# jinlinyi/PerspectiveFields

Hardware: NVIDIA H100
Metric: images/sec at 640x480 (Paramnet-360Cities-edina), H100 vs ref CPU (higher is better)
Workload: dtype f32 via 3x bf16 split MMA, fp32 accumulate

## Files before the change

include/pf_b200.h:

```cpp
#ifndef PF_B200_H_
#define PF_B200_H_

#include <stddef.h>
#include <stdint.h>

#ifdef __cplusplus
extern "C" {
#endif

#define PF_ABI_VERSION 2

typedef struct pf_engine* pf_handle;

enum pf_status { PF_OK = 0, PF_ERR_ARG = -1, PF_ERR_CUDA = -2, PF_ERR_WEIGHT = -3, PF_ERR_WORKSPACE = -4 };

enum pf_dtype { PF_F32 = 0, PF_BF16 = 1 };

enum pf_param_net { PF_PARAM_NONE = 0, PF_PARAM_CENTERED = 1 , PF_PARAM_UNCENTERED = 2  };

typedef struct pf_model_desc {
  int gravity_classes;
  int latitude_classes;
  int param_net;
  int param_input_size;
  float pixel_mean[3];
  float pixel_std[3];
} pf_model_desc;

typedef struct pf_batch {
  int n;
  const uint8_t* images_u8;
  const int64_t* image_offset;
  const float* images_chw;
  const int32_t* height;
  const int32_t* width;
  float* pred_gravity;
  float* pred_latitude;
  float* gravity_original;
  const int64_t* gravity_original_offset;
  float* latitude_original;
  const int64_t* latitude_original_offset;
  float* params;
} pf_batch;

int pf_abi_version(void);
const char* pf_last_error(void);

int64_t pf_kernel_launch_count(void);

int pf_create(int device, const pf_model_desc* desc, pf_handle* out);
int pf_create_sized(int device, const pf_model_desc* desc, int net_h, int net_w, pf_handle* out);
int pf_destroy(pf_handle h);

int pf_set_weight(pf_handle h, const char* name, const void* dev_ptr, int64_t numel, int dtype);
int pf_finalize(pf_handle h);

int64_t pf_workspace_bytes(pf_handle h, int n, int max_h);

int pf_forward(pf_handle h, const pf_batch* batch, void* workspace, int64_t workspace_bytes, void* stream);

int pf_profile_enable(pf_handle h, int on );
int pf_profile_read(pf_handle h, double* out21);
int pf_profile_kernels_enable(pf_handle h, int max_launches);
int pf_profile_kernels_read(pf_handle h, char* buf, int cap);

int pf_set_option(pf_handle h, const char* name, int value);

int pf_debug_enable(pf_handle h, int on);
int pf_debug_count(pf_handle h);
const char* pf_debug_name(pf_handle h, int i);
int64_t pf_debug_numel(pf_handle h, const char* name);
int pf_debug_copy(pf_handle h, const char* name, float* dst_dev, int64_t numel, void* stream);

typedef struct pf_camera {
  int32_t height, width;
  double focal_rel;
  double elevation, roll;
  double cx_rel, cy_rel;
  int64_t up_offset;
  int64_t lat_offset;
} pf_camera;
int pf_camera_fields(int device, const pf_camera* cams, int n, float* up, float* lat, void* stream);
int pf_camera_fields_vp(int device, const pf_camera* cams, const double* vp, int n, float* up, float* lat, void* stream);

typedef struct pf_pano_view {
  int32_t height, width;
  double f, xi;
  double az, el, roll;
  int64_t im_offset;
  int64_t field_offset;
} pf_pano_view;
int pf_pano_views(int device, const uint8_t* pano, int pano_h, int pano_w, const pf_pano_view* views, int n, uint8_t* im, float* ntheta,
                  float* nphi, float* up, float* lat, float* xy, double* offset, int32_t* status, void* stream);

typedef struct pf_equi_view {
  int32_t height, width;
  double vfov;
  double azimuth, elevation, roll;
  double ar;
  int64_t offset;
} pf_equi_view;
enum pf_equi_dtype { PF_EQUI_U8 = 0, PF_EQUI_F32 = 1 };
enum pf_equi_mode { PF_EQUI_BILINEAR = 0, PF_EQUI_NEAREST = 1 };
enum pf_equi_out { PF_EQUI_CAST = 0, PF_EQUI_UNIT = 1 };
int pf_equi_views(int device, const void* pano, int pano_h, int pano_w, int channels, int dtype, const pf_equi_view* views, int n, int mode,
                  int out_kind, int swap_rb, void* im, void* stream);

typedef struct pf_draw_canvas {
  int32_t height, width;
  int64_t img_offset;
  int64_t out_offset;
  int64_t lat_offset;
  int64_t up_offset;
  int64_t up_stride[3];
  int32_t density;
  int32_t arrow_inv_len;
  float arrow_rgb[3];
  float alpha_fill, alpha_line;
  int32_t draw_lat, draw_up;
} pf_draw_canvas;
int pf_draw_fields(int device, const pf_draw_canvas* canvases, int n, const uint8_t* img, uint8_t* out, const float* lat, const float* up,
                   void* stream);

typedef struct pf_comm* pf_comm_handle;
int pf_comm_unique_id(void* id128);
int pf_comm_create(int device, int rank, int nranks, const void* id128, pf_comm_handle* out);
int pf_comm_destroy(pf_comm_handle c);
int pf_gather(pf_comm_handle c, int root, int count, void* const* dev_ptrs, const int64_t* bytes, const int32_t* peer, void* stream);

typedef struct pf_jpeg* pf_jpeg_handle;
int pf_jpeg_create(int device, int max_threads , pf_jpeg_handle* out);
int pf_jpeg_destroy(pf_jpeg_handle j);
int pf_jpeg_info(pf_jpeg_handle j, const uint8_t* data, int64_t length, int32_t* height, int32_t* width);
int pf_jpeg_decode_batch(pf_jpeg_handle j, int n, const uint8_t* const* data, const int64_t* length, const int32_t* height,
                         const int32_t* width, uint8_t* blob, const int64_t* offset, void* stream);


int pf_op_conv_gemm(const float* x, int B, int H, int W, int Cin, const void* whi, const void* wlo, const float* bias,
                    int N, int KH, int KW, int stride, int pad, int in_relu, int act, const float* res, int res_relu,
                    float* y, void* stream);
typedef struct pf_tma_pred { const float* w; const float* b; float* out; int nc, mode; } pf_tma_pred;
typedef struct pf_tma_op {
  int mode;
  int64_t M; int K;
  int B, H, W, Cin;
  int N, groups;
  const void* a_hi; const void* a_lo; int lda, a_c0, a_gc;
  const void* a2_hi; const void* a2_lo; int lda2, c_split, a2_c0;
  const void* w_hi; const void* w_lo; const float* bias; int bias_mode, bias_gstride;
  int act; const float* gamma;
  const float* res; int ldr, r_coff, r_gcoff, res_relu;
  const float* res2; int ldr2, r2_coff, r2_gcoff;
  float* C; int ldc, c_coff, c_gcoff;
  void* s_hi; void* s_lo; int lds, s_coff, s_gcoff, split_relu;
  int phase4;
  int npred; pf_tma_pred pred[2];
  int force_bn, force_kb;
  int picked_bn, picked_kb;
  int force_sched, picked_sched;
} pf_tma_op;
int pf_op_tma(pf_tma_op* op, void* stream);
int pf_op_tma_bf16(pf_tma_op* op, void* stream);
int pf_op_conv1_ring(const void* c_hi, const void* c_lo, int B, int H, int W, const float* wf, const float* bias, float* out,
                     const float* pg_w, const float* pg_b, float* pg_out, const float* pl_w, const float* pl_b, float* pl_out, void* stream);
int pf_tma_pick_tile(int mode, int64_t M, int N, int K, int sm_count, int* bn, int* kb);
int pf_op_layernorm(const float* x, float* y, int64_t rows, int C, const float* w, const float* b, float eps, void* stream);
int pf_op_attention(const float* q, const float* kv, float* out, int B, int N, int C, int heads, void* stream);
int pf_op_attention_mma(const float* q, const float* kv, float* out, int B, int N, int C, int heads, void* stream);
int pf_op_attention_tc(const float* q, const float* kv, float* out, int B, int N, int C, int heads, void* stream);
int pf_op_attention_tc_bf16(const float* q, const float* kv, float* out, int B, int N, int C, int heads, void* stream);
int pf_op_attention_tc_keys(const float* q, const float* kv, float* out, int B, int N, int NKV, int C, int heads, int bf16, void* stream);
int pf_op_dwconv3x3_gelu(const float* x, float* y, int B, int H, int W, int C, const float* w9c, const float* bias, void* stream);
int pf_op_dwconv7x7(const float* x, float* y, int B, int H, int W, int C, const float* w49c, const float* bias, void* stream);
int pf_op_upsample2x(const float* x, float* y, int B, int H, int W, int C, void* stream);
int pf_op_preprocess(const uint8_t* img_dev, int H, int W, const float* mean3, const float* std3, float* y, void* stream);
int pf_op_preprocess_sized(const uint8_t* img_dev, int H, int W, int net_h, int net_w, const float* mean3, const float* std3, float* y, void* stream);
int pf_op_resize_u8(const uint8_t* img_dev, int H, int W, int new_h, int new_w, uint8_t* out_dev, void* stream);
int pf_op_resize_f32(const float* img_dev, int H, int W, int C, int new_h, int new_w, float* out_dev, void* stream);
int pf_op_fill_stream(float* dst, int64_t numel, float value, void* stream);
int pf_op_argmax_decode(const float* logits, float* field, int B, int HW, int NC, int is_gravity, void* stream);
int pf_op_pred_argmax_decode(const float* feat, int ld, int coff, const float* w, const float* bias, float* field, int B, int HW, int NC,
                             int is_gravity, void* stream);
int pf_op_postprocess(const float* vec, const float* lat, int n, const int32_t* height, const int32_t* width,
                      float* gravity_original, const int64_t* gravity_original_offset, float* latitude_original,
                      const int64_t* latitude_original_offset, int lat_is_sin, void* stream);
int pf_op_postprocess_sized(const float* vec, const float* lat, int n, int net_h, int net_w, const int32_t* height, const int32_t* width,
                            float* gravity_original, const int64_t* gravity_original_offset, float* latitude_original,
                            const int64_t* latitude_original_offset, int lat_is_sin, void* stream);

#ifdef __cplusplus
}
#endif
#endif
```

perspectivefields_b200/_native.py:

```python
import ctypes
import os
import subprocess

_HERE = os.path.dirname(os.path.abspath(__file__))
ROOT = os.path.dirname(_HERE)
LIB_PATH = os.path.join(_HERE, "libpf_b200.so")
SRC_DIR = os.path.join(_HERE, "csrc")
HEADER = os.path.join(ROOT, "include", "pf_b200.h")

PF_F32, PF_BF16 = 0, 1
PF_PARAM_NONE, PF_PARAM_CENTERED, PF_PARAM_UNCENTERED = 0, 1, 2

NVCC_FLAGS = ["-gencode", "arch=compute_90a,code=sm_90a", "-O3", "-lineinfo", "-std=c++17",
              "-Xcompiler", "-fPIC", "-shared", "-ldl"]


class pf_model_desc(ctypes.Structure):
    _fields_ = [("gravity_classes", ctypes.c_int), ("latitude_classes", ctypes.c_int), ("param_net", ctypes.c_int),
                ("param_input_size", ctypes.c_int), ("pixel_mean", ctypes.c_float * 3), ("pixel_std", ctypes.c_float * 3)]


class pf_camera(ctypes.Structure):
    _fields_ = [("height", ctypes.c_int32), ("width", ctypes.c_int32), ("focal_rel", ctypes.c_double), ("elevation", ctypes.c_double),
                ("roll", ctypes.c_double), ("cx_rel", ctypes.c_double), ("cy_rel", ctypes.c_double),
                ("up_offset", ctypes.c_int64), ("lat_offset", ctypes.c_int64)]


class pf_pano_view(ctypes.Structure):
    _fields_ = [("height", ctypes.c_int32), ("width", ctypes.c_int32), ("f", ctypes.c_double), ("xi", ctypes.c_double),
                ("az", ctypes.c_double), ("el", ctypes.c_double), ("roll", ctypes.c_double),
                ("im_offset", ctypes.c_int64), ("field_offset", ctypes.c_int64)]


class pf_equi_view(ctypes.Structure):
    _fields_ = [("height", ctypes.c_int32), ("width", ctypes.c_int32), ("vfov", ctypes.c_double), ("azimuth", ctypes.c_double),
                ("elevation", ctypes.c_double), ("roll", ctypes.c_double), ("ar", ctypes.c_double), ("offset", ctypes.c_int64)]


PF_EQUI_U8, PF_EQUI_F32 = 0, 1
PF_EQUI_BILINEAR, PF_EQUI_NEAREST = 0, 1
PF_EQUI_CAST, PF_EQUI_UNIT = 0, 1


class pf_draw_canvas(ctypes.Structure):
    _fields_ = [("height", ctypes.c_int32), ("width", ctypes.c_int32), ("img_offset", ctypes.c_int64), ("out_offset", ctypes.c_int64),
                ("lat_offset", ctypes.c_int64), ("up_offset", ctypes.c_int64), ("up_stride", ctypes.c_int64 * 3),
                ("density", ctypes.c_int32), ("arrow_inv_len", ctypes.c_int32), ("arrow_rgb", ctypes.c_float * 3),
                ("alpha_fill", ctypes.c_float), ("alpha_line", ctypes.c_float), ("draw_lat", ctypes.c_int32), ("draw_up", ctypes.c_int32)]


class pf_batch(ctypes.Structure):
    _fields_ = [("n", ctypes.c_int),
                ("images_u8", ctypes.c_void_p), ("image_offset", ctypes.POINTER(ctypes.c_int64)),
                ("images_chw", ctypes.c_void_p),
                ("height", ctypes.POINTER(ctypes.c_int32)), ("width", ctypes.POINTER(ctypes.c_int32)),
                ("pred_gravity", ctypes.c_void_p), ("pred_latitude", ctypes.c_void_p),
                ("gravity_original", ctypes.c_void_p), ("gravity_original_offset", ctypes.POINTER(ctypes.c_int64)),
                ("latitude_original", ctypes.c_void_p), ("latitude_original_offset", ctypes.POINTER(ctypes.c_int64)),
                ("params", ctypes.c_void_p)]


class pf_tma_pred(ctypes.Structure):
    _fields_ = [("w", ctypes.c_void_p), ("b", ctypes.c_void_p), ("out", ctypes.c_void_p), ("nc", ctypes.c_int), ("mode", ctypes.c_int)]


def _fields(spec):
    types = {"int": ctypes.c_int, "ptr": ctypes.c_void_p, "i64": ctypes.c_int64}
    out = []
    for decl in spec.split(";"):
        t, names = decl.split(None, 1)
        out += [(n.strip(), types[t]) for n in names.split(",")]
    return out


class pf_tma_op(ctypes.Structure):
    _fields_ = _fields("int mode; i64 M; int K, B, H, W, Cin, N, groups; ptr a_hi, a_lo; int lda, a_c0, a_gc; ptr a2_hi, a2_lo;"
                       "int lda2, c_split, a2_c0; ptr w_hi, w_lo, bias; int bias_mode, bias_gstride, act; ptr gamma, res;"
                       "int ldr, r_coff, r_gcoff, res_relu; ptr res2; int ldr2, r2_coff, r2_gcoff; ptr C; int ldc, c_coff, c_gcoff;"
                       "ptr s_hi, s_lo; int lds, s_coff, s_gcoff, split_relu, phase4, npred") + \
        [("pred", pf_tma_pred * 2)] + _fields("int force_bn, force_kb, picked_bn, picked_kb, force_sched, picked_sched")


def _sources():
    return sorted(os.path.join(SRC_DIR, f) for f in os.listdir(SRC_DIR) if f.endswith((".cu", ".cuh"))) + [HEADER]


def needs_build():
    if not os.path.exists(LIB_PATH):
        return True
    t = os.path.getmtime(LIB_PATH)
    return any(os.path.getmtime(s) > t for s in _sources())


def build(force=False, verbose=False):
    if not force and not needs_build():
        return LIB_PATH
    nvcc = os.environ.get("NVCC", "/usr/local/cuda/bin/nvcc")
    cmd = [nvcc] + NVCC_FLAGS + [os.path.join(SRC_DIR, "pf_b200.cu"), "-o", LIB_PATH + ".tmp"]
    if verbose:
        cmd.insert(1, "-Xptxas=-v")
    r = subprocess.run(cmd, capture_output=True, text=True)
    if r.returncode != 0:
        raise RuntimeError("nvcc failed:\n" + " ".join(cmd) + "\n" + r.stdout + r.stderr)
    os.replace(LIB_PATH + ".tmp", LIB_PATH)
    if verbose:
        print(r.stderr)
    return LIB_PATH


_lib = None


def lib():
    global _lib
    if _lib is not None:
        return _lib
    if not os.path.exists(LIB_PATH):
        raise RuntimeError(f"{LIB_PATH} is missing: run `python -c 'import __graft_entry__ as g; g.build()'` "
                           "(perspectivefields_b200 has no CPU or PyTorch fallback)")
    L = ctypes.CDLL(os.environ.get("PF_B200_LIB") or LIB_PATH)
    vp, i32, i64, f32 = ctypes.c_void_p, ctypes.c_int, ctypes.c_int64, ctypes.c_float
    sig = {
        "pf_abi_version": (i32, []),
        "pf_last_error": (ctypes.c_char_p, []),
        "pf_kernel_launch_count": (i64, []),
        "pf_create": (i32, [i32, ctypes.POINTER(pf_model_desc), ctypes.POINTER(vp)]),
        "pf_create_sized": (i32, [i32, ctypes.POINTER(pf_model_desc), i32, i32, ctypes.POINTER(vp)]),
        "pf_destroy": (i32, [vp]),
        "pf_set_weight": (i32, [vp, ctypes.c_char_p, vp, i64, i32]),
        "pf_finalize": (i32, [vp]),
        "pf_workspace_bytes": (i64, [vp, i32, i32]),
        "pf_forward": (i32, [vp, ctypes.POINTER(pf_batch), vp, i64, vp]),
        "pf_profile_enable": (i32, [vp, i32]),
        "pf_profile_read": (i32, [vp, ctypes.POINTER(ctypes.c_double)]),
        "pf_profile_kernels_enable": (i32, [vp, i32]),
        "pf_profile_kernels_read": (i32, [vp, ctypes.c_char_p, i32]),
        "pf_debug_enable": (i32, [vp, i32]),
        "pf_debug_count": (i32, [vp]),
        "pf_debug_name": (ctypes.c_char_p, [vp, i32]),
        "pf_debug_numel": (i64, [vp, ctypes.c_char_p]),
        "pf_debug_copy": (i32, [vp, ctypes.c_char_p, vp, i64, vp]),
        "pf_op_conv_gemm": (i32, [vp, i32, i32, i32, i32, vp, vp, vp, i32, i32, i32, i32, i32, i32, i32, vp, i32, vp, vp]),
        "pf_op_tma": (i32, [ctypes.POINTER(pf_tma_op), vp]),
        "pf_op_tma_bf16": (i32, [ctypes.POINTER(pf_tma_op), vp]),
        "pf_op_conv1_ring": (i32, [vp, vp, i32, i32, i32, vp, vp, vp, vp, vp, vp, vp, vp, vp, vp]),
        "pf_tma_pick_tile": (i32, [i32, i64, i32, i32, i32, ctypes.POINTER(i32), ctypes.POINTER(i32)]),
        "pf_set_option": (i32, [vp, ctypes.c_char_p, i32]),
        "pf_camera_fields": (i32, [i32, ctypes.POINTER(pf_camera), i32, vp, vp, vp]),
        "pf_camera_fields_vp": (i32, [i32, ctypes.POINTER(pf_camera), ctypes.POINTER(ctypes.c_double), i32, vp, vp, vp]),
        "pf_draw_fields": (i32, [i32, ctypes.POINTER(pf_draw_canvas), i32, vp, vp, vp, vp, vp]),
        "pf_pano_views": (i32, [i32, vp, i32, i32, ctypes.POINTER(pf_pano_view), i32, vp, vp, vp, vp, vp, vp, vp, vp, vp]),
        "pf_equi_views": (i32, [i32, vp, i32, i32, i32, i32, ctypes.POINTER(pf_equi_view), i32, i32, i32, i32, vp, vp]),
        "pf_op_layernorm": (i32, [vp, vp, i64, i32, vp, vp, f32, vp]),
        "pf_op_attention": (i32, [vp, vp, vp, i32, i32, i32, i32, vp]),
        "pf_op_attention_mma": (i32, [vp, vp, vp, i32, i32, i32, i32, vp]),
        "pf_op_attention_tc": (i32, [vp, vp, vp, i32, i32, i32, i32, vp]),
        "pf_op_attention_tc_bf16": (i32, [vp, vp, vp, i32, i32, i32, i32, vp]),
        "pf_op_attention_tc_keys": (i32, [vp, vp, vp, i32, i32, i32, i32, i32, i32, vp]),
        "pf_op_dwconv3x3_gelu": (i32, [vp, vp, i32, i32, i32, i32, vp, vp, vp]),
        "pf_op_dwconv7x7": (i32, [vp, vp, i32, i32, i32, i32, vp, vp, vp]),
        "pf_op_upsample2x": (i32, [vp, vp, i32, i32, i32, i32, vp]),
        "pf_op_preprocess": (i32, [vp, i32, i32, ctypes.POINTER(f32), ctypes.POINTER(f32), vp, vp]),
        "pf_op_preprocess_sized": (i32, [vp, i32, i32, i32, i32, ctypes.POINTER(f32), ctypes.POINTER(f32), vp, vp]),
        "pf_op_resize_u8": (i32, [vp, i32, i32, i32, i32, vp, vp]),
        "pf_op_resize_f32": (i32, [vp, i32, i32, i32, i32, i32, vp, vp]),
        "pf_op_argmax_decode": (i32, [vp, vp, i32, i32, i32, i32, vp]),
        "pf_op_fill_stream": (i32, [vp, i64, f32, vp]),
        "pf_op_pred_argmax_decode": (i32, [vp, i32, i32, vp, vp, vp, i32, i32, i32, i32, vp]),
        "pf_op_postprocess": (i32, [vp, vp, i32, ctypes.POINTER(ctypes.c_int32), ctypes.POINTER(ctypes.c_int32), vp, ctypes.POINTER(i64), vp,
                                    ctypes.POINTER(i64), i32, vp]),
        "pf_op_postprocess_sized": (i32, [vp, vp, i32, i32, i32, ctypes.POINTER(ctypes.c_int32), ctypes.POINTER(ctypes.c_int32), vp,
                                          ctypes.POINTER(i64), vp, ctypes.POINTER(i64), i32, vp]),
        "pf_comm_unique_id": (i32, [vp]),
        "pf_comm_create": (i32, [i32, i32, i32, vp, ctypes.POINTER(vp)]),
        "pf_comm_destroy": (i32, [vp]),
        "pf_gather": (i32, [vp, i32, i32, ctypes.POINTER(vp), ctypes.POINTER(i64), ctypes.POINTER(ctypes.c_int32), vp]),
        "pf_jpeg_create": (i32, [i32, i32, ctypes.POINTER(vp)]),
        "pf_jpeg_destroy": (i32, [vp]),
        "pf_jpeg_info": (i32, [vp, vp, i64, ctypes.POINTER(ctypes.c_int32), ctypes.POINTER(ctypes.c_int32)]),
        "pf_jpeg_decode_batch": (i32, [vp, i32, ctypes.POINTER(vp), ctypes.POINTER(i64), ctypes.POINTER(ctypes.c_int32),
                                       ctypes.POINTER(ctypes.c_int32), vp, ctypes.POINTER(i64), vp]),
    }
    for name, (res, args) in sig.items():
        try:
            fn = getattr(L, name)
        except AttributeError:
            if os.environ.get("PF_B200_LIB"):
                continue
            raise
        fn.restype, fn.argtypes = res, args
    if L.pf_abi_version() != 2:
        raise RuntimeError("libpf_b200.so ABI version mismatch")
    _lib = L
    return L


EXPORTS = ["pf_abi_version", "pf_last_error", "pf_kernel_launch_count", "pf_create", "pf_create_sized", "pf_destroy", "pf_set_weight",
           "pf_finalize", "pf_workspace_bytes", "pf_forward", "pf_profile_enable", "pf_profile_read", "pf_profile_kernels_enable",
           "pf_profile_kernels_read", "pf_set_option", "pf_debug_enable", "pf_debug_count", "pf_debug_name", "pf_debug_numel",
           "pf_debug_copy", "pf_camera_fields", "pf_camera_fields_vp", "pf_pano_views", "pf_equi_views", "pf_draw_fields", "pf_comm_unique_id", "pf_comm_create", "pf_comm_destroy", "pf_gather",
           "pf_jpeg_create", "pf_jpeg_destroy", "pf_jpeg_info", "pf_jpeg_decode_batch",
           "pf_op_conv_gemm", "pf_op_tma", "pf_op_tma_bf16", "pf_op_conv1_ring", "pf_tma_pick_tile", "pf_op_layernorm", "pf_op_attention",
           "pf_op_attention_mma", "pf_op_attention_tc", "pf_op_attention_tc_bf16", "pf_op_attention_tc_keys", "pf_op_dwconv3x3_gelu",
           "pf_op_dwconv7x7", "pf_op_upsample2x", "pf_op_preprocess", "pf_op_preprocess_sized", "pf_op_fill_stream", "pf_op_resize_u8",
           "pf_op_resize_f32", "pf_op_argmax_decode", "pf_op_pred_argmax_decode", "pf_op_postprocess", "pf_op_postprocess_sized"]


class PfError(RuntimeError):
    pass


def check(status):
    if status < 0:
        raise PfError(f"libpf_b200: {lib().pf_last_error().decode()} (status {status})")
    return status
```

perspectivefields_b200/csrc/gemm_tma.cuh:

```cuda
#pragma once
#include <cuda.h>

#include "tc_ptx.cuh"

namespace pf {

constexpr int MODE_GEMM = 0, MODE_HALO = 1;
constexpr int kTmaThreads = 384;
constexpr int kHaloBytes = 180 * 128;

struct TmaGemmParams {
  int M;
  int B, H, W;
  int Cin;
  int N, K;
  int a_c0, a_gc;
  int c_split, a2_c0;
  int groups;
  int b_row0;
  const float* bias; int bias_mode, bias_gstride;
  int act; const float* gamma;
  const float* res;  int ldr, r_coff, r_gcoff, res_relu;
  const float* res2; int ldr2, r2_coff, r2_gcoff;
  float* C; int ldc, c_coff, c_gcoff;
  __nv_bfloat16* Shi; __nv_bfloat16* Slo; int lds, s_coff, s_gcoff, split_relu;
  const float* pred_w; const float* pred_b; float* pred_out; int pred_nc, pred_mode;
  int phase4;
};

template <int BN, int MODE, int KB, bool PP = false, int NP = 3> struct TmaCfg {
  static_assert(KB == 32 || KB == 64, "KB");
  static_assert(BN % 32 == 0 && BN <= 256, "BN");
  static_assert(!PP || MODE == MODE_GEMM, "the ping-pong schedule is a GEMM-mode schedule");
  static_assert(NP == 1 || NP == 3, "NP");
  static constexpr int kPlanes = NP == 3 ? 2 : 1;
  static constexpr int kTileM = PP ? 64 : 128;
  static constexpr int kBPlane = BN * KB * 2;
  static constexpr int kAPlane = kTileM * KB * 2;
  static constexpr int kStage = (MODE == MODE_GEMM ? kPlanes * kAPlane : 0) + kPlanes * kBPlane;
  static constexpr int kABuf = kPlanes * kHtPlaneBytes;
  static constexpr int kAccPitch = 68;
  static constexpr int kAccStage = 2 * 64 * kAccPitch * 4;
  static constexpr int kBudget = 225 * 1024 - kAccStage - (MODE == MODE_HALO ? 2 * kABuf : 0);
  static constexpr int kStagesRaw = kBudget / kStage;
  static constexpr int kStages = kStagesRaw > 16 ? 16 : kStagesRaw;
  static constexpr int kSmemBytes = (MODE == MODE_HALO ? 2 * kABuf : 0) + kStages * kStage + kAccStage + 512 + 1024;
  static_assert(kStages >= 2, "ring too shallow");
  static_assert(kSmemBytes <= 227 * 1024, "shared memory per block");
};

__device__ __forceinline__ void mbar_expect_tx(uint32_t bar, uint32_t bytes) {
  asm volatile("mbarrier.arrive.expect_tx.shared::cta.b64 _, [%0], %1;\n" ::"r"(bar), "r"(bytes) : "memory");
}
__device__ __forceinline__ void tma_load_2d(uint32_t dst, const CUtensorMap* map, uint32_t bar, int c0, int c1) {
  asm volatile("cp.async.bulk.tensor.2d.shared::cluster.global.mbarrier::complete_tx::bytes [%0], [%1, {%3, %4}], [%2];\n"
               ::"r"(dst), "l"(reinterpret_cast<uint64_t>(map)), "r"(bar), "r"(c0), "r"(c1) : "memory");
}
__device__ __forceinline__ void tma_load_4d(uint32_t dst, const CUtensorMap* map, uint32_t bar, int c0, int c1, int c2, int c3) {
  asm volatile("cp.async.bulk.tensor.4d.shared::cluster.global.mbarrier::complete_tx::bytes [%0], [%1, {%3, %4, %5, %6}], [%2];\n"
               ::"r"(dst), "l"(reinterpret_cast<uint64_t>(map)), "r"(bar), "r"(c0), "r"(c1), "r"(c2), "r"(c3) : "memory");
}
__device__ __forceinline__ void tma_prefetch_desc(const CUtensorMap* map) {
  asm volatile("prefetch.tensormap [%0];\n" ::"l"(reinterpret_cast<uint64_t>(map)) : "memory");
}

struct TmaMaps {
  CUtensorMap a_hi, a_lo, a2_hi, a2_lo, b_hi, b_lo;
};

template <int BN, int MODE, int KB, bool PP = false, int NP = 3>
__global__ void __launch_bounds__(kTmaThreads, 1) gemm_tma_kernel(const __grid_constant__ TmaMaps maps, const TmaGemmParams p, int tiles_x, int tiles_y) {
  using Cfg = TmaCfg<BN, MODE, KB, PP, NP>;
  constexpr bool kLo = NP == 3;
  constexpr int NS = Cfg::kStages;
  constexpr int SPC = 9 * (64 / KB);
  constexpr int kConsumerWarps = PP ? 4 : 8;
  extern __shared__ unsigned char smem_dyn[];
  const uint32_t raw = smem_u32(smem_dyn);
  const uint32_t sbase = (raw + 1023u) & ~1023u;
  unsigned char* sm = smem_dyn + (sbase - raw);
  const uint32_t a_base = sbase;
  const uint32_t ring = sbase + (MODE == MODE_HALO ? 2 * Cfg::kABuf : 0);
  const uint32_t acc_base = ring + NS * Cfg::kStage;
  const uint32_t bars = acc_base + Cfg::kAccStage;
  auto full_b = [&](int s) { return bars + 8u * s; };
  auto empty_b = [&](int s) { return bars + 8u * (NS + s); };
  auto full_a = [&](int i) { return bars + 8u * (2 * NS + i); };
  auto empty_a = [&](int i) { return bars + 8u * (2 * NS + 2 + i); };
  auto order_b = [&](int w) { return bars + 8u * (2 * NS + 4 + w); };

  const int tid = threadIdx.x, lane = tid & 31, warp = tid >> 5;
  const int n_tiles = cdiv(p.N, BN);
  const int m_tiles = MODE == MODE_GEMM ? cdiv(p.M, Cfg::kTileM) : p.B * tiles_x * tiles_y;
  const int total_tiles = m_tiles * n_tiles * p.groups;
  const int nchunks = MODE == MODE_HALO ? p.Cin / 64 : 0;
  const int nk = MODE == MODE_GEMM ? p.K / KB : nchunks * SPC;
  const bool b_resident = MODE == MODE_HALO && nchunks == 1 && SPC <= NS;

  if (tid == 0) {
    tma_prefetch_desc(&maps.a_hi); tma_prefetch_desc(&maps.b_hi);
    if (kLo) { tma_prefetch_desc(&maps.a_lo); tma_prefetch_desc(&maps.b_lo); }
    for (int s = 0; s < NS; ++s) { mbar_init(full_b(s), 1); mbar_init(empty_b(s), kConsumerWarps); }
    for (int i = 0; i < 2; ++i) { mbar_init(full_a(i), 1); mbar_init(empty_a(i), kConsumerWarps); mbar_init(order_b(i), 4); }
    fence_mbar_init();
  }
  __syncthreads();
  pdl_wait();
  pdl_launch();

  auto decode = [&](int tile, int& mt, int& g, int& n0) {
    n0 = (tile % n_tiles) * BN;
    tile /= n_tiles;
    g = tile % p.groups;
    mt = tile / p.groups;
  };

  if (warp < 4) {
    asm volatile("setmaxnreg.dec.sync.aligned.u32 40;\n");
    if (warp == 0 && lane == 0) {
      int it = 0;
      for (int tile = blockIdx.x; tile < total_tiles; tile += gridDim.x) {
        int mt, g, n0;
        decode(tile, mt, g, n0);
        const int brow = p.b_row0 + g * p.N + n0;
        if (b_resident && it > 0) break;
        for (int kc = 0; kc < nk; ++kc, ++it) {
          const int s = it % NS;
          mbar_wait(empty_b(s), ((it / NS) & 1) ^ 1);
          mbar_expect_tx(full_b(s), Cfg::kStage);
          const uint32_t st = ring + s * Cfg::kStage;
          int kcol;
          if (MODE == MODE_GEMM) {
            kcol = kc * KB;
            tma_load_2d(st, &maps.a_hi, full_b(s), p.a_c0 + g * p.a_gc + kcol, mt * Cfg::kTileM);
            if (kLo) tma_load_2d(st + Cfg::kAPlane, &maps.a_lo, full_b(s), p.a_c0 + g * p.a_gc + kcol, mt * Cfg::kTileM);
          } else {
            const int c = kc / SPC, u = kc - c * SPC;
            kcol = KB == 32 ? (u >> 1) * p.Cin + c * 64 + (u & 1) * 32 : u * p.Cin + c * 64;
          }
          const uint32_t bdst = st + (MODE == MODE_GEMM ? Cfg::kPlanes * Cfg::kAPlane : 0);
          tma_load_2d(bdst, &maps.b_hi, full_b(s), kcol, brow);
          if (kLo) tma_load_2d(bdst + Cfg::kBPlane, &maps.b_lo, full_b(s), kcol, brow);
        }
      }
    } else if (MODE == MODE_HALO && warp == 1 && lane == 0) {
      int ita = 0;
      for (int tile = blockIdx.x; tile < total_tiles; tile += gridDim.x) {
        int mt, g, n0;
        decode(tile, mt, g, n0);
        const int tx = mt % tiles_x, ty = (mt / tiles_x) % tiles_y, bimg = mt / (tiles_x * tiles_y);
        for (int c = 0; c < nchunks; ++c, ++ita) {
          const int buf = ita & 1;
          mbar_wait(empty_a(buf), ((ita >> 1) & 1) ^ 1);
          mbar_expect_tx(full_a(buf), Cfg::kPlanes * kHaloBytes);
          const uint32_t dst = a_base + buf * Cfg::kABuf;
          const int ci = c * 64;
          if (p.c_split > 0 && ci >= p.c_split) {
            tma_load_4d(dst, &maps.a2_hi, full_a(buf), p.a2_c0 + ci - p.c_split, tx * kHtTileW - 1, ty * kHtTileH - 1, bimg);
            if (kLo) tma_load_4d(dst + kHtPlaneBytes, &maps.a2_lo, full_a(buf), p.a2_c0 + ci - p.c_split, tx * kHtTileW - 1, ty * kHtTileH - 1, bimg);
          } else {
            tma_load_4d(dst, &maps.a_hi, full_a(buf), p.a_c0 + g * p.a_gc + ci, tx * kHtTileW - 1, ty * kHtTileH - 1, bimg);
            if (kLo) tma_load_4d(dst + kHtPlaneBytes, &maps.a_lo, full_a(buf), p.a_c0 + g * p.a_gc + ci, tx * kHtTileW - 1, ty * kHtTileH - 1, bimg);
          }
        }
      }
    }
    return;
  }

  asm volatile("setmaxnreg.inc.sync.aligned.u32 232;\n");
  const int wg = (warp >> 2) - 1;
  const int wt = tid & 127;
  float* stage = reinterpret_cast<float*>(sm + (acc_base - sbase)) + wg * 64 * Cfg::kAccPitch;
  const int erow = wt & 63, eh = wt >> 6;
  const int r = PP ? erow : wg * 64 + erow;
  constexpr int kTileStep = PP ? 2 : 1;
  float acc[BN / 2];
  int it = 0, ita = 0;
  for (int tl = PP ? wg : 0, tile = blockIdx.x + tl * gridDim.x; tile < total_tiles; tile += kTileStep * gridDim.x, tl += kTileStep) {
    int mt, g, n0;
    decode(tile, mt, g, n0);
    if (PP) {
      it = tl * nk;
      if (tl > 0) mbar_wait(order_b(wg ^ 1), ((tl - 1) >> 1) & 1);
    }
    int prev_s = -1, prev_buf = -1;
    fence_regs(acc);
    for (int kc = 0; kc < nk; ++kc, ++it) {
      const int s = it % NS;
      uint32_t a_hi, a_lo;
      bool chunk_end = false;
      int buf = 0;
      if (MODE == MODE_HALO) {
        const int c = kc / SPC, u = kc - c * SPC;
        const int tap = KB == 32 ? (u >> 1) : u, ky = tap / 3, kx = tap - ky * 3;
        buf = ita & 1;
        if (u == 0) mbar_wait(full_a(buf), (ita >> 1) & 1);
        a_hi = a_base + buf * Cfg::kABuf + ((ky + 8 * wg) * kHtHaloW + kx) * 128 + (KB == 32 ? (u & 1) * 64 : 0);
        a_lo = a_hi + kHtPlaneBytes;
        chunk_end = u == SPC - 1;
      } else {
        a_hi = ring + s * Cfg::kStage + (PP ? 0 : wg * 64 * KB * 2);
        a_lo = a_hi + Cfg::kAPlane;
      }
      const int sb = b_resident ? kc : s;
      if (!b_resident || tl == 0) mbar_wait(full_b(sb), b_resident ? 0 : ((it / NS) & 1));
      const uint32_t b_hi = ring + sb * Cfg::kStage + (MODE == MODE_GEMM ? Cfg::kPlanes * Cfg::kAPlane : 0);
      const uint64_t dah = MODE == MODE_HALO ? ht_a_desc(a_hi) : wgmma_tile_desc<KB>(a_hi);
      const uint64_t dbh = wgmma_tile_desc<KB>(b_hi);
      wgmma_fence();
      if (kLo) {
        const uint64_t dal = MODE == MODE_HALO ? ht_a_desc(a_lo) : wgmma_tile_desc<KB>(a_lo);
        const uint64_t dbl = wgmma_tile_desc<KB>(b_hi + Cfg::kBPlane);
#pragma unroll
        for (int kk = 0; kk < KB / 16; ++kk) {
          const uint32_t first = (kc | kk) ? 1u : 0u;
          wgmma_bf16<BN>(acc, dal + 2 * kk, dbh + 2 * kk, first);
          wgmma_bf16<BN>(acc, dah + 2 * kk, dbl + 2 * kk, 1u);
          wgmma_bf16<BN>(acc, dah + 2 * kk, dbh + 2 * kk, 1u);
        }
      } else {
#pragma unroll
        for (int kk = 0; kk < KB / 16; ++kk) wgmma_bf16<BN>(acc, dah + 2 * kk, dbh + 2 * kk, (kc | kk) ? 1u : 0u);
      }
      wgmma_commit();
      wgmma_wait<1>();
      if (lane == 0 && prev_s >= 0) {
        if (!b_resident) mbar_arrive(empty_b(prev_s));
        if (MODE == MODE_HALO && prev_buf >= 0) mbar_arrive(empty_a(prev_buf));
      }
      prev_s = s;
      prev_buf = chunk_end ? buf : -1;
      if (MODE == MODE_HALO && chunk_end) ++ita;
    }
    if (PP && lane == 0) mbar_arrive(order_b(wg));
    wgmma_wait<0>();
    fence_regs(acc);
    if (lane == 0 && prev_s >= 0) {
      if (!b_resident) mbar_arrive(empty_b(prev_s));
      if (MODE == MODE_HALO && prev_buf >= 0) mbar_arrive(empty_a(prev_buf));
    }

    long long m;
    bool valid;
    int cls_off = 0;
    int bimg = 0, oy = 0, ox = 0;
    if (MODE == MODE_GEMM) {
      m = (long long)mt * Cfg::kTileM + r;
      valid = m < p.M;
    } else {
      const int tx = mt % tiles_x, ty = (mt / tiles_x) % tiles_y;
      bimg = mt / (tiles_x * tiles_y);
      oy = ty * kHtTileH + (r >> 3); ox = tx * kHtTileW + (r & 7);
      valid = oy < p.H && ox < p.W;
      m = ((long long)bimg * p.H + oy) * p.W + ox;
      if (p.bias_mode == 2) {
        const int ry = oy == 0 ? 0 : (oy == p.H - 1 ? 2 : 1);
        const int rx = ox == 0 ? 0 : (ox == p.W - 1 ? 2 : 1);
        cls_off = (ry * 3 + rx) * p.N;
      }
    }
    const float* __restrict__ bias = p.bias ? p.bias + (long long)g * p.bias_gstride : nullptr;
    const int frow = (wt >> 5) * 16 + (lane >> 2), fcol = 2 * (lane & 3);
#pragma unroll
    for (int rd = 0; rd < (BN + 63) / 64; ++rd) {
      named_bar_sync(1 + wg, 128);
#pragma unroll
      for (int jb = 0; jb < 8; ++jb) {
        const int cb = rd * 8 + jb;
        if (cb < BN / 8) {
          float* d0 = stage + frow * Cfg::kAccPitch + jb * 8 + fcol;
          *reinterpret_cast<float2*>(d0) = make_float2(acc[4 * cb], acc[4 * cb + 1]);
          *reinterpret_cast<float2*>(d0 + 8 * Cfg::kAccPitch) = make_float2(acc[4 * cb + 2], acc[4 * cb + 3]);
        }
      }
      named_bar_sync(1 + wg, 128);
      const int ch = 2 * rd + eh;
      const bool ph4 = MODE == MODE_HALO && BN == 128 && p.phase4;
      const bool staged_split = p.Shi && !ph4;
      float o[32];
      if (ch < BN / 32) {
        const int nb = n0 + ch * 32;
        const long long mo = ph4 ? ((long long)bimg * 2 * p.H + 2 * oy + (ch >> 1)) * (2 * p.W) + 2 * ox + (ch & 1) : m;
        const int nbo = ph4 ? 0 : nb;
        const bool chunk_ok = nb < p.N;
        const float* srow = stage + erow * Cfg::kAccPitch + eh * 32;
#pragma unroll
        for (int j = 0; j < 32; j += 4) {
          const float4 t = *reinterpret_cast<const float4*>(srow + j);
          o[j] = t.x; o[j + 1] = t.y; o[j + 2] = t.z; o[j + 3] = t.w;
        }
        if (valid && chunk_ok) {
          if (p.bias_mode) {
#pragma unroll
            for (int j = 0; j < 32; j += 4) {
              const float4 bv = __ldg(reinterpret_cast<const float4*>(bias + cls_off + nb + j));
              o[j] += bv.x; o[j + 1] += bv.y; o[j + 2] += bv.z; o[j + 3] += bv.w;
            }
          }
          if (p.act == 1) {
#pragma unroll
            for (int j = 0; j < 32; ++j) o[j] = fmaxf(o[j], 0.f);
          } else if (p.act == 2) {
#pragma unroll
            for (int j = 0; j < 32; ++j) o[j] = gelu_erf(o[j]);
          }
          if (p.gamma) {
#pragma unroll
            for (int j = 0; j < 32; j += 4) {
              const float4 gv = __ldg(reinterpret_cast<const float4*>(p.gamma + nb + j));
              o[j] *= gv.x; o[j + 1] *= gv.y; o[j + 2] *= gv.z; o[j + 3] *= gv.w;
            }
          }
          if (p.res) {
            const float* rp = p.res + m * p.ldr + p.r_coff + g * p.r_gcoff + nb;
#pragma unroll
            for (int j = 0; j < 32; j += 4) {
              float4 rv = *reinterpret_cast<const float4*>(rp + j);
              if (p.res_relu) { rv.x = fmaxf(rv.x, 0.f); rv.y = fmaxf(rv.y, 0.f); rv.z = fmaxf(rv.z, 0.f); rv.w = fmaxf(rv.w, 0.f); }
              o[j] += rv.x; o[j + 1] += rv.y; o[j + 2] += rv.z; o[j + 3] += rv.w;
            }
          }
          if (p.res2) {
            const float* rp = p.res2 + m * p.ldr2 + p.r2_coff + g * p.r2_gcoff + nb;
#pragma unroll
            for (int j = 0; j < 32; j += 4) {
              const float4 rv = *reinterpret_cast<const float4*>(rp + j);
              o[j] += rv.x; o[j + 1] += rv.y; o[j + 2] += rv.z; o[j + 3] += rv.w;
            }
          }
          if (MODE == MODE_HALO && (BN == 32 || BN == 128) && p.pred_w) {
            float v0 = __ldg(p.pred_b), v1 = p.pred_nc > 1 ? __ldg(p.pred_b + 1) : 0.f;
#pragma unroll
            for (int j = 0; j < 32; j += 4) {
              const float4 w0 = __ldg(reinterpret_cast<const float4*>(p.pred_w + j));
              v0 = fmaf(o[j], w0.x, v0); v0 = fmaf(o[j + 1], w0.y, v0); v0 = fmaf(o[j + 2], w0.z, v0); v0 = fmaf(o[j + 3], w0.w, v0);
              if (p.pred_nc > 1) {
                const float4 w1 = __ldg(reinterpret_cast<const float4*>(p.pred_w + 32 + j));
                v1 = fmaf(o[j], w1.x, v1); v1 = fmaf(o[j + 1], w1.y, v1); v1 = fmaf(o[j + 2], w1.z, v1); v1 = fmaf(o[j + 3], w1.w, v1);
              }
            }
            const long long HWl = (long long)p.H * p.W * (ph4 ? 4 : 1);
            const long long bi = mo / HWl, pix = mo - bi * HWl;
            float* po = p.pred_out + bi * p.pred_nc * HWl + pix;
            if (p.pred_mode == 1) {
              const float nrm = fmaxf(sqrtf(v0 * v0 + v1 * v1), 1e-12f);
              po[0] = v0 / nrm; po[HWl] = v1 / nrm;
            } else {
              po[0] = fminf(fmaxf(v0, -1.f), 1.f);
            }
          }
        }
        if (chunk_ok && (p.C || (p.Shi && !staged_split))) {
          const bool odd = lane & 1;
          const bool valid_p = __shfl_xor_sync(0xffffffffu, (int)valid, 1) != 0;
          const long long mo_p = mo + (odd ? -1 : 1) * (ph4 ? 2 : 1);
          const long long moA = odd ? mo_p : mo, moB = odd ? mo : mo_p;
          const bool vA = odd ? valid_p : valid, vB = odd ? valid : valid_p;
          if (p.C) {
            float* cA = p.C + moA * p.ldc + p.c_coff + g * p.c_gcoff + nbo + (odd ? 4 : 0);
            float* cB = p.C + moB * p.ldc + p.c_coff + g * p.c_gcoff + nbo + (odd ? 4 : 0);
#pragma unroll
            for (int t = 0; t < 4; ++t) {
              float k[4], rr[4];
#pragma unroll
              for (int e = 0; e < 4; ++e) {
                k[e] = odd ? o[8 * t + 4 + e] : o[8 * t + e];
                rr[e] = __shfl_xor_sync(0xffffffffu, odd ? o[8 * t + e] : o[8 * t + 4 + e], 1);
              }
              if (vA) *reinterpret_cast<float4*>(cA + 8 * t) = odd ? make_float4(rr[0], rr[1], rr[2], rr[3]) : make_float4(k[0], k[1], k[2], k[3]);
              if (vB) *reinterpret_cast<float4*>(cB + 8 * t) = odd ? make_float4(k[0], k[1], k[2], k[3]) : make_float4(rr[0], rr[1], rr[2], rr[3]);
            }
          }
          if (p.Shi && !staged_split) {
            const long long sA = moA * p.lds + p.s_coff + g * p.s_gcoff + nbo + (odd ? 8 : 0);
            const long long sB = moB * p.lds + p.s_coff + g * p.s_gcoff + nbo + (odd ? 8 : 0);
#pragma unroll
            for (int t = 0; t < 2; ++t) {
              float k[8], rr[8];
#pragma unroll
              for (int e = 0; e < 8; ++e) {
                const float mine = odd ? o[16 * t + 8 + e] : o[16 * t + e], give = odd ? o[16 * t + e] : o[16 * t + 8 + e];
                k[e] = p.split_relu ? fmaxf(mine, 0.f) : mine;
                rr[e] = __shfl_xor_sync(0xffffffffu, p.split_relu ? fmaxf(give, 0.f) : give, 1);
              }
              uint4 kh, kl, rh, rl;
              split_bf16x2(k[0], k[1], kh.x, kl.x); split_bf16x2(k[2], k[3], kh.y, kl.y);
              split_bf16x2(k[4], k[5], kh.z, kl.z); split_bf16x2(k[6], k[7], kh.w, kl.w);
              split_bf16x2(rr[0], rr[1], rh.x, rl.x); split_bf16x2(rr[2], rr[3], rh.y, rl.y);
              split_bf16x2(rr[4], rr[5], rh.z, rl.z); split_bf16x2(rr[6], rr[7], rh.w, rl.w);
              if (vA) {
                *reinterpret_cast<uint4*>(p.Shi + sA + 16 * t) = odd ? rh : kh;
                *reinterpret_cast<uint4*>(p.Slo + sA + 16 * t) = odd ? rl : kl;
              }
              if (vB) {
                *reinterpret_cast<uint4*>(p.Shi + sB + 16 * t) = odd ? kh : rh;
                *reinterpret_cast<uint4*>(p.Slo + sB + 16 * t) = odd ? kl : rl;
              }
            }
          }
        }
      }
      if (staged_split) {
        named_bar_sync(1 + wg, 128);
        unsigned char* sS = reinterpret_cast<unsigned char*>(stage);
        if (ch < BN / 32) {
#pragma unroll
          for (int t = 0; t < 4; ++t) {
            uint4 h, l;
            float k[8];
#pragma unroll
            for (int e = 0; e < 8; ++e) k[e] = p.split_relu ? fmaxf(o[8 * t + e], 0.f) : o[8 * t + e];
            split_bf16x2(k[0], k[1], h.x, l.x); split_bf16x2(k[2], k[3], h.y, l.y);
            split_bf16x2(k[4], k[5], h.z, l.z); split_bf16x2(k[6], k[7], h.w, l.w);
            const int off = erow * 128 + (((eh * 4 + t) ^ (erow & 7)) << 4);
            *reinterpret_cast<uint4*>(sS + off) = h;
            *reinterpret_cast<uint4*>(sS + 64 * 128 + off) = l;
          }
        }
        named_bar_sync(1 + wg, 128);
#pragma unroll
        for (int i = wt; i < 2 * 64 * 8; i += 128) {
          const int lo_plane = i >> 9, rr = (i >> 3) & 63, pc = i & 7;
          const int col = rd * 64 + pc * 8;
          if (col >= BN || n0 + col >= p.N) continue;
          long long mr;
          bool vr;
          if (MODE == MODE_GEMM) {
            mr = (long long)mt * Cfg::kTileM + (PP ? 0 : wg * 64) + rr;
            vr = mr < p.M;
          } else {
            const int rt = wg * 64 + rr, tx = mt % tiles_x, ty = (mt / tiles_x) % tiles_y;
            const int py = ty * kHtTileH + (rt >> 3), px = tx * kHtTileW + (rt & 7);
            vr = py < p.H && px < p.W;
            mr = ((long long)bimg * p.H + py) * p.W + px;
          }
          if (!vr) continue;
          const uint4 v = *reinterpret_cast<const uint4*>(sS + lo_plane * 64 * 128 + rr * 128 + ((pc ^ (rr & 7)) << 4));
          *reinterpret_cast<uint4*>((lo_plane ? p.Slo : p.Shi) + mr * p.lds + p.s_coff + g * p.s_gcoff + n0 + col) = v;
        }
      }
    }
  }
}

}
```

perspectivefields_b200/csrc/pf_b200.cu:

```cuda
#include "../../include/pf_b200.h"

#include <cuda_runtime.h>
#include <nvtx3/nvToolsExt.h>

#include <atomic>
#include <cctype>
#include <cmath>
#include <cstdarg>
#include <cstdio>
#include <cstdlib>
#include <cstring>
#include <map>
#include <mutex>
#include <string>
#include <functional>
#include <unordered_map>
#include <vector>

#include "common.cuh"
#include "tma_host.cuh"
#include "attention_mma.cuh"
#include "layers.cuh"
#include "prepost.cuh"
#include "pano.cuh"
#include "equi.cuh"
#include "draw.cuh"
#include "comm.cuh"
#include "jpeg.cuh"

using namespace pf;

static thread_local std::string g_err;
static std::atomic<long long> g_launches{0};

static int fail(int code, const char* fmt, ...) {
  char buf[1024];
  va_list ap;
  va_start(ap, fmt);
  vsnprintf(buf, sizeof(buf), fmt, ap);
  va_end(ap);
  g_err = buf;
  return code;
}
#define CU(expr)                                                                                    \
  do {                                                                                              \
    cudaError_t e__ = (expr);                                                                       \
    if (e__ != cudaSuccess) return fail(PF_ERR_CUDA, "%s: %s (%s:%d)", #expr, cudaGetErrorString(e__), __FILE__, __LINE__); \
  } while (0)
static char g_crumb[96] = "";
static bool sync_debug() {
  static int v = -1;
  if (v < 0) v = getenv("PF_SYNC_DEBUG") ? 1 : 0;
  return v == 1;
}
struct KernelProf {
  bool on = false;
  cudaStream_t st = nullptr;
  std::vector<cudaEvent_t> pool;
  size_t used = 0;
  struct Rec { const char* expr; cudaEvent_t a, b; };
  std::vector<Rec> recs;
  cudaEvent_t next() { return used < pool.size() ? pool[used++] : nullptr; }
};
static thread_local KernelProf* tl_kp = nullptr;
#define LAUNCHED(expr)                                                                              \
  do {                                                                                              \
    KernelProf* kp__ = tl_kp;                                                                       \
    cudaEvent_t ka__ = (kp__ && kp__->on) ? kp__->next() : nullptr;                                 \
    if (ka__) cudaEventRecord(ka__, kp__->st);                                                      \
    cudaError_t e__ = (expr);                                                                       \
    g_launches.fetch_add(1, std::memory_order_relaxed);                                             \
    if (ka__) {                                                                                     \
      cudaEvent_t kb__ = kp__->next();                                                              \
      if (kb__) { cudaEventRecord(kb__, kp__->st); kp__->recs.push_back({#expr, ka__, kb__}); }     \
    }                                                                                               \
    if (e__ == cudaSuccess && sync_debug()) e__ = cudaDeviceSynchronize();                          \
    if (e__ != cudaSuccess) return fail(PF_ERR_CUDA, "%s: %s (%s:%d, after tap '%s')", #expr, cudaGetErrorString(e__), __FILE__, __LINE__, g_crumb); \
  } while (0)
struct NvtxRange {
  explicit NvtxRange(const char* name) { nvtxRangePushA(name); }
  ~NvtxRange() { nvtxRangePop(); }
};
#define TRY(expr)                \
  do {                           \
    int r__ = (expr);            \
    if (r__ != PF_OK) return r__; \
  } while (0)

static const int kMitDims[4] = {64, 128, 320, 512};
static const int kMitHeads[4] = {1, 2, 5, 8};
static const int kMitDepths[4] = {3, 4, 18, 3};
static const int kMitSr[4] = {8, 4, 2, 1};
static const int kCnxDims[4] = {96, 192, 384, 768};
static const int kCnxDepths[4] = {3, 3, 9, 3};

struct WeightRef { const void* p; long long numel; int dtype; };
struct GemmW { const __nv_bfloat16* hi = nullptr; const __nv_bfloat16* lo = nullptr; const float* b = nullptr; };
struct LnW { const float* w = nullptr; const float* b = nullptr; };

struct MitBlockW { LnW ln1, srln, ln2; GemmW q, sr, kv, proj, fc1, fc2; const float* dw_w; const float* dw_b; };
struct CnxBlockW { const float* dw_w; const float* dw_b; LnW ln; GemmW pw1, pw2; const float* gamma; };

struct Arena {
  char* base = nullptr;
  long long cap = 0, off = 0, peak = 0;
  bool dry = false, keep = false;
  void* alloc(long long bytes) {
    off = (off + 255) & ~255LL;
    void* p = dry ? nullptr : base + off;
    off += bytes;
    if (off > peak) peak = off;
    return p;
  }
  float* f(long long n) { return (float*)alloc(n * 4); }
  long long mark() const { return off; }
  void release(long long m) { if (!keep) off = m; }
};

struct pf_engine {
  int device = 0;
  pf_model_desc desc{};
  int net_h = kNet, net_w = kNet;
  bool finalized = false;
  std::unordered_map<std::string, WeightRef> weights;
  const float *embed1_w, *embed1_b, *llenc_w, *llenc_b;
  LnW embed_ln[4], stage_norm[4];
  GemmW embed[4];
  GemmW embed1g, llencg;
  std::vector<MitBlockW> blocks[4];
  GemmW proc[4];
  GemmW rcu[4][2][2];
  GemmW conv0, conv1;
  GemmW conv1p;
  const float *conv1f_w, *conv1f_b;
  bool use_fork = false;
  cudaStream_t side = nullptr;
  cudaEvent_t ev_fork = nullptr, ev_join = nullptr;
  bool use_dwln = false;
  bool use_pdl = true;
  bool decode_only = false;
  bool use_attn_split = true;
  bool use_phase = true;
  const float *pred_g_w, *pred_g_b, *pred_l_w, *pred_l_b;
  const float *pn_stem_w, *pn_stem_b;
  LnW pn_stem_ln, pn_ds_ln[4], pn_norm;
  GemmW pn_ds[4];
  std::vector<CnxBlockW> pn_blocks[4];
  const float *pn_head_w, *pn_head_b;
  struct DevTable { int ksize; int* bounds; int* coeffs; };
  std::map<std::pair<int, int>, DevTable> tables;
  char* table_dev = nullptr;
  char* table_host = nullptr;
  long long table_off = 0;
  KernelProf kp;
  struct MapKey {
    const void* base; long long d0, d1, d2; int kind, box, kb;
    bool operator==(const MapKey& o) const { return base == o.base && d0 == o.d0 && d1 == o.d1 && d2 == o.d2 && kind == o.kind && box == o.box && kb == o.kb; }
  };
  struct MapKeyHash {
    size_t operator()(const MapKey& k) const {
      size_t h = std::hash<const void*>()(k.base);
      for (long long v : {k.d0, k.d1, k.d2, (long long)k.kind, (long long)k.box, (long long)k.kb}) h = h * 1000003u ^ std::hash<long long>()(v);
      return h;
    }
  };
  std::unordered_map<MapKey, CUtensorMap, MapKeyHash> map_cache;
  bool use_stem_tc = true;
  bool use_attn_mma = true;
  bool bf16 = false;
  int sm_count = 132;
  bool profile = false;
  struct ProfRec { cudaEvent_t a, b; double flops; int cfg; int M, N, K, KH, stride, groups, Cin; };
  std::vector<ProfRec> prof;
  std::vector<cudaEvent_t> ev_pool;
  bool debug = false;
  std::vector<std::pair<std::string, std::pair<const float*, long long>>> taps;
};

static int get_w(pf_engine* e, const std::string& name, int dtype, long long numel, const void** out) {
  auto it = e->weights.find(name);
  if (it == e->weights.end()) return fail(PF_ERR_WEIGHT, "missing weight '%s'", name.c_str());
  if (it->second.dtype != dtype) return fail(PF_ERR_WEIGHT, "weight '%s': wrong dtype", name.c_str());
  if (it->second.numel != numel) return fail(PF_ERR_WEIGHT, "weight '%s': numel %lld, expected %lld", name.c_str(), it->second.numel, numel);
  *out = it->second.p;
  return PF_OK;
}
static int get_f(pf_engine* e, const std::string& n, long long numel, const float** out) { return get_w(e, n, PF_F32, numel, (const void**)out); }
static int get_gemm(pf_engine* e, const std::string& n, long long N, long long K, long long nbias, GemmW* g, int groups = 1) {
  TRY(get_w(e, n + ".whi", PF_BF16, groups * N * K, (const void**)&g->hi));
  TRY(get_w(e, n + ".wlo", PF_BF16, groups * N * K, (const void**)&g->lo));
  TRY(get_f(e, n + ".b", groups * nbias, &g->b));
  return PF_OK;
}
static int get_ln(pf_engine* e, const std::string& n, int C, LnW* l) {
  TRY(get_f(e, n + ".w", C, &l->w));
  TRY(get_f(e, n + ".b", C, &l->b));
  return PF_OK;
}

static int resolve_weights(pf_engine* e) {
  char nm[128];
  TRY(get_f(e, "embed1.w", 147 * 64, &e->embed1_w));
  TRY(get_f(e, "embed1.b", 64, &e->embed1_b));
  TRY(get_f(e, "llenc.w", 147 * 64, &e->llenc_w));
  TRY(get_f(e, "llenc.b", 64, &e->llenc_b));
  TRY(get_gemm(e, "embed1g", 64, 160, 64, &e->embed1g));
  TRY(get_gemm(e, "llencg", 64, 160, 64, &e->llencg));
  for (int s = 0; s < 4; ++s) {
    const int C = kMitDims[s];
    snprintf(nm, sizeof nm, "embed%d.ln", s + 1);
    TRY(get_ln(e, nm, C, &e->embed_ln[s]));
    if (s > 0) {
      snprintf(nm, sizeof nm, "embed%d", s + 1);
      TRY(get_gemm(e, nm, C, 9LL * kMitDims[s - 1], C, &e->embed[s]));
    }
    e->blocks[s].resize(kMitDepths[s]);
    for (int i = 0; i < kMitDepths[s]; ++i) {
      MitBlockW& b = e->blocks[s][i];
      char p[64];
      snprintf(p, sizeof p, "s%d.b%d.", s + 1, i);
      std::string P(p);
      TRY(get_ln(e, P + "ln1", C, &b.ln1));
      TRY(get_gemm(e, P + "q", C, C, C, &b.q));
      if (kMitSr[s] > 1) {
        TRY(get_gemm(e, P + "sr", C, (long long)kMitSr[s] * kMitSr[s] * C, C, &b.sr));
        TRY(get_ln(e, P + "srln", C, &b.srln));
      }
      TRY(get_gemm(e, P + "kv", 2 * C, C, 2 * C, &b.kv));
      TRY(get_gemm(e, P + "proj", C, C, C, &b.proj));
      TRY(get_ln(e, P + "ln2", C, &b.ln2));
      TRY(get_gemm(e, P + "fc1", 4 * C, C, 4 * C, &b.fc1));
      TRY(get_f(e, P + "dw.w", 9LL * 4 * C, &b.dw_w));
      TRY(get_f(e, P + "dw.b", 4 * C, &b.dw_b));
      TRY(get_gemm(e, P + "fc2", C, 4 * C, C, &b.fc2));
    }
    snprintf(nm, sizeof nm, "s%d.norm", s + 1);
    TRY(get_ln(e, nm, C, &e->stage_norm[s]));
  }
  for (int l = 0; l < 4; ++l) {
    snprintf(nm, sizeof nm, "head.proc%d", l + 1);
    TRY(get_gemm(e, nm, 512, 9LL * kMitDims[l], 9 * 512, &e->proc[l]));
  }
  for (int f = 0; f < 4; ++f)
    for (int u = 0; u < 2; ++u) {
      if (f == 3 && u == 0) continue;
      for (int c = 0; c < 2; ++c) {
        snprintf(nm, sizeof nm, "head.f%d.u%d.c%d", f + 1, u + 1, c + 1);
        TRY(get_gemm(e, nm, 256, 2304, 256, &e->rcu[f][u][c], 2));
      }
    }
  TRY(get_gemm(e, "head.conv0", 64, 9 * 320, 64, &e->conv0, 2));
  TRY(get_gemm(e, "head.conv1", 32, 9 * 64, 32, &e->conv1, 2));
  TRY(get_gemm(e, "head.conv1p", 128, 9 * 64, 128, &e->conv1p, 2));
  TRY(get_f(e, "head.conv1f.w", 2LL * 9 * 64 * 32, &e->conv1f_w));
  TRY(get_f(e, "head.conv1f.b", 64, &e->conv1f_b));
  TRY(get_f(e, "head.pred_g.w", 32LL * e->desc.gravity_classes, &e->pred_g_w));
  TRY(get_f(e, "head.pred_g.b", e->desc.gravity_classes, &e->pred_g_b));
  TRY(get_f(e, "head.pred_l.w", 32LL * e->desc.latitude_classes, &e->pred_l_w));
  TRY(get_f(e, "head.pred_l.b", e->desc.latitude_classes, &e->pred_l_b));
  if (e->desc.param_net != PF_PARAM_NONE) {
    TRY(get_f(e, "pn.stem.w", 48 * 96, &e->pn_stem_w));
    TRY(get_f(e, "pn.stem.b", 96, &e->pn_stem_b));
    TRY(get_ln(e, "pn.stem.ln", 96, &e->pn_stem_ln));
    for (int k = 1; k < 4; ++k) {
      snprintf(nm, sizeof nm, "pn.ds%d.ln", k);
      TRY(get_ln(e, nm, kCnxDims[k - 1], &e->pn_ds_ln[k]));
      snprintf(nm, sizeof nm, "pn.ds%d", k);
      TRY(get_gemm(e, nm, kCnxDims[k], 4LL * kCnxDims[k - 1], kCnxDims[k], &e->pn_ds[k]));
    }
    for (int s = 0; s < 4; ++s) {
      const int C = kCnxDims[s];
      e->pn_blocks[s].resize(kCnxDepths[s]);
      for (int j = 0; j < kCnxDepths[s]; ++j) {
        CnxBlockW& b = e->pn_blocks[s][j];
        char p[64];
        snprintf(p, sizeof p, "pn.s%d.b%d.", s, j);
        std::string P(p);
        TRY(get_f(e, P + "dw.w", 49LL * C, &b.dw_w));
        TRY(get_f(e, P + "dw.b", C, &b.dw_b));
        TRY(get_ln(e, P + "ln", C, &b.ln));
        TRY(get_gemm(e, P + "pw1", 4 * C, C, 4 * C, &b.pw1));
        TRY(get_gemm(e, P + "pw2", C, 4 * C, C, &b.pw2));
        TRY(get_f(e, P + "gamma", C, &b.gamma));
      }
    }
    TRY(get_ln(e, "pn.norm", 768, &e->pn_norm));
    TRY(get_f(e, "pn.head.w", 5 * 768, &e->pn_head_w));
    TRY(get_f(e, "pn.head.b", 5, &e->pn_head_b));
  }
  return PF_OK;
}

struct Fwd {
  pf_engine* e;
  Arena ar;
  cudaStream_t st;
  bool dry;
  int n;

  int tap(const char* name, const float* p, long long numel) {
    if (!e->debug) return PF_OK;
    float* cp = ar.f(numel);
    if (dry) return PF_OK;
    snprintf(g_crumb, sizeof g_crumb, "%s", name);
    if (sync_debug()) fprintf(stderr, "[pf tap] %s cp=%p (+%lld of cap %lld) p=%p numel=%lld\n", name, (void*)cp, (long long)((char*)cp - ar.base), ar.cap, (const void*)p, numel);
    CU(cudaMemcpyAsync(cp, p, numel * 4, cudaMemcpyDeviceToDevice, st));
    if (sync_debug()) CU(cudaDeviceSynchronize());
    e->taps.push_back({name, {cp, numel}});
    return PF_OK;
  }
  int tapf(const float* p, long long numel, const char* fmt, ...) {
    if (!e->debug) return PF_OK;
    char buf[96];
    va_list ap;
    va_start(ap, fmt);
    vsnprintf(buf, sizeof buf, fmt, ap);
    va_end(ap);
    return tap(buf, p, numel);
  }

  SplitT salloc(long long pixels, int ld) {
    SplitT t;
    t.hi = (__nv_bfloat16*)ar.alloc(pixels * ld * 2);
    t.lo = (__nv_bfloat16*)ar.alloc(pixels * ld * 2);
    t.ld = ld;
    return t;
  }
  int tap_split(const char* name, const SplitT& t, long long numel) {
    if (!e->debug) return PF_OK;
    float* cp = ar.f(numel);
    if (dry) return PF_OK;
    snprintf(g_crumb, sizeof g_crumb, "%s", name);
    LAUNCHED((merge_split_kernel<<<(unsigned)cdivl(numel, 256), 256, 0, st>>>(t.hi, t.lo, cp, numel), cudaGetLastError()));
    e->taps.push_back({name, {cp, numel}});
    return PF_OK;
  }
  static cudaError_t gemm_tma_gemm_mode(const TmaMaps& maps, const TmaGemmParams& p, int bn, int kb, bool pp, int np, int sms, cudaStream_t st, const PredTail* pred) {
    return gemm_tma_launch(MODE_GEMM, maps, p, bn, kb, pp, np, sms, st, pred);
  }
  static cudaError_t gemm_tma_halo_mode(const TmaMaps& maps, const TmaGemmParams& p, int bn, int kb, bool pp, int np, int sms, cudaStream_t st, const PredTail* pred) {
    return gemm_tma_launch(MODE_HALO, maps, p, bn, kb, pp, np, sms, st, pred);
  }
  int np() const { return e->bf16 ? 1 : 3; }
  int force_bn = 0, force_kb = 0;
  int force_sched = 0;
  int picked_bn = 0, picked_kb = 0, picked_sched = 0;
  int pick_tile(int mode, const TmaGemmParams& p, const PredTail* pred, int& bn, int& kb, bool& pp) {
    tma_pick_tile(mode, p.M, p.N, p.K, e->sm_count, bn, kb);
    if (force_bn) { bn = force_bn; kb = tma_pick_kb(bn, p.K, mode); }
    if (force_kb) kb = force_kb;
    pp = mode == MODE_GEMM && (force_sched ? force_sched == 2 : tma_pick_pingpong(p.M, p.N, p.K, bn, e->sm_count));
    if (const char* msg = gemm_tma_check(mode, p, bn, kb, pred != nullptr, pp, np())) return fail(PF_ERR_ARG, "TMA engine, %s (bn %d, kb %d): %s", mode == MODE_GEMM ? "GEMM mode" : "halo mode", bn, kb, msg);
    picked_bn = bn; picked_kb = kb; picked_sched = mode == MODE_GEMM ? (pp ? 2 : 1) : 0;
    return PF_OK;
  }
  int launch_tma(int mode, const TmaMaps& maps, const TmaGemmParams& p, int bn, int kb, bool pp, const PredTail* pred = nullptr) {
    if (e->profile) {
      pf_engine::ProfRec r{};
      for (cudaEvent_t* ev : {&r.a, &r.b}) {
        if (e->ev_pool.empty()) { CU(cudaEventCreate(ev)); }
        else { *ev = e->ev_pool.back(); e->ev_pool.pop_back(); }
      }
      const double Mrows = mode == MODE_GEMM ? (double)p.M : (double)p.B * p.H * p.W;
      r.flops = 2.0 * Mrows * (double)p.N * (double)p.K * (double)p.groups;
      r.cfg = mode == MODE_GEMM ? 5 : 6;
      r.M = (int)Mrows; r.N = p.N; r.K = p.K; r.KH = mode == MODE_GEMM ? 1 : 3; r.stride = 1; r.groups = p.groups; r.Cin = p.Cin;
      CU(cudaEventRecord(r.a, st));
      if (mode == MODE_GEMM) LAUNCHED(gemm_tma_gemm_mode(maps, p, bn, kb, pp, np(), e->sm_count, st, pred));
      else LAUNCHED(gemm_tma_halo_mode(maps, p, bn, kb, pp, np(), e->sm_count, st, pred));
      CU(cudaEventRecord(r.b, st));
      e->prof.push_back(r);
      return PF_OK;
    }
    if (mode == MODE_GEMM) LAUNCHED(gemm_tma_gemm_mode(maps, p, bn, kb, pp, np(), e->sm_count, st, pred));
    else LAUNCHED(gemm_tma_halo_mode(maps, p, bn, kb, pp, np(), e->sm_count, st, pred));
    return PF_OK;
  }
  struct Epi {
    float* C = nullptr; int ldc = 0, c_coff = 0, c_gcoff = 0;
    SplitT S; int s_coff = 0, s_gcoff = 0, split_relu = 0;
    int act = 0; const float* gamma = nullptr;
    const float* res = nullptr; int ldr = 0, r_coff = 0, r_gcoff = 0, res_relu = 0;
    const float* res2 = nullptr; int ldr2 = 0, r2_coff = 0, r2_gcoff = 0;
    int bias_mode = 1;
    int phase4 = 0;
  };
  static void fill_epi(TmaGemmParams& p, const GemmW& w, const Epi& o, int bias_gstride) {
    p.bias = w.b; p.bias_mode = w.b ? o.bias_mode : 0; p.bias_gstride = bias_gstride;
    p.act = o.act; p.gamma = o.gamma;
    p.res = o.res; p.ldr = o.ldr; p.r_coff = o.r_coff; p.r_gcoff = o.r_gcoff; p.res_relu = o.res_relu;
    p.res2 = o.res2; p.ldr2 = o.ldr2; p.r2_coff = o.r2_coff; p.r2_gcoff = o.r2_gcoff;
    p.C = o.C; p.ldc = o.ldc; p.c_coff = o.c_coff; p.c_gcoff = o.c_gcoff;
    p.Shi = o.S.hi; p.Slo = o.S.lo; p.lds = o.S.ld; p.s_coff = o.s_coff; p.s_gcoff = o.s_gcoff; p.split_relu = o.split_relu;
    p.phase4 = o.phase4;
  }
  template <class F>
  const char* cached_map(CUtensorMap* out, const pf_engine::MapKey& key, F&& make) {
    auto it = e->map_cache.find(key);
    if (it != e->map_cache.end()) { *out = it->second; return nullptr; }
    const char* msg = make(out);
    if (!msg) {
      if (e->map_cache.size() > 20000) e->map_cache.clear();
      e->map_cache.emplace(key, *out);
    }
    return msg;
  }
  const char* map2d(CUtensorMap* m, const void* base, long long cols, long long rows, long long ld, int box_rows, int kb) {
    return cached_map(m, pf_engine::MapKey{base, cols, rows, ld, 0, box_rows, kb}, [&](CUtensorMap* o) { return tma_map_2d(o, base, cols, rows, ld, box_rows, kb); });
  }
  const char* map_halo(CUtensorMap* m, const void* base, int B, int H, int W, int ld) {
    return cached_map(m, pf_engine::MapKey{base, ((long long)B << 32) | (unsigned)H, W, ld, 3, 0, 0}, [&](CUtensorMap* o) { return tma_map_halo(o, base, B, H, W, ld); });
  }
  int tgemm(const SplitT& A, long long M, int K, int a_c0, const GemmW& w, int N, const Epi& o) {
    if (dry) return PF_OK;
    if (K % 32 || N % 32 || A.ld % 8) return fail(PF_ERR_ARG, "tgemm: K/N must be multiples of 32");
    if (o.res2 || o.bias_mode == 2) return fail(PF_ERR_ARG, "tgemm: second residual / border-class bias are halo-mode features");
    TmaGemmParams p{};
    p.M = (int)M; p.Cin = K; p.N = N; p.K = K; p.a_c0 = a_c0; p.groups = 1;
    fill_epi(p, w, o, 0);
    TmaMaps maps{};
    int bn, kb;
    bool pp;
    TRY(pick_tile(MODE_GEMM, p, nullptr, bn, kb, pp));
    const char* msg = nullptr;
    const int a_rows = pp ? 64 : 128;
    if (!msg) msg = map2d(&maps.a_hi, A.hi, A.ld, M, A.ld, a_rows, kb);
    if (!msg) msg = map2d(&maps.a_lo, A.lo, A.ld, M, A.ld, a_rows, kb);
    if (!msg) msg = map2d(&maps.b_hi, w.hi, K, N, K, bn, kb);
    if (!msg) msg = map2d(&maps.b_lo, w.lo, K, N, K, bn, kb);
    if (msg) return fail(PF_ERR_CUDA, "%s", msg);
    maps.a2_hi = maps.a_hi; maps.a2_lo = maps.a_lo;
    return launch_tma(MODE_GEMM, maps, p, bn, kb, pp);
  }
  int thalo(const SplitT& A, int a_c0, int a_gc, const SplitT* A2, int c_split, int a2_c0, int B, int H, int W, int Cin, const GemmW& w, int N,
            int groups, int bias_gstride, const Epi& o, const PredTail* pred = nullptr) {
    if (dry) return PF_OK;
    if (Cin % 64 || N % 32 || (A2 && c_split % 64)) return fail(PF_ERR_ARG, "thalo: Cin must be a multiple of 64, N of 32");
    if (w.b && o.bias_mode == 2 && (H < 2 || W < 2)) return fail(PF_ERR_ARG, "thalo: border-class bias needs H, W >= 2 (got %dx%d)", H, W);
    TmaGemmParams p{};
    p.B = B; p.H = H; p.W = W; p.Cin = Cin; p.N = N; p.K = 9 * Cin; p.a_c0 = a_c0; p.a_gc = a_gc; p.groups = groups;
    p.c_split = A2 ? c_split : 0; p.a2_c0 = a2_c0;
    fill_epi(p, w, o, bias_gstride);
    TmaMaps maps{};
    int bn, kb;
    bool pp;
    TRY(pick_tile(MODE_HALO, p, pred, bn, kb, pp));
    const char* msg = nullptr;
    if (!msg) msg = map_halo(&maps.a_hi, A.hi, B, H, W, A.ld);
    if (!msg) msg = map_halo(&maps.a_lo, A.lo, B, H, W, A.ld);
    if (A2) {
      if (!msg) msg = map_halo(&maps.a2_hi, A2->hi, B, H, W, A2->ld);
      if (!msg) msg = map_halo(&maps.a2_lo, A2->lo, B, H, W, A2->ld);
    } else { maps.a2_hi = maps.a_hi; maps.a2_lo = maps.a_lo; }
    if (!msg) msg = map2d(&maps.b_hi, w.hi, p.K, (long long)groups * N, p.K, bn, kb);
    if (!msg) msg = map2d(&maps.b_lo, w.lo, p.K, (long long)groups * N, p.K, bn, kb);
    if (msg) return fail(PF_ERR_CUDA, "%s", msg);
    return launch_tma(MODE_HALO, maps, p, bn, kb, pp, pred);
  }
  int tconv_gather(const SplitT& A, int B, int H, int W, int Cin, int KH, int stride, int pad, const GemmW& w, int N, const Epi& o) {
    const int OH = (H + 2 * pad - KH) / stride + 1, OW = (W + 2 * pad - KH) / stride + 1;
    const long long M = (long long)B * OH * OW;
    const int K = KH * KH * Cin;
    const long long m = ar.mark();
    SplitT col = salloc(M, K);
    if (!dry) {
      if (Cin % 8) return fail(PF_ERR_ARG, "tconv_gather: Cin %% 8");
      LAUNCHED(launch_pdl(im2col_split_kernel, dim3(ew_grid(M * K / 8)), dim3(256), 0, st, A.hi, A.lo, A.ld, col.hi, col.lo, B, H, W, Cin, OH, OW, KH, stride, pad));
    }
    int r = tgemm(col, M, K, 0, w, N, o);
    ar.release(m);
    return r;
  }
  int ln_split(const float* x, const SplitT& y, long long rows, int C, const LnW& w, float eps, float* yf = nullptr) {
    if (dry) return PF_OK;
    LAUNCHED(layernorm_launch(x, yf, rows, C, w.w, w.b, eps, st, y));
    return PF_OK;
  }
  int ln_split_patch(const float* x, const SplitT& y, const SplitT& patch, long long rows, int C, const LnW& w, float eps, int RH, int RW, int sr) {
    if (dry) return PF_OK;
    LAUNCHED(layernorm_launch(x, nullptr, rows, C, w.w, w.b, eps, st, y, patch, RH, RW, sr));
    return PF_OK;
  }
  int ln(const float* x, float* y, long long rows, int C, const LnW& w, float eps) {
    if (dry) return PF_OK;
    LAUNCHED(layernorm_launch(x, y, rows, C, w.w, w.b, eps, st));
    return PF_OK;
  }
};

constexpr long long kTableSlabBytes = 8LL << 20;
static int get_table(pf_engine* e, int in_size, int out_size, pf_engine::DevTable* out, cudaStream_t st) {
  auto it = e->tables.find({in_size, out_size});
  if (it == e->tables.end()) {
    ResampleTable t = make_resample_table(in_size, out_size);
    const long long nb = (long long)t.bounds.size() * sizeof(int), nc = (long long)t.coeffs.size() * sizeof(int);
    const long long need = ((nb + 255) & ~255LL) + ((nc + 255) & ~255LL);
    if (need > kTableSlabBytes) return fail(PF_ERR_ARG, "image axis of %d pixels is too long for the resize tables", in_size);
    if (e->table_off + need > kTableSlabBytes) {
      CU(cudaStreamSynchronize(st));
      e->tables.clear();
      e->table_off = 0;
    }
    pf_engine::DevTable d{};
    d.ksize = t.ksize;
    const long long o0 = e->table_off, o1 = o0 + ((nb + 255) & ~255LL);
    memcpy(e->table_host + o0, t.bounds.data(), nb);
    memcpy(e->table_host + o1, t.coeffs.data(), nc);
    d.bounds = (int*)(e->table_dev + o0);
    d.coeffs = (int*)(e->table_dev + o1);
    CU(cudaMemcpyAsync(e->table_dev + o0, e->table_host + o0, need, cudaMemcpyHostToDevice, st));
    e->table_off += need;
    it = e->tables.emplace(std::make_pair(in_size, out_size), d).first;
  }
  *out = it->second;
  return PF_OK;
}

static int pre_rows_needed(int H, int OH) {
  const double scale = (double)H / OH;
  const double support = scale < 1.0 ? 1.0 : scale;
  return (int)(kPreRows * scale) + 2 * (int)ceil(support) + 3;
}
static int pre_max_smem_rows(int OW) { return kPreSmemBytes / (OW * 3); }

static int fwd_preprocess(Fwd& F, const pf_batch* bt, float*& x0, PreImage*& d_pre, PostImage*& d_post) {
  pf_engine* e = F.e;
  const pf_model_desc& D = e->desc;
  const int n = F.n;
  const bool dry = F.dry;
  cudaStream_t st = F.st;
  Arena& ar = F.ar;
  const int NH = e->net_h, NW = e->net_w;
  const int max_rows = pre_max_smem_rows(NW);
  x0 = ar.f((long long)n * NH * NW * 4);
  d_pre = (PreImage*)ar.alloc((long long)n * sizeof(PreImage));
  d_post = (PostImage*)ar.alloc((long long)n * sizeof(PostImage));
  if (!dry) {
    if (bt->images_u8) {
      std::vector<PreImage> pre(n);
      int max_h = 1;
      for (int i = 0; i < n; ++i) {
        const int H = bt->height[i], W = bt->width[i];
        if (H < 1 || W < 1) return fail(PF_ERR_ARG, "image %d has size %dx%d", i, H, W);
        pf_engine::DevTable tx, ty;
        TRY(get_table(e, W, NW, &tx, st));
        TRY(get_table(e, H, NH, &ty, st));
        if (ty.ksize + 1 > max_rows) return fail(PF_ERR_ARG, "image %d is too tall (%d rows) for the resize kernel", i, H);
        pre[i] = PreImage{bt->image_offset[i], H, W, tx.ksize, ty.ksize, tx.bounds, tx.coeffs, ty.bounds, ty.coeffs};
        if (H > max_h) max_h = H;
      }
      CU(cudaMemcpyAsync(d_pre, pre.data(), n * sizeof(PreImage), cudaMemcpyHostToDevice, st));
      int rows = pre_rows_needed(max_h, NH);
      if (rows > max_rows) rows = max_rows;
      const int smem = rows * NW * 3;
      LAUNCHED((preprocess_kernel<<<dim3(NH / kPreRows, n), NW, smem, st>>>(bt->images_u8, d_pre, x0, D.pixel_mean[0], D.pixel_mean[1],
                                                                           D.pixel_mean[2], D.pixel_std[0], D.pixel_std[1], D.pixel_std[2], rows, NH, NW),
                cudaGetLastError()));
    } else {
      const long long total = (long long)n * NH * NW;
      LAUNCHED((normalize_chw_kernel<<<(unsigned)cdivl(total, 256), 256, 0, st>>>(bt->images_chw, x0, n, NH, NW, D.pixel_mean[0], D.pixel_mean[1],
                                                                                 D.pixel_mean[2], D.pixel_std[0], D.pixel_std[1], D.pixel_std[2]),
                cudaGetLastError()));
    }
  }
  return PF_OK;
}

static int launch_postprocess(const float* vec, const float* lat, int n, int SH, int SW, const int32_t* height, const int32_t* width, const int64_t* g_off,
                              const int64_t* l_off, float* g_out, float* l_out, int lat_is_sin, PostImage* d_post, cudaStream_t st) {
  std::vector<PostImage> post(n);
  long long total = 0;
  int max_h = 1, max_wp = 4;
  for (int i = 0; i < n; ++i) {
    if (height[i] < 1 || width[i] < 1) return fail(PF_ERR_ARG, "image %d has size %dx%d", i, height[i], width[i]);
    post[i] = PostImage{height[i], width[i], g_off[i], l_off[i], total};
    total += (long long)height[i] * width[i];
    if (height[i] > max_h) max_h = height[i];
    const int wp = (width[i] + 3) / 4 * 4;
    if (wp <= kPostMaxW && wp > max_wp) max_wp = wp;
  }
  CU(cudaMemcpyAsync(d_post, post.data(), n * sizeof(PostImage), cudaMemcpyHostToDevice, st));
  const int smem = post_smem_bytes(SW, max_wp);
  LAUNCHED((postprocess_kernel<<<dim3((unsigned)cdiv(max_h, kPostBand), (unsigned)n), kPostThreads, smem, st>>>(vec, lat, d_post, g_out, l_out, lat_is_sin, SH, SW),
            cudaGetLastError()));
  return PF_OK;
}

static int fwd_tails_post(Fwd& F, const pf_batch* bt, const float* conv1_out, PostImage* d_post, bool pred_done = false) {
  pf_engine* e = F.e;
  const pf_model_desc& D = e->desc;
  const int n = F.n;
  const bool dry = F.dry;
  cudaStream_t st = F.st;
  Arena& ar = F.ar;
  const int HW = e->net_h * e->net_w;
  const bool cls_g = D.gravity_classes != 2, cls_l = D.latitude_classes != 1;
  const bool fused_decode = e->decode_only && (cls_g || cls_l);
  if (e->decode_only && cls_g != cls_l) return fail(PF_ERR_ARG, "decode_only needs both heads to be classification heads");
  const float* vec = dry ? nullptr : bt->pred_gravity;
  const float* lat = dry ? nullptr : bt->pred_latitude;
  if (e->debug) {
    float* rg = ar.f((long long)n * D.gravity_classes * HW);
    float* rl = ar.f((long long)n * D.latitude_classes * HW);
    if (!dry) {
      const unsigned grid = (unsigned)cdivl((long long)n * HW, 128);
      LAUNCHED((pred_tail_kernel<<<grid, 128, D.gravity_classes * 33 * 4, st>>>(conv1_out, 64, 0, e->pred_g_w, e->pred_g_b, rg, n, HW, D.gravity_classes, 0), cudaGetLastError()));
      LAUNCHED((pred_tail_kernel<<<grid, 128, D.latitude_classes * 33 * 4, st>>>(conv1_out, 64, 32, e->pred_l_w, e->pred_l_b, rl, n, HW, D.latitude_classes, 0), cudaGetLastError()));
    }
    TRY(F.tap("head.raw_g", rg, (long long)n * D.gravity_classes * HW));
    TRY(F.tap("head.raw_l", rl, (long long)n * D.latitude_classes * HW));
  }
  if (fused_decode) {
    if (!dry) {
      const unsigned grid = ew_grid((long long)n * HW * 4);
      LAUNCHED((pred_argmax_decode_kernel<<<grid, 256, D.gravity_classes * 37 * 4, st>>>(conv1_out, 64, 0, e->pred_g_w, e->pred_g_b, bt->pred_gravity, n, HW,
                                                                                      D.gravity_classes, 1), cudaGetLastError()));
      LAUNCHED((pred_argmax_decode_kernel<<<grid, 256, D.latitude_classes * 37 * 4, st>>>(conv1_out, 64, 32, e->pred_l_w, e->pred_l_b, bt->pred_latitude, n, HW,
                                                                                       D.latitude_classes, 0), cudaGetLastError()));
    }
  } else {
    if (!dry && !pred_done) {
      const unsigned grid = (unsigned)cdivl((long long)n * HW, 128);
      LAUNCHED((pred_tail_kernel<<<grid, 128, D.gravity_classes * 33 * 4, st>>>(conv1_out, 64, 0, e->pred_g_w, e->pred_g_b, bt->pred_gravity, n, HW,
                                                                             D.gravity_classes, D.gravity_classes == 2 ? 1 : 0), cudaGetLastError()));
      LAUNCHED((pred_tail_kernel<<<grid, 128, D.latitude_classes * 33 * 4, st>>>(conv1_out, 64, 32, e->pred_l_w, e->pred_l_b, bt->pred_latitude, n, HW,
                                                                              D.latitude_classes, D.latitude_classes == 1 ? 2 : 0), cudaGetLastError()));
    }
    if (cls_g) {
      float* dv = ar.f((long long)n * 2 * HW);
      if (!dry) LAUNCHED((argmax_decode_kernel<<<(unsigned)cdivl((long long)n * HW, 256), 256, 0, st>>>(bt->pred_gravity, dv, n, HW, D.gravity_classes, 1), cudaGetLastError()));
      vec = dv;
    }
    if (cls_l) {
      float* dl = ar.f((long long)n * HW);
      if (!dry) LAUNCHED((argmax_decode_kernel<<<(unsigned)cdivl((long long)n * HW, 256), 256, 0, st>>>(bt->pred_latitude, dl, n, HW, D.latitude_classes, 0), cudaGetLastError()));
      lat = dl;
    }
  }
  if (!dry)
    TRY(launch_postprocess(vec, lat, n, e->net_h, e->net_w, bt->height, bt->width, bt->gravity_original_offset, bt->latitude_original_offset, bt->gravity_original,
                           bt->latitude_original, cls_l ? 0 : 1, d_post, st));
  return PF_OK;
}

static int run_forward_tma(Fwd& F, const pf_batch* bt) {
  pf_engine* e = F.e;
  const pf_model_desc& D = e->desc;
  const int n = F.n;
  const bool dry = F.dry;
  cudaStream_t st = F.st;
  Arena& ar = F.ar;
  using Epi = Fwd::Epi;
  const int NH = e->net_h, NW = e->net_w;
  int RH[4], RW[4];
  for (int s = 0; s < 4; ++s) { RH[s] = NH >> (s + 2); RW[s] = NW >> (s + 2); }
  const int nkv = RH[3] * RW[3];
  if ((NH != kNet || NW != kNet) && (!e->use_attn_mma || !e->use_attn_split || !e->use_stem_tc || !e->use_phase))
    return fail(PF_ERR_ARG, "options attn_mma / attn_split / stem_tc / phase_conv1 = 0 (reference paths of the 320 x 320 graph) need a 320 x 320 "
                            "working size; this engine runs at %d x %d", NH, NW);

  float* x0; PreImage* d_pre; PostImage* d_post;
  {
    NvtxRange r_("pf:preprocess");
    TRY(fwd_preprocess(F, bt, x0, d_pre, d_post));
  }
  TRY(F.tap("pre", x0, (long long)n * NH * NW * 4));

  NvtxRange* sect = new NvtxRange("pf:ll_enc");
  struct SectGuard { NvtxRange*& p; ~SectGuard() { delete p; } } sect_guard{sect};
  auto section = [&](const char* name) { delete sect; sect = nullptr; sect = new NvtxRange(name); };
  SplitT cfeat[4];
  for (int s = 0; s < 4; ++s) cfeat[s] = F.salloc((long long)n * RH[s] * RW[s], kMitDims[s]);
  const int LH = NH / 2, LW = NW / 2;
  SplitT ll = F.salloc((long long)n * LH * LW, 64);
  if (e->use_stem_tc) {
    const long long m = ar.mark();
    const long long M = (long long)n * LH * LW;
    SplitT col = F.salloc(M, 160);
    if (!dry) LAUNCHED(launch_pdl(stem_gather_kernel, dim3(ew_grid(stem_gather_threads(n, LH, LW))), dim3(256), 0, st, x0, col.hi, col.lo, n, LH, LW, 2, NH, NW));
    Epi o; o.S = ll; o.act = 1;
    TRY(F.tgemm(col, M, 160, 0, e->llencg, 64, o));
    ar.release(m);
  } else if (!dry) {
    LAUNCHED((stem_conv_launch<7, 7, 2, 3, 64>(x0, 4, n, kNet, kNet, e->llenc_w, e->llenc_b, nullptr, 1, st, ll)));
  }
  TRY(F.tap_split("ll", ll, (long long)n * LH * LW * 64));

  for (int s = 0; s < 4; ++s) {
    { char nm[32]; snprintf(nm, sizeof nm, "pf:mit.stage%d", s + 1); section(nm); }
    const int C = kMitDims[s], N = RH[s] * RW[s], heads = kMitHeads[s], sr = kMitSr[s];
    const long long rows = (long long)n * N;
    const long long m = ar.mark();
    float* x = ar.f(rows * C);
    float* tf = ar.f(rows * C);
    SplitT t1 = F.salloc(rows, C);
    SplitT t1p;
    if (sr > 1) t1p = F.salloc((long long)n * nkv, sr * sr * C);
    SplitT q = F.salloc(rows, C);
    SplitT a = F.salloc(rows, C);
    float* t2f = ar.f((long long)n * nkv * C);
    SplitT t2 = F.salloc((long long)n * nkv, C);
    SplitT kv = F.salloc((long long)n * nkv, 2 * C);
    const bool qkv_split = e->use_attn_mma && e->use_attn_split;
    float* qf = qkv_split ? nullptr : ar.f(rows * C);
    float* kvf = qkv_split ? nullptr : ar.f((long long)n * nkv * 2 * C);
    float* h1 = ar.f(rows * 4 * C);
    SplitT h2 = F.salloc(rows, 4 * C);
    if (s == 0 && e->use_stem_tc) {
      const long long mm = ar.mark();
      SplitT col = F.salloc(rows, 160);
      if (!dry) LAUNCHED(launch_pdl(stem_gather_kernel, dim3(ew_grid(stem_gather_threads(n, RH[0], RW[0]))), dim3(256), 0, st, x0, col.hi, col.lo, n, RH[0], RW[0], 4, NH, NW));
      Epi o; o.C = tf; o.ldc = C;
      TRY(F.tgemm(col, rows, 160, 0, e->embed1g, 64, o));
      ar.release(mm);
    } else if (s == 0) {
      if (!dry) LAUNCHED((stem_conv_launch<7, 7, 4, 3, 64>(x0, 4, n, kNet, kNet, e->embed1_w, e->embed1_b, tf, 0, st)));
    } else {
      Epi o; o.C = tf; o.ldc = C;
      TRY(F.tconv_gather(cfeat[s - 1], n, RH[s - 1], RW[s - 1], kMitDims[s - 1], 3, 2, 1, e->embed[s], C, o));
    }
    TRY(F.ln(tf, x, rows, C, e->embed_ln[s], 1e-5f));
    TRY(F.tapf(x, rows * C, "mit.s%d.embed", s + 1));
    for (int i = 0; i < kMitDepths[s]; ++i) {
      const MitBlockW& b = e->blocks[s][i];
      if (sr > 1) TRY(F.ln_split_patch(x, t1, t1p, rows, C, b.ln1, 1e-6f, RH[s], RW[s], sr));
      else TRY(F.ln_split(x, t1, rows, C, b.ln1, 1e-6f));
      Epi oq, okv;
      if (qkv_split) { oq.S = q; okv.S = kv; } else { oq.C = qf; oq.ldc = C; okv.C = kvf; okv.ldc = 2 * C; }
      const bool fork = !dry && sr > 1 && e->use_fork && e->side && !e->kp.on && !e->profile && !sync_debug() && !e->debug;
      if (fork) {
        CU(cudaEventRecord(e->ev_fork, st));
        CU(cudaStreamWaitEvent(e->side, e->ev_fork, 0));
        F.st = e->side;
      }
      if (sr > 1) {
        { Epi o; o.C = t2f; o.ldc = C; TRY(F.tgemm(t1p, (long long)n * nkv, sr * sr * C, 0, b.sr, C, o)); }
        TRY(F.ln_split(t2f, t2, (long long)n * nkv, C, b.srln, 1e-5f));
        TRY(F.tgemm(t2, (long long)n * nkv, C, 0, b.kv, 2 * C, okv));
      }
      if (fork) {
        CU(cudaEventRecord(e->ev_join, e->side));
        F.st = st;
      }
      TRY(F.tgemm(t1, rows, C, 0, b.q, C, oq));
      if (fork) CU(cudaStreamWaitEvent(st, e->ev_join, 0));
      if (sr > 1) {
      } else {
        TRY(F.tgemm(t1, rows, C, 0, b.kv, 2 * C, okv));
      }
      if (!dry) {
        if (qkv_split) LAUNCHED(attention_mma_launch(nullptr, nullptr, nullptr, n, N, C, heads, st, a, q, kv, F.np(), nkv));
        else if (e->use_attn_mma) LAUNCHED(attention_mma_launch(qf, kvf, nullptr, n, N, C, heads, st, a, SplitT(), SplitT(), F.np()));
        else LAUNCHED(attention_launch(qf, kvf, nullptr, n, N, C, heads, st, a));
      }
      { Epi o; o.C = x; o.ldc = C; o.res = x; o.ldr = C; TRY(F.tgemm(a, rows, C, 0, b.proj, C, o)); }
      TRY(F.tapf(x, rows * C, "mit.s%d.b%d.attn", s + 1, i));
      TRY(F.ln_split(x, t1, rows, C, b.ln2, 1e-6f));
      { Epi o; o.C = h1; o.ldc = 4 * C; TRY(F.tgemm(t1, rows, C, 0, b.fc1, 4 * C, o)); }
      if (!dry) LAUNCHED(launch_pdl(dwconv3x3_gelu_kernel, dim3(ew_grid((long long)n * ((RH[s] + 1) / 2) * ((RW[s] + PF_DW3_PX - 1) / PF_DW3_PX) * C)), dim3(256), 0, st, h1, nullptr, n, RH[s], RW[s], 4 * C, b.dw_w, b.dw_b, h2.hi, h2.lo));
      { Epi o; o.C = x; o.ldc = C; o.res = x; o.ldr = C; TRY(F.tgemm(h2, rows, 4 * C, 0, b.fc2, C, o)); }
      TRY(F.tapf(x, rows * C, "mit.s%d.b%d", s + 1, i));
    }
    TRY(F.ln_split(x, cfeat[s], rows, C, e->stage_norm[s], 1e-6f));
    { char nm[32]; snprintf(nm, sizeof nm, "mit.c%d", s + 1); TRY(F.tap_split(nm, cfeat[s], rows * C)); }
    ar.release(m);
  }

  float* conv1_out = ar.f((long long)n * NH * NW * 64);
  bool fuse_pred = false;
  {
    const long long m = ar.mark();
    float* fused = nullptr;
    SplitT fused_s;
    for (int lvl = 4; lvl >= 1; --lvl) {
      { char nm[32]; snprintf(nm, sizeof nm, "pf:heads.level%d", lvl); section(nm); }
      const int rh = RH[lvl - 1], rw = RW[lvl - 1], Cin = kMitDims[lvl - 1];
      const long long px = (long long)n * rh * rw;
      float* t = ar.f(px * 512);
      SplitT rt = F.salloc(px, 512);
      SplitT u = F.salloc(px, 512);
      float* v = ar.f(px * 512);
      SplitT rv = F.salloc(px, 512);
      float* w2 = ar.f(px * 512);
      {
        Epi o; o.C = t; o.ldc = 512; o.S = rt; o.split_relu = 1; o.bias_mode = 2;
        TRY(F.thalo(cfeat[lvl - 1], 0, 0, nullptr, 0, 0, n, rh, rw, Cin, e->proc[lvl - 1], 512, 1, 0, o));
        TRY(F.tapf(t, px * 512, "head.proc%d", lvl));
      }
      auto rcu = [&](const SplitT& A, const GemmW& w, Epi o) {
        o.c_gcoff = 256; o.s_gcoff = 256; o.r_gcoff = 256; o.r2_gcoff = 256;
        return F.thalo(A, 0, 256, nullptr, 0, 0, n, rh, rw, 256, w, 256, 2, 256, o);
      };
      const float* of = t;
      const SplitT* os = &rt;
      if (lvl < 4) {
        { Epi o; o.S = u; o.act = 1; TRY(rcu(rt, e->rcu[lvl - 1][0][0], o)); }
        { Epi o; o.C = v; o.ldc = 512; o.S = rv; o.split_relu = 1; o.res = t; o.ldr = 512; o.res_relu = 1; o.res2 = fused; o.ldr2 = 512;
          TRY(rcu(u, e->rcu[lvl - 1][0][1], o)); }
        of = v; os = &rv;
      }
      { Epi o; o.S = u; o.act = 1; TRY(rcu(*os, e->rcu[lvl - 1][1][0], o)); }
      { Epi o; o.C = w2; o.ldc = 512; o.res = of; o.ldr = 512; o.res_relu = 1; TRY(rcu(u, e->rcu[lvl - 1][1][1], o)); }
      if (lvl > 1) {
        float* up = ar.f(px * 4 * 512);
        if (!dry) LAUNCHED(launch_pdl(upsample2x_kernel, dim3(ew_grid(upsample2x_threads(n, rh, rw, 512))), dim3(256), 0, st, w2, 512, 0, up, 512, 0, n, rh, rw, 512, nullptr, nullptr));
        fused = up;
        TRY(F.tapf(up, px * 4 * 512, "head.fusion%d", lvl));
      } else {
        fused_s = F.salloc(px * 4, 512);
        if (!dry) LAUNCHED(launch_pdl(upsample2x_kernel, dim3(ew_grid(upsample2x_threads(n, rh, rw, 512))), dim3(256), 0, st, w2, 512, 0, nullptr, 512, 0, n, rh, rw, 512, fused_s.hi, fused_s.lo));
        TRY(F.tap_split("head.fusion1", fused_s, px * 4 * 512));
      }
    }
    section("pf:heads.fuse_convs");
    fuse_pred = D.gravity_classes == 2 && D.latitude_classes == 1;
    const bool keep_conv1 = !fuse_pred || e->debug;
    PredTail pt[2] = {{e->pred_g_w, e->pred_g_b, dry ? nullptr : bt->pred_gravity, 2, 1}, {e->pred_l_w, e->pred_l_b, dry ? nullptr : bt->pred_latitude, 1, 2}};
    if (e->use_phase) {
      SplitT c0s = F.salloc((long long)n * LH * LW, 128);
      {
        Epi o; o.S = c0s; o.s_gcoff = 64; o.act = 1;
        TRY(F.thalo(fused_s, 0, 256, &ll, 256, 0, n, LH, LW, 320, e->conv0, 64, 2, 64, o));
        TRY(F.tap_split("head.conv0", c0s, (long long)n * LH * LW * 128));
      }
      Epi o; o.ldc = 64; o.c_gcoff = 32; o.act = 1; o.phase4 = 1;
      if (keep_conv1) o.C = conv1_out;
      TRY(F.thalo(c0s, 0, 64, nullptr, 0, 0, n, LH, LW, 64, e->conv1p, 128, 2, 128, o, fuse_pred ? pt : nullptr));
      if (!dry) {
        const dim3 grid((unsigned)cdiv(conv1_ring_count(NH, NW), kRingPx), (unsigned)n);
        LAUNCHED((conv1_ring_kernel<<<grid, 256, kRingSmem, st>>>(c0s.hi, c0s.lo, LH, LW, e->conv1f_w, e->conv1f_b, keep_conv1 ? conv1_out : nullptr,
                                                                 fuse_pred ? e->pred_g_w : nullptr, e->pred_g_b, bt->pred_gravity,
                                                                 fuse_pred ? e->pred_l_w : nullptr, e->pred_l_b, bt->pred_latitude), cudaGetLastError()));
      }
    } else {
      float* c0 = ar.f((long long)n * 160 * 160 * 128);
      {
        Epi o; o.C = c0; o.ldc = 128; o.c_gcoff = 64; o.act = 1;
        TRY(F.thalo(fused_s, 0, 256, &ll, 256, 0, n, 160, 160, 320, e->conv0, 64, 2, 64, o));
        TRY(F.tap("head.conv0", c0, (long long)n * 160 * 160 * 128));
      }
      SplitT c0u = F.salloc((long long)n * kNet * kNet, 128);
      if (!dry) LAUNCHED(launch_pdl(upsample2x_kernel, dim3(ew_grid(upsample2x_threads(n, 160, 160, 128))), dim3(256), 0, st, c0, 128, 0, nullptr, 128, 0, n, 160, 160, 128, c0u.hi, c0u.lo));
      Epi o; o.ldc = 64; o.c_gcoff = 32; o.act = 1;
      if (keep_conv1) o.C = conv1_out;
      TRY(F.thalo(c0u, 0, 64, nullptr, 0, 0, n, kNet, kNet, 64, e->conv1, 32, 2, 32, o, fuse_pred ? pt : nullptr));
    }
    if (keep_conv1) TRY(F.tap("head.conv1", conv1_out, (long long)n * NH * NW * 64));
    ar.release(m);
  }
  section("pf:tails_postprocess");
  TRY(fwd_tails_post(F, bt, conv1_out, d_post, fuse_pred));

  if (D.param_net != PF_PARAM_NONE) {
    section("pf:paramnet");
    if (D.gravity_classes != 2 || D.latitude_classes != 1) return fail(PF_ERR_ARG, "ParamNet needs regression heads");
    const bool centered = D.param_net == PF_PARAM_CENTERED;
    const int SH = centered ? NH : D.param_input_size, SW = centered ? NW : D.param_input_size;
    float* pin = ar.f((long long)n * SH * SW * 4);
    if (!dry) LAUNCHED((pack_fields_kernel<<<(unsigned)cdivl((long long)n * SH * SW, 256), 256, 0, st>>>(bt->pred_gravity, bt->pred_latitude, pin, n, NH, NW, SH, SW), cudaGetLastError()));
    int rh = SH / 4, rw = SW / 4;
    float* x = ar.f((long long)n * rh * rw * 96);
    if (!dry) LAUNCHED((stem_conv_launch<4, 4, 4, 0, 96>(pin, 4, n, SH, SW, e->pn_stem_w, e->pn_stem_b, x, 0, st)));
    TRY(F.ln(x, x, (long long)n * rh * rw, 96, e->pn_stem_ln, 1e-6f));
    for (int s = 0; s < 4; ++s) {
      const int C = kCnxDims[s];
      if (s > 0) {
        const int r2h = rh / 2, r2w = rw / 2;
        SplitT y = F.salloc((long long)n * r2h * r2w, 4 * kCnxDims[s - 1]);
        TRY(F.ln_split_patch(x, SplitT(), y, (long long)n * rh * rw, kCnxDims[s - 1], e->pn_ds_ln[s], 1e-6f, rh, rw, 2));
        float* xn = ar.f((long long)n * r2h * r2w * C);
        Epi o; o.C = xn; o.ldc = C;
        TRY(F.tgemm(y, (long long)n * r2h * r2w, 4 * kCnxDims[s - 1], 0, e->pn_ds[s], C, o));
        x = xn; rh = r2h; rw = r2w;
      }
      const long long rows = (long long)n * rh * rw;
      float* yf = ar.f(rows * C);
      SplitT y = F.salloc(rows, C);
      SplitT h = F.salloc(rows, 4 * C);
      for (int j = 0; j < kCnxDepths[s]; ++j) {
        const CnxBlockW& b = e->pn_blocks[s][j];
        if (e->use_dwln) {
          if (!dry) LAUNCHED(dwconv7x7_ln_launch(x, n, rh, rw, C, b.dw_w, b.dw_b, b.ln.w, b.ln.b, 1e-6f, y, st));
        } else {
          if (!dry) LAUNCHED(launch_pdl(dwconv7x7_kernel, dim3(ew_grid((long long)n * ((rh + 1) / 2) * ((rw + PF_DW7_PX - 1) / PF_DW7_PX) * (C / 4))), dim3(256), 0, st, x, yf, n, rh, rw, C, b.dw_w, b.dw_b));
          TRY(F.ln_split(yf, y, rows, C, b.ln, 1e-6f));
        }
        { Epi o; o.S = h; o.act = 2; TRY(F.tgemm(y, rows, C, 0, b.pw1, 4 * C, o)); }
        { Epi o; o.C = x; o.ldc = C; o.res = x; o.ldr = C; o.gamma = b.gamma; TRY(F.tgemm(h, rows, 4 * C, 0, b.pw2, C, o)); }
      }
      TRY(F.tapf(x, rows * C, "cnx.s%d", s));
    }
    if (!dry) {
      if (!bt->params) return fail(PF_ERR_ARG, "params output is NULL");
      LAUNCHED((param_tail_kernel<<<n, 256, 0, st>>>(x, rh * rw, e->pn_norm.w, e->pn_norm.b, e->pn_head_w, e->pn_head_b, bt->params, D.param_net), cudaGetLastError()));
    }
  }
  return PF_OK;
}

extern "C" {

int pf_abi_version(void) { return PF_ABI_VERSION; }
const char* pf_last_error(void) { return g_err.c_str(); }
int64_t pf_kernel_launch_count(void) { return g_launches.load(); }

static int configure_device(int device) {
  static std::mutex mu;
  static std::vector<char> done;
  std::lock_guard<std::mutex> lock(mu);
  if (device < (int)done.size() && done[device]) return PF_OK;
  CU(gemm_tma_configure_device(3));
  CU(gemm_tma_configure_device(1));
  CU(attention_mma_configure_device());
  CU(cudaFuncSetAttribute(attention_kernel, cudaFuncAttributeMaxDynamicSharedMemorySize, kAttnSmem));
  CU(cudaFuncSetAttribute(conv1_ring_kernel, cudaFuncAttributeMaxDynamicSharedMemorySize, kRingSmem));
  CU(cudaFuncSetAttribute(preprocess_kernel, cudaFuncAttributeMaxDynamicSharedMemorySize, kPreSmemBytes));
  CU(cudaFuncSetAttribute(postprocess_kernel, cudaFuncAttributeMaxDynamicSharedMemorySize, kPostSmemMax));
  if (device >= (int)done.size()) done.resize(device + 1, 0);
  done[device] = 1;
  return PF_OK;
}
static int configure_current_device() {
  int dev = 0;
  CU(cudaGetDevice(&dev));
  return configure_device(dev);
}

static bool net_size_ok(int h, int w) {
  return h >= 64 && w >= 64 && h <= 640 && w <= 640 && h % 32 == 0 && w % 32 == 0 && (h / 32) * (w / 32) <= kAmMaxKeys;
}

int pf_create(int device, const pf_model_desc* desc, pf_handle* out) { return pf_create_sized(device, desc, kNet, kNet, out); }

int pf_create_sized(int device, const pf_model_desc* desc, int net_h, int net_w, pf_handle* out) {
  if (!desc || !out) return fail(PF_ERR_ARG, "pf_create: null argument");
  if (!net_size_ok(net_h, net_w))
    return fail(PF_ERR_ARG, "pf_create: working size %dx%d: height and width must be multiples of 32 in [64, 640] with (H/32)*(W/32) <= %d", net_h, net_w, kAmMaxKeys);
  if (!((desc->gravity_classes == 2 || desc->gravity_classes == 73) && (desc->latitude_classes == 1 || desc->latitude_classes == 180)))
    return fail(PF_ERR_ARG, "pf_create: unsupported head widths %d/%d", desc->gravity_classes, desc->latitude_classes);
  if (desc->param_net < 0 || desc->param_net > 2) return fail(PF_ERR_ARG, "pf_create: bad param_net");
  if (desc->param_net == PF_PARAM_UNCENTERED && (desc->param_input_size < 32 || desc->param_input_size > kNet || desc->param_input_size % 32))
    return fail(PF_ERR_ARG, "pf_create: param_input_size must be a multiple of 32 in [32, 320]");
  int count = 0;
  CU(cudaGetDeviceCount(&count));
  if (device < 0 || device >= count) return fail(PF_ERR_CUDA, "pf_create: no CUDA device %d (found %d)", device, count);
  CU(cudaSetDevice(device));
  cudaDeviceProp prop;
  CU(cudaGetDeviceProperties(&prop, device));
  if (prop.major != 9 || prop.minor != 0) return fail(PF_ERR_CUDA, "pf_create: device %d is sm_%d%d; this library is built for sm_90a only", device, prop.major, prop.minor);
  TRY(configure_device(device));
  pf_engine* e = new pf_engine();
  e->device = device;
  e->sm_count = prop.multiProcessorCount;
  e->desc = *desc;
  e->net_h = net_h;
  e->net_w = net_w;
  if (cudaMalloc(&e->table_dev, kTableSlabBytes) != cudaSuccess || cudaMallocHost(&e->table_host, kTableSlabBytes) != cudaSuccess) {
    const int r = fail(PF_ERR_CUDA, "pf_create: resize-table slab: %s", cudaGetErrorString(cudaGetLastError()));
    cudaFree(e->table_dev);
    delete e;
    return r;
  }
  if (cudaStreamCreateWithFlags(&e->side, cudaStreamNonBlocking) != cudaSuccess || cudaEventCreateWithFlags(&e->ev_fork, cudaEventDisableTiming) != cudaSuccess ||
      cudaEventCreateWithFlags(&e->ev_join, cudaEventDisableTiming) != cudaSuccess) {
    const int r = fail(PF_ERR_CUDA, "pf_create: side stream / events: %s", cudaGetErrorString(cudaGetLastError()));
    pf_destroy(e);
    return r;
  }
  *out = e;
  return PF_OK;
}

int pf_destroy(pf_handle h) {
  if (!h) return PF_OK;
  cudaSetDevice(h->device);
  if (h->side) { cudaStreamSynchronize(h->side); cudaStreamDestroy(h->side); }
  if (h->ev_fork) cudaEventDestroy(h->ev_fork);
  if (h->ev_join) cudaEventDestroy(h->ev_join);
  cudaFree(h->table_dev);
  cudaFreeHost(h->table_host);
  for (auto& r : h->prof) { cudaEventDestroy(r.a); cudaEventDestroy(r.b); }
  for (auto ev : h->ev_pool) cudaEventDestroy(ev);
  for (auto ev : h->kp.pool) cudaEventDestroy(ev);
  delete h;
  return PF_OK;
}

int pf_set_weight(pf_handle h, const char* name, const void* dev_ptr, int64_t numel, int dtype) {
  if (!h || !name || !dev_ptr) return fail(PF_ERR_ARG, "pf_set_weight: null argument");
  if (((uintptr_t)dev_ptr & 15) != 0) return fail(PF_ERR_ARG, "pf_set_weight: '%s' is not 16-byte aligned", name);
  h->weights[name] = WeightRef{dev_ptr, numel, dtype};
  h->finalized = false;
  return PF_OK;
}

int pf_finalize(pf_handle h) {
  if (!h) return fail(PF_ERR_ARG, "pf_finalize: null handle");
  TRY(resolve_weights(h));
  h->finalized = true;
  return PF_OK;
}

int64_t pf_workspace_bytes(pf_handle h, int n, int max_h) {
  if (!h || n < 1) return fail(PF_ERR_ARG, "pf_workspace_bytes: bad argument");
  Fwd F{h, Arena{}, nullptr, true, n};
  F.ar.dry = true;
  F.ar.keep = h->debug;
  (void)max_h;
  int r = run_forward_tma(F, nullptr);
  if (r != PF_OK) return r;
  return F.ar.peak + 4096;
}

int pf_forward(pf_handle h, const pf_batch* bt, void* workspace, int64_t workspace_bytes, void* stream) {
  if (!h || !bt || !workspace) return fail(PF_ERR_ARG, "pf_forward: null argument");
  if (!h->finalized) return fail(PF_ERR_WEIGHT, "pf_forward: pf_finalize has not succeeded");
  if (bt->n < 1) return fail(PF_ERR_ARG, "pf_forward: empty batch");
  if ((bt->images_u8 != nullptr) == (bt->images_chw != nullptr)) return fail(PF_ERR_ARG, "pf_forward: exactly one of images_u8 / images_chw");
  if (bt->images_u8 && !bt->image_offset) return fail(PF_ERR_ARG, "pf_forward: image_offset is NULL");
  if (!bt->height || !bt->width || !bt->pred_gravity || !bt->pred_latitude || !bt->gravity_original || !bt->latitude_original ||
      !bt->gravity_original_offset || !bt->latitude_original_offset)
    return fail(PF_ERR_ARG, "pf_forward: null input/output pointer");
  CU(cudaSetDevice(h->device));
  Fwd F{h, Arena{}, (cudaStream_t)stream, false, bt->n};
  F.ar.base = (char*)workspace;
  F.ar.cap = workspace_bytes;
  F.ar.keep = h->debug;
  {
    Fwd T{h, Arena{}, nullptr, true, bt->n};
    T.ar.dry = true; T.ar.keep = h->debug;
    TRY(run_forward_tma(T, nullptr));
    if (T.ar.peak > workspace_bytes) return fail(PF_ERR_WORKSPACE, "pf_forward: workspace %lld B < required %lld B", (long long)workspace_bytes, T.ar.peak);
  }
  if (((uintptr_t)workspace & 255) != 0) return fail(PF_ERR_ARG, "pf_forward: workspace must be 256-byte aligned");
  h->taps.clear();
  h->kp.st = (cudaStream_t)stream;
  tl_kp = &h->kp;
  pdl_enabled() = h->use_pdl && !h->kp.on && !h->profile && !sync_debug();
  const int r = run_forward_tma(F, bt);
  pdl_enabled() = false;
  tl_kp = nullptr;
  return r;
}

int pf_profile_enable(pf_handle h, int on) {
  if (!h) return fail(PF_ERR_ARG, "null handle");
  h->profile = on != 0;
  while (on > 1 && (long long)h->ev_pool.size() < 2LL * on) {
    cudaEvent_t ev;
    CU(cudaEventCreate(&ev));
    h->ev_pool.push_back(ev);
  }
  return PF_OK;
}
int pf_profile_kernels_enable(pf_handle h, int max_launches) {
  if (!h) return fail(PF_ERR_ARG, "null handle");
  CU(cudaSetDevice(h->device));
  KernelProf& kp = h->kp;
  kp.on = max_launches > 0;
  kp.used = 0;
  kp.recs.clear();
  while ((long long)kp.pool.size() < 2LL * max_launches) {
    cudaEvent_t ev;
    CU(cudaEventCreate(&ev));
    kp.pool.push_back(ev);
  }
  return PF_OK;
}
int pf_profile_kernels_read(pf_handle h, char* buf, int cap) {
  if (!h || !buf || cap < 1) return fail(PF_ERR_ARG, "pf_profile_kernels_read: bad argument");
  std::map<std::string, std::pair<int, double>> agg;
  std::vector<std::string> order;
  for (const auto& r : h->kp.recs) {
    float ms = 0.f;
    CU(cudaEventElapsedTime(&ms, r.a, r.b));
    const char* c = r.expr;
    while (*c == '(' || *c == ' ') ++c;
    const char* e = c;
    while (*e && (isalnum((unsigned char)*e) || *e == '_')) ++e;
    std::string name(c, e);
    if (name == "launch_pdl" && *e == '(') {
      c = e + 1;
      e = c;
      while (*e && (isalnum((unsigned char)*e) || *e == '_')) ++e;
      name.assign(c, e);
    }
    if (*e == '<' && e[1] != '<') { const char* t = strchr(e, '>'); if (t) name.append(e, t + 1); }
    auto it = agg.find(name);
    if (it == agg.end()) { order.push_back(name); it = agg.emplace(name, std::make_pair(0, 0.0)).first; }
    it->second.first += 1;
    it->second.second += ms;
  }
  std::string out = "kernel,launches,ms\n";
  for (const auto& n : order) {
    char line[256];
    snprintf(line, sizeof line, "%s,%d,%.4f\n", n.c_str(), agg[n].first, agg[n].second);
    out += line;
  }
  if ((int)out.size() + 1 > cap) return fail(PF_ERR_ARG, "pf_profile_kernels_read: buffer too small (%d needed)", (int)out.size() + 1);
  memcpy(buf, out.c_str(), out.size() + 1);
  h->kp.used = 0;
  h->kp.recs.clear();
  return (int)out.size();
}
int pf_set_option(pf_handle h, const char* name, int value) {
  if (!h || !name) return fail(PF_ERR_ARG, "pf_set_option: null argument");
  if (!strcmp(name, "attn_mma")) { h->use_attn_mma = value != 0; return PF_OK; }
  if (!strcmp(name, "stem_tc")) { h->use_stem_tc = value != 0; return PF_OK; }
  if (!strcmp(name, "phase_conv1")) { h->use_phase = value != 0; return PF_OK; }
  if (!strcmp(name, "attn_split")) { h->use_attn_split = value != 0; return PF_OK; }
  if (!strcmp(name, "decode_only")) { h->decode_only = value != 0; return PF_OK; }
  if (!strcmp(name, "pdl")) { h->use_pdl = value != 0; return PF_OK; }
  if (!strcmp(name, "dw_ln")) { h->use_dwln = value != 0; return PF_OK; }
  if (!strcmp(name, "fork")) { h->use_fork = value != 0; return PF_OK; }
  if (!strcmp(name, "bf16")) { h->bf16 = value != 0; return PF_OK; }
  return fail(PF_ERR_ARG, "pf_set_option: unknown option '%s'", name);
}
int pf_profile_read(pf_handle h, double* out9) {
  if (!h || !out9) return fail(PF_ERR_ARG, "pf_profile_read: null argument");
  for (int i = 0; i < 21; ++i) out9[i] = 0.0;
  FILE* csv = nullptr;
  if (const char* path = getenv("PF_PROFILE_CSV")) {
    csv = fopen(path, "w");
    if (csv) fprintf(csv, "engine_cfg,M,N,K,Cin,KH,stride,groups,ms,algorithmic_tflops\n");
  }
  for (auto& r : h->prof) {
    float ms = 0.f;
    CU(cudaEventSynchronize(r.b));
    CU(cudaEventElapsedTime(&ms, r.a, r.b));
    if (csv) fprintf(csv, "%d,%d,%d,%d,%d,%d,%d,%d,%.4f,%.1f\n", r.cfg, r.M, r.N, r.K, r.Cin, r.KH, r.stride, r.groups, ms, r.flops / (ms * 1e9));
    out9[r.cfg * 3 + 0] += ms;
    out9[r.cfg * 3 + 1] += r.flops;
    out9[r.cfg * 3 + 2] += 1.0;
    h->ev_pool.push_back(r.a);
    h->ev_pool.push_back(r.b);
  }
  if (csv) fclose(csv);
  h->prof.clear();
  return PF_OK;
}

int pf_debug_enable(pf_handle h, int on) {
  if (!h) return fail(PF_ERR_ARG, "null handle");
  h->debug = on != 0;
  h->taps.clear();
  return PF_OK;
}
int pf_debug_count(pf_handle h) { return h ? (int)h->taps.size() : 0; }
const char* pf_debug_name(pf_handle h, int i) { return (h && i >= 0 && i < (int)h->taps.size()) ? h->taps[i].first.c_str() : ""; }
int64_t pf_debug_numel(pf_handle h, const char* name) {
  if (!h || !name) return -1;
  for (auto& t : h->taps) if (t.first == name) return t.second.second;
  return -1;
}
int pf_debug_copy(pf_handle h, const char* name, float* dst, int64_t numel, void* stream) {
  if (!h || !name || !dst) return fail(PF_ERR_ARG, "pf_debug_copy: null argument");
  for (auto& t : h->taps)
    if (t.first == name) {
      if (numel != t.second.second) return fail(PF_ERR_ARG, "pf_debug_copy: '%s' has %lld elements", name, t.second.second);
      CU(cudaMemcpyAsync(dst, t.second.first, numel * 4, cudaMemcpyDeviceToDevice, (cudaStream_t)stream));
      return PF_OK;
    }
  return fail(PF_ERR_ARG, "pf_debug_copy: no tap '%s'", name);
}

#define NCCL_TRY(expr)                                                                                              \
  do {                                                                                                              \
    int r__ = (expr);                                                                                               \
    if (r__ != kNcclSuccess) return fail(PF_ERR_CUDA, "%s: %s", #expr, api.GetErrorString ? api.GetErrorString(r__) : "NCCL error"); \
  } while (0)
int pf_comm_unique_id(void* id128) {
  if (!id128) return fail(PF_ERR_ARG, "pf_comm_unique_id: null argument");
  const NcclApi& api = nccl_api();
  if (api.error) return fail(PF_ERR_CUDA, "%s", api.error);
  static_assert(sizeof(NcclUniqueId) == 128, "ncclUniqueId is 128 bytes");
  NCCL_TRY(api.GetUniqueId((NcclUniqueId*)id128));
  return PF_OK;
}
int pf_comm_create(int device, int rank, int nranks, const void* id128, pf_comm_handle* out) {
  if (!id128 || !out || nranks < 1 || rank < 0 || rank >= nranks) return fail(PF_ERR_ARG, "pf_comm_create: bad argument");
  const NcclApi& api = nccl_api();
  if (api.error) return fail(PF_ERR_CUDA, "%s", api.error);
  CU(cudaSetDevice(device));
  NcclUniqueId id;
  memcpy(&id, id128, sizeof id);
  pf_comm* c = new pf_comm();
  c->device = device; c->rank = rank; c->nranks = nranks;
  const int r = api.CommInitRank(&c->comm, nranks, id, rank);
  if (r != kNcclSuccess) { delete c; return fail(PF_ERR_CUDA, "ncclCommInitRank: %s", api.GetErrorString(r)); }
  *out = c;
  return PF_OK;
}
int pf_comm_destroy(pf_comm_handle c) {
  if (!c) return PF_OK;
  const NcclApi& api = nccl_api();
  cudaSetDevice(c->device);
  if (c->comm && api.CommDestroy) api.CommDestroy(c->comm);
  delete c;
  return PF_OK;
}
int pf_gather(pf_comm_handle c, int root, int count, void* const* dev_ptrs, const int64_t* bytes, const int32_t* peer, void* stream) {
  if (!c || count < 0 || root < 0 || root >= c->nranks || (count > 0 && (!dev_ptrs || !bytes))) return fail(PF_ERR_ARG, "pf_gather: bad argument");
  if (c->rank == root && count > 0 && !peer) return fail(PF_ERR_ARG, "pf_gather: the root needs the source rank of every segment");
  const NcclApi& api = nccl_api();
  CU(cudaSetDevice(c->device));
  if (count == 0) return PF_OK;
  NCCL_TRY(api.GroupStart());
  for (int i = 0; i < count; ++i) {
    int r;
    if (c->rank == root) {
      if (peer[i] < 0 || peer[i] >= c->nranks || peer[i] == root) { api.GroupEnd(); return fail(PF_ERR_ARG, "pf_gather: segment %d comes from rank %d", i, peer[i]); }
      r = api.Recv(dev_ptrs[i], (size_t)bytes[i], kNcclUint8, peer[i], c->comm, (cudaStream_t)stream);
    } else {
      r = api.Send(dev_ptrs[i], (size_t)bytes[i], kNcclUint8, root, c->comm, (cudaStream_t)stream);
    }
    if (r != kNcclSuccess) { api.GroupEnd(); return fail(PF_ERR_CUDA, "ncclSend/Recv: %s", api.GetErrorString(r)); }
  }
  NCCL_TRY(api.GroupEnd());
  return PF_OK;
}

int pf_jpeg_create(int device, int max_threads, pf_jpeg_handle* out) {
  if (!out) return fail(PF_ERR_ARG, "pf_jpeg_create: null argument");
  const NvjpegApi& api = nvjpeg_api();
  if (api.error) return fail(PF_ERR_CUDA, "%s", api.error);
  CU(cudaSetDevice(device));
  pf_jpeg* j = new pf_jpeg();
  j->device = device;
  if (api.CreateSimple(&j->handle) != NVJPEG_STATUS_SUCCESS) { delete j; return fail(PF_ERR_CUDA, "nvjpegCreateSimple failed"); }
  int nt = max_threads > 0 ? max_threads : (int)std::thread::hardware_concurrency() / 2;
  nt = nt < 1 ? 1 : (nt > 32 ? 32 : nt);
  j->workers.resize(nt);
  bool ok = cudaEventCreateWithFlags(&j->start, cudaEventDisableTiming) == cudaSuccess;
  for (auto& w : j->workers) {
    ok = ok && api.StateCreate(j->handle, &w.state) == NVJPEG_STATUS_SUCCESS;
    ok = ok && cudaStreamCreateWithFlags(&w.stream, cudaStreamNonBlocking) == cudaSuccess;
    ok = ok && cudaEventCreateWithFlags(&w.done, cudaEventDisableTiming) == cudaSuccess;
  }
  if (!ok) { pf_jpeg_destroy(j); return fail(PF_ERR_CUDA, "pf_jpeg_create: decoder state / stream creation failed"); }
  *out = j;
  return PF_OK;
}
int pf_jpeg_destroy(pf_jpeg_handle j) {
  if (!j) return PF_OK;
  const NvjpegApi& api = nvjpeg_api();
  cudaSetDevice(j->device);
  for (auto& w : j->workers) {
    if (w.stream) cudaStreamSynchronize(w.stream);
    if (w.state) api.StateDestroy(w.state);
    if (w.stream) cudaStreamDestroy(w.stream);
    if (w.done) cudaEventDestroy(w.done);
  }
  if (j->start) cudaEventDestroy(j->start);
  if (j->handle) api.Destroy(j->handle);
  delete j;
  return PF_OK;
}
int pf_jpeg_info(pf_jpeg_handle j, const uint8_t* data, int64_t length, int32_t* height, int32_t* width) {
  if (!j || !data || length < 4 || !height || !width) return fail(PF_ERR_ARG, "pf_jpeg_info: bad argument");
  const NvjpegApi& api = nvjpeg_api();
  int nc = 0, ws[NVJPEG_MAX_COMPONENT] = {0}, hs[NVJPEG_MAX_COMPONENT] = {0};
  nvjpegChromaSubsampling_t ss;
  if (api.GetImageInfo(j->handle, data, (size_t)length, &nc, &ss, ws, hs) != NVJPEG_STATUS_SUCCESS) return fail(PF_ERR_ARG, "pf_jpeg_info: not a decodable JPEG stream");
  *height = hs[0]; *width = ws[0];
  return PF_OK;
}
int pf_jpeg_decode_batch(pf_jpeg_handle j, int n, const uint8_t* const* data, const int64_t* length, const int32_t* height, const int32_t* width,
                         uint8_t* blob, const int64_t* offset, void* stream) {
  if (!j || n < 1 || !data || !length || !height || !width || !blob || !offset) return fail(PF_ERR_ARG, "pf_jpeg_decode_batch: bad argument");
  const NvjpegApi& api = nvjpeg_api();
  CU(cudaSetDevice(j->device));
  cudaStream_t st = (cudaStream_t)stream;
  CU(cudaEventRecord(j->start, st));
  const int nt = (int)j->workers.size() < n ? (int)j->workers.size() : n;
  std::atomic<int> next{0}, failed{-1};
  auto work = [&](int t) {
    cudaSetDevice(j->device);
    pf_jpeg::Worker& w = j->workers[t];
    cudaStreamWaitEvent(w.stream, j->start, 0);
    for (int i = next.fetch_add(1); i < n; i = next.fetch_add(1)) {
      nvjpegImage_t dst{};
      dst.channel[0] = blob + offset[i];
      dst.pitch[0] = (size_t)width[i] * 3;
      if (api.Decode(j->handle, w.state, data[i], (size_t)length[i], NVJPEG_OUTPUT_BGRI, &dst, w.stream) != NVJPEG_STATUS_SUCCESS) failed.store(i);
    }
    cudaEventRecord(w.done, w.stream);
  };
  std::vector<std::thread> threads;
  for (int t = 1; t < nt; ++t) threads.emplace_back(work, t);
  work(0);
  for (auto& th : threads) th.join();
  for (int t = 0; t < nt; ++t) CU(cudaStreamWaitEvent(st, j->workers[t].done, 0));
  if (failed.load() >= 0) return fail(PF_ERR_ARG, "pf_jpeg_decode_batch: image %d could not be decoded", failed.load());
  return PF_OK;
}

int pf_op_conv_gemm(const float* x, int B, int H, int W, int Cin, const void* whi, const void* wlo, const float* bias, int N, int KH, int KW,
                    int stride, int pad, int in_relu, int act, const float* res, int res_relu, float* y, void* stream) {
  if (!x || !whi || !wlo || !y) return fail(PF_ERR_ARG, "pf_op_conv_gemm: null argument");
  if (KH != KW) return fail(PF_ERR_ARG, "pf_op_conv_gemm: square filters only");
  TRY(configure_current_device());
  cudaStream_t st = (cudaStream_t)stream;
  int dev = 0;
  CU(cudaGetDevice(&dev));
  cudaDeviceProp prop;
  CU(cudaGetDeviceProperties(&prop, dev));
  pf_engine tmp;
  tmp.device = dev;
  tmp.sm_count = prop.multiProcessorCount;
  const int OH = (H + 2 * pad - KH) / stride + 1, OW = (W + 2 * pad - KW) / stride + 1;
  const long long nx = (long long)B * H * W * Cin;
  const long long colb = (long long)B * OH * OW * KH * KW * Cin * 4 + (1 << 20);
  char* scratch = nullptr;
  CU(cudaMalloc(&scratch, nx * 4 + colb + 4096));
  Fwd F{&tmp, Arena{}, st, false, B};
  F.ar.base = scratch; F.ar.cap = nx * 4 + colb + 4096;
  SplitT A = F.salloc((long long)B * H * W, Cin);
  int r = PF_OK;
  {
    cudaError_t le = (split_kernel<<<(unsigned)cdivl(nx, 256), 256, 0, st>>>(x, A.hi, A.lo, nx, in_relu), cudaGetLastError());
    g_launches.fetch_add(1, std::memory_order_relaxed);
    if (le != cudaSuccess) r = fail(PF_ERR_CUDA, "split_kernel: %s", cudaGetErrorString(le));
  }
  GemmW w{(const __nv_bfloat16*)whi, (const __nv_bfloat16*)wlo, bias};
  Fwd::Epi o;
  o.C = y; o.ldc = N; o.act = act; o.res = res; o.ldr = N; o.res_relu = res_relu;
  if (r == PF_OK) {
    if (KH == 3 && stride == 1 && pad == 1 && Cin % 64 == 0) r = F.thalo(A, 0, 0, nullptr, 0, 0, B, H, W, Cin, w, N, 1, 0, o);
    else if (KH == 1 && stride == 1 && pad == 0) r = F.tgemm(A, (long long)B * H * W, Cin, 0, w, N, o);
    else r = F.tconv_gather(A, B, H, W, Cin, KH, stride, pad, w, N, o);
  }
  cudaError_t se = cudaStreamSynchronize(st);
  cudaFree(scratch);
  if (r != PF_OK) return r;
  if (se != cudaSuccess) return fail(PF_ERR_CUDA, "pf_op_conv_gemm: %s", cudaGetErrorString(se));
  return PF_OK;
}
static int op_tma(pf_tma_op* op, void* stream, bool bf16) {
  if (!op || !op->a_hi || !op->a_lo || !op->w_hi || !op->w_lo) return fail(PF_ERR_ARG, "pf_op_tma: null argument");
  const pf_tma_op& q = *op;
  if (q.mode != MODE_GEMM && q.mode != MODE_HALO) return fail(PF_ERR_ARG, "pf_op_tma: mode %d", q.mode);
  if (!q.C && !q.s_hi) return fail(PF_ERR_ARG, "pf_op_tma: no output (C and S are both NULL)");
  if (!q.s_hi != !q.s_lo || !q.a2_hi != !q.a2_lo) return fail(PF_ERR_ARG, "pf_op_tma: a split pair needs both planes");
  if (q.bias_mode < 0 || q.bias_mode > 2 || q.act < 0 || q.act > 2) return fail(PF_ERR_ARG, "pf_op_tma: bias_mode %d / act %d", q.bias_mode, q.act);
  if (q.groups < 1 || q.groups > 2 || q.N < 1) return fail(PF_ERR_ARG, "pf_op_tma: groups %d, N %d", q.groups, q.N);
  if (q.npred != 0 && q.npred != q.groups) return fail(PF_ERR_ARG, "pf_op_tma: npred must be 0 or groups");
  if (q.mode == MODE_GEMM && (q.groups != 1 || q.a2_hi || q.phase4 || q.npred || q.M < 1 || q.M > INT32_MAX))
    return fail(PF_ERR_ARG, "pf_op_tma: GEMM mode runs one group of 1..2^31-1 rows without A2, phase4 or prediction tail");
  if (q.mode == MODE_HALO && (q.B < 1 || q.H < 1 || q.W < 1)) return fail(PF_ERR_ARG, "pf_op_tma: image size %dx%dx%d", q.B, q.H, q.W);
  TRY(configure_current_device());
  int dev = 0;
  CU(cudaGetDevice(&dev));
  cudaDeviceProp prop;
  CU(cudaGetDeviceProperties(&prop, dev));
  pf_engine tmp;
  tmp.device = dev;
  tmp.sm_count = prop.multiProcessorCount;
  tmp.bf16 = bf16;
  Fwd F{&tmp, Arena{}, (cudaStream_t)stream, false, q.B};
  if (q.force_sched < 0 || q.force_sched > 2 || (q.force_sched && q.mode != MODE_GEMM)) return fail(PF_ERR_ARG, "pf_op_tma: force_sched %d", q.force_sched);
  F.force_bn = q.force_bn; F.force_kb = q.force_kb; F.force_sched = q.force_sched;
  const SplitT A{(__nv_bfloat16*)q.a_hi, (__nv_bfloat16*)q.a_lo, q.lda};
  const SplitT A2{(__nv_bfloat16*)q.a2_hi, (__nv_bfloat16*)q.a2_lo, q.lda2};
  const GemmW w{(const __nv_bfloat16*)q.w_hi, (const __nv_bfloat16*)q.w_lo, q.bias};
  Fwd::Epi o;
  o.C = q.C; o.ldc = q.ldc; o.c_coff = q.c_coff; o.c_gcoff = q.c_gcoff;
  o.S = SplitT{(__nv_bfloat16*)q.s_hi, (__nv_bfloat16*)q.s_lo, q.lds}; o.s_coff = q.s_coff; o.s_gcoff = q.s_gcoff; o.split_relu = q.split_relu;
  o.act = q.act; o.gamma = q.gamma;
  o.res = q.res; o.ldr = q.ldr; o.r_coff = q.r_coff; o.r_gcoff = q.r_gcoff; o.res_relu = q.res_relu;
  o.res2 = q.res2; o.ldr2 = q.ldr2; o.r2_coff = q.r2_coff; o.r2_gcoff = q.r2_gcoff;
  o.bias_mode = q.bias_mode; o.phase4 = q.phase4;
  PredTail pt[2];
  for (int g = 0; g < q.npred; ++g) {
    const pf_tma_pred& s = q.pred[g];
    if (!s.w || !s.b || !s.out || !(s.mode == 1 ? s.nc == 2 : (s.mode == 2 && s.nc == 1))) return fail(PF_ERR_ARG, "pf_op_tma: prediction tail %d", g);
    pt[g] = PredTail{s.w, s.b, s.out, s.nc, s.mode};
  }
  op->picked_bn = op->picked_kb = op->picked_sched = 0;
  const int r = q.mode == MODE_GEMM ? F.tgemm(A, q.M, q.K, q.a_c0, w, q.N, o)
                                    : F.thalo(A, q.a_c0, q.a_gc, q.a2_hi ? &A2 : nullptr, q.c_split, q.a2_c0, q.B, q.H, q.W, q.Cin, w, q.N, q.groups,
                                              q.bias_gstride, o, q.npred ? pt : nullptr);
  if (r == PF_OK) { op->picked_bn = F.picked_bn; op->picked_kb = F.picked_kb; op->picked_sched = F.picked_sched; }
  return r;
}
int pf_op_tma(pf_tma_op* op, void* stream) { return op_tma(op, stream, false); }
int pf_op_tma_bf16(pf_tma_op* op, void* stream) { return op_tma(op, stream, true); }
int pf_op_conv1_ring(const void* c_hi, const void* c_lo, int B, int H, int W, const float* wf, const float* bias, float* out,
                     const float* pg_w, const float* pg_b, float* pg_out, const float* pl_w, const float* pl_b, float* pl_out, void* stream) {
  if (!c_hi || !c_lo || !wf || !bias) return fail(PF_ERR_ARG, "pf_op_conv1_ring: null argument");
  const bool tail = pg_w || pg_b || pg_out || pl_w || pl_b || pl_out;
  if (tail && !(pg_w && pg_b && pg_out && pl_w && pl_b && pl_out)) return fail(PF_ERR_ARG, "pf_op_conv1_ring: the prediction tail needs all six pointers");
  if (!out && !tail) return fail(PF_ERR_ARG, "pf_op_conv1_ring: no output");
  if (B < 1 || H < 2 || W < 2) return fail(PF_ERR_ARG, "pf_op_conv1_ring: needs B >= 1 and H, W >= 2 (got %dx%dx%d)", B, H, W);
  TRY(configure_current_device());
  const dim3 grid((unsigned)cdiv(conv1_ring_count(2 * H, 2 * W), kRingPx), (unsigned)B);
  LAUNCHED((conv1_ring_kernel<<<grid, 256, kRingSmem, (cudaStream_t)stream>>>((const __nv_bfloat16*)c_hi, (const __nv_bfloat16*)c_lo, H, W, wf, bias, out,
                                                                             pg_w, pg_b, pg_out, pl_w, pl_b, pl_out), cudaGetLastError()));
  return PF_OK;
}
int pf_tma_pick_tile(int mode, int64_t M, int N, int K, int sm_count, int* bn, int* kb) {
  if (!bn || !kb || (mode != MODE_GEMM && mode != MODE_HALO) || N < 1 || K < 1 || sm_count < 1) return fail(PF_ERR_ARG, "pf_tma_pick_tile: bad argument");
  tma_pick_tile(mode, M, N, K, sm_count, *bn, *kb);
  return PF_OK;
}
int pf_camera_fields(int device, const pf_camera* cams, int n, float* up, float* lat, void* stream) {
  return pf_camera_fields_vp(device, cams, nullptr, n, up, lat, stream);
}
int pf_camera_fields_vp(int device, const pf_camera* cams, const double* vp, int n, float* up, float* lat, void* stream) {
  if (!cams || n < 1 || (!up && !lat)) return fail(PF_ERR_ARG, "pf_camera_fields: bad argument");
  if (vp) {
    for (int i = 0; i < n; ++i)
      if (std::isfinite(vp[2 * i]) != std::isfinite(vp[2 * i + 1]))
        return fail(PF_ERR_ARG, "pf_camera_fields_vp: image %d: a vanishing point needs two finite coordinates (or two NaN)", i);
  }
  CU(cudaSetDevice(device));
  for (int i0 = 0; i0 < n; i0 += kCamChunk) {
    const int m = n - i0 < kCamChunk ? n - i0 : kCamChunk;
    CamBatch b{};
    long long max_q = 1;
    for (int i = 0; i < m; ++i) {
      const pf_camera& c = cams[i0 + i];
      if (c.height < 1 || c.width < 1 || !(c.focal_rel != 0.0)) return fail(PF_ERR_ARG, "pf_camera_fields: image %d: size %dx%d, focal %g", i0 + i, c.height, c.width, c.focal_rel);
      if ((c.up_offset & 1) != 0) return fail(PF_ERR_ARG, "pf_camera_fields: up_offset must be even (8-byte stores)");
      CamImage& o = b.im[i];
      o.H = c.height; o.W = c.width;
      o.f = c.focal_rel * c.height;
      o.cx = (c.cx_rel + 0.5) * c.width; o.cy = (c.cy_rel + 0.5) * c.height;
      o.sr = sin(c.roll); o.cr = cos(c.roll); o.se = sin(c.elevation); o.ce = cos(c.elevation);
      o.sgn = c.elevation > 0 ? 1.0 : (c.elevation < 0 ? -1.0 : 0.0);
      o.vp = vp && std::isfinite(vp[2 * (i0 + i)]);
      if (o.vp) { o.vpx = vp[2 * (i0 + i)]; o.vpy = vp[2 * (i0 + i) + 1]; o.sgn = 1.0; }
      o.up_off = c.up_offset; o.lat_off = c.lat_offset;
      const long long qd = (long long)c.height * ((c.width + 3) / 4);
      if (qd > max_q) max_q = qd;
    }
    const dim3 grid((unsigned)cdivl(max_q, 256), (unsigned)m);
    LAUNCHED((camera_fields_kernel<<<grid, 256, 0, (cudaStream_t)stream>>>(b, up, lat), cudaGetLastError()));
  }
  return PF_OK;
}

int pf_pano_views(int device, const uint8_t* pano, int pano_h, int pano_w, const pf_pano_view* views, int n, uint8_t* im, float* ntheta,
                  float* nphi, float* up, float* lat, float* xy, double* offset, int32_t* status, void* stream) {
  if (!pano || !views || n < 1) return fail(PF_ERR_ARG, "pf_pano_views: null panorama / views or n < 1");
  if (pano_h < 2 || pano_w < 2) return fail(PF_ERR_ARG, "pf_pano_views: panorama of %dx%d (needs at least 2x2)", pano_h, pano_w);
  if (!im && !ntheta && !nphi && !up && !lat && !xy && !offset && !status) return fail(PF_ERR_ARG, "pf_pano_views: no output");
  for (int i = 0; i < n; ++i) {
    const pf_pano_view& c = views[i];
    if (c.height < 1 || c.width < 1) return fail(PF_ERR_ARG, "pf_pano_views: view %d has size %dx%d", i, c.height, c.width);
    if (!std::isfinite(c.f) || !(c.f > 0.0) || !std::isfinite(c.xi) || !std::isfinite(c.az) || !std::isfinite(c.el) || !std::isfinite(c.roll))
      return fail(PF_ERR_ARG, "pf_pano_views: view %d: f must be finite and > 0, xi and the angles finite (f %g, xi %g)", i, c.f, c.xi);
    if (c.im_offset < 0 || c.field_offset < 0) return fail(PF_ERR_ARG, "pf_pano_views: view %d has a negative offset", i);
  }
  CU(cudaSetDevice(device));
  PanoMap m{};
  m.Hp = pano_h; m.Wp = pano_w;
  m.ax = (M_PI - -M_PI) / ((pano_w - 1.0) - 0);
  m.bx = M_PI - m.ax * (pano_w - 1.0);
  m.iax = 1.0 / m.ax;
  m.ay = (-M_PI / 2.0 - M_PI / 2.0) / ((pano_h - 1.0) - 0);
  m.by = M_PI / 2.0 - m.ay * 0;
  m.iay = 1.0 / m.ay;
  auto rad = [](double deg) { return deg * M_PI / 180; };
  for (int i0 = 0; i0 < n; i0 += kPanoChunk) {
    const int cnt = n - i0 < kPanoChunk ? n - i0 : kPanoChunk;
    PanoBatch b{};
    long long max_px = 1;
    for (int i = 0; i < cnt; ++i) {
      const pf_pano_view& c = views[i0 + i];
      PanoView& o = b.v[i];
      o.H = c.height; o.W = c.width;
      o.f = c.f; o.xi = c.xi; o.one_m_xi2 = 1 - c.xi * c.xi;
      o.u0 = c.width / 2.0; o.v0 = c.height / 2.0;
      const double ce = cos(rad(c.el)), se = sin(rad(c.el)), ca = cos(rad(c.az)), sa = sin(rad(c.az)), cr = cos(rad(c.roll)), sr = sin(rad(c.roll));
      const double rel[9] = {1.0, 0.0, 0.0, 0.0, ce, -se, 0.0, se, ce};
      const double raz[9] = {ca, 0.0, sa, 0.0, 1.0, 0.0, -sa, 0.0, ca};
      const double rroll[9] = {cr, -sr, 0.0, sr, cr, 0.0, 0.0, 0.0, 1.0};
      memcpy(o.rel, rel, sizeof rel); memcpy(o.raz, raz, sizeof raz); memcpy(o.rroll, rroll, sizeof rroll);
      const double fmin = sqrt(-(1 - c.xi * c.xi) * ((1 - o.u0) * (1 - o.u0) + (1 - o.v0) * (1 - o.v0))) * 1.0001;
      o.masked = c.f < fmin;
      const double r = sqrt(-(c.f * c.f) / (1 - c.xi * c.xi));
      o.r2 = r * r;
      o.ci0 = nearbyint(c.height / 2.0); o.ci1 = nearbyint(c.width / 2.0);
      o.im_off = c.im_offset; o.fld_off = c.field_offset;
      const long long px = (long long)c.height * c.width;
      if (px > max_px) max_px = px;
    }
    const dim3 grid((unsigned)cdivl(max_px, (long long)kPanoThreads * kPanoPix) + 1, (unsigned)cnt);
    LAUNCHED((pano_views_kernel<<<grid, kPanoThreads, 0, (cudaStream_t)stream>>>(b, m, pano, im, ntheta, nphi, up, lat, xy, offset, status, i0),
              cudaGetLastError()));
  }
  return PF_OK;
}

int pf_equi_views(int device, const void* pano, int pano_h, int pano_w, int channels, int dtype, const pf_equi_view* views, int n, int mode,
                  int out_kind, int swap_rb, void* im, void* stream) {
  if (!pano || !views || !im || n < 1) return fail(PF_ERR_ARG, "pf_equi_views: null panorama / views / im or n < 1");
  if (pano_h < 1 || pano_w < 1) return fail(PF_ERR_ARG, "pf_equi_views: panorama of %dx%d", pano_h, pano_w);
  if (channels != 1 && channels != 3) return fail(PF_ERR_ARG, "pf_equi_views: %d channels (1 or 3)", channels);
  if (dtype != PF_EQUI_U8 && dtype != PF_EQUI_F32) return fail(PF_ERR_ARG, "pf_equi_views: unknown dtype %d", dtype);
  if (mode != PF_EQUI_BILINEAR && mode != PF_EQUI_NEAREST) return fail(PF_ERR_ARG, "pf_equi_views: unknown mode %d", mode);
  if (out_kind != PF_EQUI_CAST && out_kind != PF_EQUI_UNIT) return fail(PF_ERR_ARG, "pf_equi_views: unknown out_kind %d", out_kind);
  if (out_kind == PF_EQUI_UNIT && dtype != PF_EQUI_U8) return fail(PF_ERR_ARG, "pf_equi_views: the unit path needs a uint8 panorama");
  if (swap_rb != 0 && (swap_rb != 1 || channels != 3)) return fail(PF_ERR_ARG, "pf_equi_views: swap_rb must be 0, or 1 with 3 channels");
  const int esize = dtype == PF_EQUI_F32 ? 4 : 1;
  std::vector<double> fov_x(n);
  for (int i = 0; i < n; ++i) {
    const pf_equi_view& c = views[i];
    if (c.height < 1 || c.width < 1) return fail(PF_ERR_ARG, "pf_equi_views: view %d has size %dx%d", i, c.height, c.width);
    if (!std::isfinite(c.azimuth) || !std::isfinite(c.elevation) || !std::isfinite(c.roll))
      return fail(PF_ERR_ARG, "pf_equi_views: view %d: non-finite angle", i);
    if (!std::isfinite(c.vfov) || !(c.vfov > 0.0 && c.vfov < 180.0) || !std::isfinite(c.ar) || !(c.ar > 0.0))
      return fail(PF_ERR_ARG, "pf_equi_views: view %d: vfov %g must lie in (0, 180) and ar %g be finite and > 0", i, c.vfov, c.ar);
    fov_x[i] = 2 * atan(tan(c.vfov * M_PI / 180.0 / 2) * c.ar) * 180 / M_PI;
    if (!(fov_x[i] > 0.0 && fov_x[i] < 180.0)) return fail(PF_ERR_ARG, "pf_equi_views: view %d: fov_x %g must lie in (0, 180)", i, fov_x[i]);
    if (c.offset < 0 || c.offset % esize != 0) return fail(PF_ERR_ARG, "pf_equi_views: view %d: offset %lld (>= 0, a multiple of %d)", i,
                                                          (long long)c.offset, esize);
  }
  CU(cudaSetDevice(device));
  EquiMap m{};
  m.Hp = pano_h; m.Wp = pano_w; m.C = channels;
  m.nearest = mode == PF_EQUI_NEAREST; m.swap_rb = swap_rb;
  m.su = pano_w / (2 * M_PI); m.sv = pano_h / M_PI;
  for (int i0 = 0; i0 < n; i0 += kEquiChunk) {
    const int cnt = n - i0 < kEquiChunk ? n - i0 : kEquiChunk;
    EquiBatch b{};
    long long max_px = 1;
    for (int i = 0; i < cnt; ++i) {
      const pf_equi_view& c = views[i0 + i];
      EquiView& o = b.v[i];
      o.H = c.height; o.W = c.width;
      o.f = c.width / (2 * tan(fov_x[i0 + i] * M_PI / 180 / 2));
      o.u0 = c.width / 2.0; o.v0 = c.height / 2.0;
      const double roll = c.roll / 180 * M_PI, el = c.elevation / 180 * M_PI, az = c.azimuth / 180 * M_PI;
      o.cr = cos(roll); o.sr = sin(roll); o.ce = cos(el); o.se = sin(el); o.ca = cos(az); o.sa = sin(az);
      o.off = c.offset;
      const long long px = (long long)c.height * c.width;
      if (px > max_px) max_px = px;
    }
    const dim3 grid((unsigned)cdivl(max_px, (long long)kEquiThreads * kEquiPix), (unsigned)cnt);
    cudaStream_t st = (cudaStream_t)stream;
    unsigned char* out = (unsigned char*)im;
    if (dtype == PF_EQUI_F32)
      LAUNCHED((equi_views_kernel<float, false><<<grid, kEquiThreads, 0, st>>>(b, m, (const float*)pano, out), cudaGetLastError()));
    else if (out_kind == PF_EQUI_UNIT)
      LAUNCHED((equi_views_kernel<unsigned char, true><<<grid, kEquiThreads, 0, st>>>(b, m, (const unsigned char*)pano, out), cudaGetLastError()));
    else
      LAUNCHED((equi_views_kernel<unsigned char, false><<<grid, kEquiThreads, 0, st>>>(b, m, (const unsigned char*)pano, out), cudaGetLastError()));
  }
  return PF_OK;
}

static DrawStyle draw_style() {
  static const double anchors[5][3] = {{0.0, 0.0, 0.3}, {0.0, 0.0, 1.0}, {1.0, 1.0, 1.0}, {1.0, 0.0, 0.0}, {0.5, 0.0, 0.0}};
  auto seismic = [&](double t, int ch) {
    const int e = std::min((int)std::floor(256.0 * t), 255);
    const double x = e / 255.0;
    const int s = std::min((int)(x * 4.0), 3);
    const double dist = (x - s / 4.0) / 0.25;
    return 255.0 * (dist * (anchors[s + 1][ch] - anchors[s][ch]) + anchors[s][ch]);
  };
  DrawStyle st{};
  const int nb = kDrawLevels - 1;
  for (int k = 0; k < kDrawLevels; ++k) {
    st.lev[k] = (float)(k == nb ? M_PI / 2 : -M_PI / 2 + k * (M_PI / nb));
    for (int ch = 0; ch < 3; ++ch) {
      st.line[k][ch] = (float)seismic((double)k / nb, ch);
      if (k < nb) st.band[k][ch] = (float)seismic((k + 0.5) / nb, ch);
    }
  }
  return st;
}

int pf_draw_fields(int device, const pf_draw_canvas* cs, int n, const uint8_t* img, uint8_t* out, const float* lat, const float* up, void* stream) {
  if (!cs || n < 1 || !img || !out) return fail(PF_ERR_ARG, "pf_draw_fields: null canvases / img / out or n < 1");
  auto unit = [](float x) { return std::isfinite(x) && x >= 0.f && x <= 1.f; };
  for (int i = 0; i < n; ++i) {
    const pf_draw_canvas& c = cs[i];
    if (c.height < 1 || c.width < 1 || (long long)c.height * c.width >= (1LL << 31))
      return fail(PF_ERR_ARG, "pf_draw_fields: canvas %d has size %dx%d", i, c.height, c.width);
    if (c.img_offset < 0 || c.out_offset < 0) return fail(PF_ERR_ARG, "pf_draw_fields: canvas %d has a negative image offset", i);
    if (!unit(c.alpha_fill) || !unit(c.alpha_line)) return fail(PF_ERR_ARG, "pf_draw_fields: canvas %d: alphas must lie in [0, 1]", i);
    if (c.draw_lat && (!lat || c.lat_offset < 0)) return fail(PF_ERR_ARG, "pf_draw_fields: canvas %d draws the latitude without a latitude map", i);
    if (c.draw_up) {
      if (!up || c.up_offset < 0 || c.up_stride[0] < 0 || c.up_stride[1] < 0 || c.up_stride[2] < 0)
        return fail(PF_ERR_ARG, "pf_draw_fields: canvas %d draws arrows without an up field, or with a negative offset / stride", i);
      if (c.density < 1 || c.arrow_inv_len < 1 || c.width / c.density < 1 || c.height / c.density < 1)
        return fail(PF_ERR_ARG, "pf_draw_fields: canvas %d (%dx%d): density %d and arrow_inv_len %d must be >= 1 and leave W // density, "
                    "H // density >= 1", i, c.height, c.width, c.density, c.arrow_inv_len);
      if (!unit(c.arrow_rgb[0]) || !unit(c.arrow_rgb[1]) || !unit(c.arrow_rgb[2])) return fail(PF_ERR_ARG, "pf_draw_fields: canvas %d: arrow colour outside [0, 1]", i);
    }
  }
  CU(cudaSetDevice(device));
  const DrawStyle st = draw_style();
  for (int i0 = 0; i0 < n; i0 += kDrawChunk) {
    const int cnt = n - i0 < kDrawChunk ? n - i0 : kDrawChunk;
    DrawBatch b{};
    long long max_tiles = 1;
    for (int i = 0; i < cnt; ++i) {
      const pf_draw_canvas& c = cs[i0 + i];
      DrawCanvas& o = b.c[i];
      o.H = c.height; o.W = c.width;
      o.tiles_x = cdiv(c.width, kDrawTW);
      o.draw_lat = c.draw_lat != 0; o.draw_up = c.draw_up != 0;
      o.alpha_fill = c.alpha_fill; o.alpha_line = c.alpha_line;
      o.img_off = c.img_offset; o.out_off = c.out_offset; o.lat_off = c.lat_offset; o.up_off = c.up_offset;
      o.us_row = c.up_stride[0]; o.us_col = c.up_stride[1]; o.us_comp = c.up_stride[2];
      if (o.draw_up) {
        o.sx = c.width / c.density; o.sy = c.height / c.density;
        o.nx = cdiv(c.width, o.sx); o.ny = cdiv(c.height, o.sy);
        const double diag = std::sqrt((double)c.width * c.width + (double)c.height * c.height), q = c.arrow_inv_len;
        const double mod = std::fmod(diag, q), div = (diag - mod) / q;
        double fl = std::floor(div);
        if (div - fl > 0.5) fl += 1.0;
        o.len = (float)fl;
        const double sq = std::sqrt((double)o.nx * o.ny);
        o.w = (float)(0.06 * c.width / std::min(std::max(sq, 8.0), 25.0));
        for (int ch = 0; ch < 3; ++ch) o.rgb[ch] = 255.f * c.arrow_rgb[ch];
      }
      const long long tiles = (long long)o.tiles_x * cdiv(c.height, kDrawTH);
      if (tiles > max_tiles) max_tiles = tiles;
    }
    const dim3 grid((unsigned)max_tiles, (unsigned)cnt);
    LAUNCHED((draw_fields_kernel<<<grid, kDrawThreads, 0, (cudaStream_t)stream>>>(b, st, img, out, lat, up), cudaGetLastError()));
  }
  return PF_OK;
}

static int upload_table(const ResampleTable& t, int** bounds, int** coeffs) {
  CU(cudaMalloc(bounds, t.bounds.size() * 4));
  CU(cudaMalloc(coeffs, t.coeffs.size() * 4));
  CU(cudaMemcpy(*bounds, t.bounds.data(), t.bounds.size() * 4, cudaMemcpyHostToDevice));
  CU(cudaMemcpy(*coeffs, t.coeffs.data(), t.coeffs.size() * 4, cudaMemcpyHostToDevice));
  return PF_OK;
}
int pf_op_resize_u8(const uint8_t* img, int H, int W, int new_h, int new_w, uint8_t* out, void* stream) {
  if (!img || !out || H < 1 || W < 1 || new_h < 1 || new_w < 1) return fail(PF_ERR_ARG, "pf_op_resize_u8: bad argument");
  cudaStream_t st = (cudaStream_t)stream;
  if (H == new_h && W == new_w) {
    CU(cudaMemcpyAsync(out, img, (size_t)H * W * 3, cudaMemcpyDeviceToDevice, st));
    return PF_OK;
  }
  ResampleTable tx = make_resample_table(W, new_w), ty = make_resample_table(H, new_h);
  int *bx = nullptr, *cx = nullptr, *by = nullptr, *cy = nullptr;
  unsigned char* tmp = nullptr;
  int r = upload_table(tx, &bx, &cx);
  if (r == PF_OK) r = upload_table(ty, &by, &cy);
  if (r == PF_OK && cudaMalloc(&tmp, (size_t)H * new_w * 3) != cudaSuccess) r = fail(PF_ERR_CUDA, "pf_op_resize_u8: cudaMalloc");
  if (r == PF_OK) {
    cudaError_t le = (resize_u8_h_kernel<<<(unsigned)cdivl((long long)H * new_w, 256), 256, 0, st>>>(img, H, W, new_w, bx, cx, tx.ksize, tmp), cudaGetLastError());
    if (le == cudaSuccess) le = (resize_u8_v_kernel<<<(unsigned)cdivl((long long)new_h * new_w, 256), 256, 0, st>>>(tmp, H, new_w, new_h, by, cy, ty.ksize, out), cudaGetLastError());
    g_launches.fetch_add(2, std::memory_order_relaxed);
    if (le == cudaSuccess) le = cudaStreamSynchronize(st);
    if (le != cudaSuccess) r = fail(PF_ERR_CUDA, "pf_op_resize_u8: %s", cudaGetErrorString(le));
  }
  cudaFree(bx); cudaFree(cx); cudaFree(by); cudaFree(cy); cudaFree(tmp);
  return r;
}
int pf_op_resize_f32(const float* img, int H, int W, int C, int new_h, int new_w, float* out, void* stream) {
  if (!img || !out || H < 1 || W < 1 || C < 1 || new_h < 1 || new_w < 1) return fail(PF_ERR_ARG, "pf_op_resize_f32: bad argument");
  LAUNCHED((resize_f32_kernel<<<(unsigned)cdivl((long long)new_h * new_w * C, 256), 256, 0, (cudaStream_t)stream>>>(img, H, W, C, new_h, new_w, out), cudaGetLastError()));
  return PF_OK;
}
int pf_op_argmax_decode(const float* logits, float* field, int B, int HW, int NC, int is_gravity, void* stream) {
  if (!logits || !field || B < 1 || HW < 1 || NC < 1) return fail(PF_ERR_ARG, "pf_op_argmax_decode: bad argument");
  LAUNCHED((argmax_decode_kernel<<<(unsigned)cdivl((long long)B * HW, 256), 256, 0, (cudaStream_t)stream>>>(logits, field, B, HW, NC, is_gravity), cudaGetLastError()));
  return PF_OK;
}
int pf_op_pred_argmax_decode(const float* feat, int ld, int coff, const float* w, const float* bias, float* field, int B, int HW, int NC, int is_gravity,
                             void* stream) {
  if (!feat || !w || !bias || !field || B < 1 || HW < 1 || NC < 1 || NC > 256 || (ld & 3) || (coff & 3)) return fail(PF_ERR_ARG, "pf_op_pred_argmax_decode: bad argument");
  LAUNCHED((pred_argmax_decode_kernel<<<ew_grid((long long)B * HW * 4), 256, NC * 37 * 4, (cudaStream_t)stream>>>(feat, ld, coff, w, bias, field, B, HW, NC, is_gravity),
            cudaGetLastError()));
  return PF_OK;
}
int pf_op_postprocess(const float* vec, const float* lat, int n, const int32_t* height, const int32_t* width, float* gravity_original,
                      const int64_t* gravity_original_offset, float* latitude_original, const int64_t* latitude_original_offset, int lat_is_sin,
                      void* stream) {
  if (!vec || !lat || n < 1 || !height || !width || !gravity_original || !gravity_original_offset || !latitude_original || !latitude_original_offset)
    return fail(PF_ERR_ARG, "pf_op_postprocess: bad argument");
  return pf_op_postprocess_sized(vec, lat, n, kNet, kNet, height, width, gravity_original, gravity_original_offset, latitude_original, latitude_original_offset,
                                 lat_is_sin, stream);
}
int pf_op_postprocess_sized(const float* vec, const float* lat, int n, int net_h, int net_w, const int32_t* height, const int32_t* width, float* gravity_original,
                            const int64_t* gravity_original_offset, float* latitude_original, const int64_t* latitude_original_offset, int lat_is_sin,
                            void* stream) {
  if (!vec || !lat || n < 1 || !height || !width || !gravity_original || !gravity_original_offset || !latitude_original || !latitude_original_offset)
    return fail(PF_ERR_ARG, "pf_op_postprocess: bad argument");
  if (!net_size_ok(net_h, net_w)) return fail(PF_ERR_ARG, "pf_op_postprocess: unsupported working size %dx%d", net_h, net_w);
  TRY(configure_current_device());
  PostImage* d_post = nullptr;
  CU(cudaMalloc(&d_post, n * sizeof(PostImage)));
  int r = launch_postprocess(vec, lat, n, net_h, net_w, height, width, gravity_original_offset, latitude_original_offset, gravity_original, latitude_original,
                             lat_is_sin, d_post, (cudaStream_t)stream);
  cudaError_t se = cudaStreamSynchronize((cudaStream_t)stream);
  cudaFree(d_post);
  if (r == PF_OK && se != cudaSuccess) r = fail(PF_ERR_CUDA, "pf_op_postprocess: %s", cudaGetErrorString(se));
  return r;
}

int pf_op_fill_stream(float* dst, int64_t numel, float value, void* stream) {
  if (!dst || numel < 4 || (numel & 3) || ((uintptr_t)dst & 15)) return fail(PF_ERR_ARG, "pf_op_fill_stream: bad argument");
  LAUNCHED((fill_stream_kernel<<<132 * 16, 256, 0, (cudaStream_t)stream>>>(reinterpret_cast<float4*>(dst), numel / 4, value), cudaGetLastError()));
  return PF_OK;
}
int pf_op_layernorm(const float* x, float* y, int64_t rows, int C, const float* w, const float* b, float eps, void* stream) {
  LAUNCHED(layernorm_launch(x, y, rows, C, w, b, eps, (cudaStream_t)stream));
  return PF_OK;
}
int pf_op_attention(const float* q, const float* kv, float* out, int B, int N, int C, int heads, void* stream) {
  TRY(configure_current_device());
  if (C != heads * kAttnD) return fail(PF_ERR_ARG, "pf_op_attention: head_dim must be 64");
  LAUNCHED(attention_launch(q, kv, out, B, N, C, heads, (cudaStream_t)stream));
  return PF_OK;
}
int pf_op_attention_mma(const float* q, const float* kv, float* out, int B, int N, int C, int heads, void* stream) {
  TRY(configure_current_device());
  if (C != heads * kAmD) return fail(PF_ERR_ARG, "pf_op_attention_mma: head_dim must be 64");
  LAUNCHED(attention_mma_launch(q, kv, out, B, N, C, heads, (cudaStream_t)stream));
  return PF_OK;
}
static int op_attention_tc(const float* q, const float* kv, float* out, int B, int N, int C, int heads, void* stream, int np, int nkv = kAmKeys) {
  if (!q || !kv || !out || C != heads * kAmD) return fail(PF_ERR_ARG, "pf_op_attention_tc: head_dim must be 64");
  if (B < 1 || N < 1 || nkv < 1 || nkv > kAmMaxKeys) return fail(PF_ERR_ARG, "pf_op_attention_tc: B %d, N %d, %d keys (1..%d)", B, N, nkv, kAmMaxKeys);
  TRY(configure_current_device());
  cudaStream_t st = (cudaStream_t)stream;
  int dev = 0;
  CU(cudaGetDevice(&dev));
  cudaDeviceProp prop;
  CU(cudaGetDeviceProperties(&prop, dev));
  pf_engine tmp;
  tmp.device = dev;
  tmp.sm_count = prop.multiProcessorCount;
  const long long nq = (long long)B * N * C, nkve = (long long)B * nkv * 2 * C;
  char* scratch = nullptr;
  CU(cudaMalloc(&scratch, (2 * nq + nkve) * 4 + 8192));
  Fwd F{&tmp, Arena{}, st, false, B};
  F.ar.base = scratch; F.ar.cap = (2 * nq + nkve) * 4 + 8192;
  SplitT qs = F.salloc((long long)B * N, C), kvs = F.salloc((long long)B * nkv, 2 * C), as = F.salloc((long long)B * N, C);
  int r = PF_OK;
  cudaError_t le = (split_kernel<<<(unsigned)cdivl(nq, 256), 256, 0, st>>>(q, qs.hi, qs.lo, nq, 0), cudaGetLastError());
  if (le == cudaSuccess) le = (split_kernel<<<(unsigned)cdivl(nkve, 256), 256, 0, st>>>(kv, kvs.hi, kvs.lo, nkve, 0), cudaGetLastError());
  if (le != cudaSuccess) r = fail(PF_ERR_CUDA, "split_kernel: %s", cudaGetErrorString(le));
  if (r == PF_OK) {
    le = attention_mma_launch(nullptr, nullptr, nullptr, B, N, C, heads, st, as, qs, kvs, np, nkv);
    if (le != cudaSuccess) r = fail(PF_ERR_CUDA, "attention_mma_launch: %s", cudaGetErrorString(le));
  }
  if (r == PF_OK) {
    le = (merge_split_kernel<<<(unsigned)cdivl(nq, 256), 256, 0, st>>>(as.hi, as.lo, out, nq), cudaGetLastError());
    if (le != cudaSuccess) r = fail(PF_ERR_CUDA, "merge_split_kernel: %s", cudaGetErrorString(le));
  }
  cudaError_t se = cudaStreamSynchronize(st);
  cudaFree(scratch);
  if (r == PF_OK && se != cudaSuccess) r = fail(PF_ERR_CUDA, "pf_op_attention_tc: %s", cudaGetErrorString(se));
  return r;
}
int pf_op_attention_tc(const float* q, const float* kv, float* out, int B, int N, int C, int heads, void* stream) {
  return op_attention_tc(q, kv, out, B, N, C, heads, stream, 3);
}
int pf_op_attention_tc_bf16(const float* q, const float* kv, float* out, int B, int N, int C, int heads, void* stream) {
  return op_attention_tc(q, kv, out, B, N, C, heads, stream, 1);
}
int pf_op_attention_tc_keys(const float* q, const float* kv, float* out, int B, int N, int NKV, int C, int heads, int bf16, void* stream) {
  return op_attention_tc(q, kv, out, B, N, C, heads, stream, bf16 ? 1 : 3, NKV);
}
int pf_op_dwconv3x3_gelu(const float* x, float* y, int B, int H, int W, int C, const float* w, const float* bias, void* stream) {
  if (C % 4) return fail(PF_ERR_ARG, "C %% 4");
  LAUNCHED(launch_pdl(dwconv3x3_gelu_kernel, dim3(ew_grid((long long)B * ((H + 1) / 2) * ((W + PF_DW3_PX - 1) / PF_DW3_PX) * (C / 4))), dim3(256), 0, (cudaStream_t)stream, x, y, B, H, W, C, w, bias, nullptr, nullptr));
  return PF_OK;
}
int pf_op_dwconv7x7(const float* x, float* y, int B, int H, int W, int C, const float* w, const float* bias, void* stream) {
  if (C % 4) return fail(PF_ERR_ARG, "C %% 4");
  LAUNCHED(launch_pdl(dwconv7x7_kernel, dim3(ew_grid((long long)B * ((H + 1) / 2) * ((W + PF_DW7_PX - 1) / PF_DW7_PX) * (C / 4))), dim3(256), 0, (cudaStream_t)stream, x, y, B, H, W, C, w, bias));
  return PF_OK;
}
int pf_op_upsample2x(const float* x, float* y, int B, int H, int W, int C, void* stream) {
  if (C % 4) return fail(PF_ERR_ARG, "C %% 4");
  LAUNCHED(launch_pdl(upsample2x_kernel, dim3(ew_grid(upsample2x_threads(B, H, W, C))), dim3(256), 0, (cudaStream_t)stream, x, C, 0, y, C, 0, B, H, W, C, nullptr, nullptr));
  return PF_OK;
}
int pf_op_preprocess(const uint8_t* img, int H, int W, const float* mean3, const float* std3, float* y, void* stream) {
  return pf_op_preprocess_sized(img, H, W, kNet, kNet, mean3, std3, y, stream);
}
int pf_op_preprocess_sized(const uint8_t* img, int H, int W, int net_h, int net_w, const float* mean3, const float* std3, float* y, void* stream) {
  if (!img || !mean3 || !std3 || !y || H < 1 || W < 1) return fail(PF_ERR_ARG, "pf_op_preprocess: bad argument");
  if (!net_size_ok(net_h, net_w)) return fail(PF_ERR_ARG, "pf_op_preprocess: unsupported working size %dx%d", net_h, net_w);
  TRY(configure_current_device());
  ResampleTable tx = make_resample_table(W, net_w), ty = make_resample_table(H, net_h);
  const int max_rows = pre_max_smem_rows(net_w);
  if (ty.ksize + 1 > max_rows) return fail(PF_ERR_ARG, "image too tall");
  int *bx, *cx, *by, *cy;
  PreImage* d;
  CU(cudaMalloc(&bx, tx.bounds.size() * 4)); CU(cudaMalloc(&cx, tx.coeffs.size() * 4));
  CU(cudaMalloc(&by, ty.bounds.size() * 4)); CU(cudaMalloc(&cy, ty.coeffs.size() * 4));
  CU(cudaMalloc(&d, sizeof(PreImage)));
  CU(cudaMemcpy(bx, tx.bounds.data(), tx.bounds.size() * 4, cudaMemcpyHostToDevice));
  CU(cudaMemcpy(cx, tx.coeffs.data(), tx.coeffs.size() * 4, cudaMemcpyHostToDevice));
  CU(cudaMemcpy(by, ty.bounds.data(), ty.bounds.size() * 4, cudaMemcpyHostToDevice));
  CU(cudaMemcpy(cy, ty.coeffs.data(), ty.coeffs.size() * 4, cudaMemcpyHostToDevice));
  PreImage pi{0, H, W, tx.ksize, ty.ksize, bx, cx, by, cy};
  CU(cudaMemcpy(d, &pi, sizeof pi, cudaMemcpyHostToDevice));
  int rows = pre_rows_needed(H, net_h);
  if (rows > max_rows) rows = max_rows;
  const int smem = rows * net_w * 3;
  LAUNCHED((preprocess_kernel<<<dim3(net_h / kPreRows, 1), net_w, smem, (cudaStream_t)stream>>>(img, d, y, mean3[0], mean3[1], mean3[2], std3[0], std3[1], std3[2], rows,
                                                                                                 net_h, net_w),
            cudaGetLastError()));
  CU(cudaStreamSynchronize((cudaStream_t)stream));
  cudaFree(bx); cudaFree(cx); cudaFree(by); cudaFree(cy); cudaFree(d);
  return PF_OK;
}

}
```

perspectivefields_b200/csrc/tma_host.cuh:

```cuda
#pragma once
#include <cuda.h>
#include <cuda_runtime.h>

#include <cstdlib>
#include <string>

#include "gemm_tma.cuh"

namespace pf {

typedef CUresult (*PFN_tensorMapEncodeTiled)(CUtensorMap*, CUtensorMapDataType, cuuint32_t, void*, const cuuint64_t*, const cuuint64_t*,
                                             const cuuint32_t*, const cuuint32_t*, CUtensorMapInterleave, CUtensorMapSwizzle,
                                             CUtensorMapL2promotion, CUtensorMapFloatOOBfill);

inline PFN_tensorMapEncodeTiled tma_encoder() {
  static PFN_tensorMapEncodeTiled fn = nullptr;
  if (!fn) {
    void* p = nullptr;
    cudaDriverEntryPointQueryResult q;
    if (cudaGetDriverEntryPoint("cuTensorMapEncodeTiled", &p, cudaEnableDefault, &q) == cudaSuccess && q == cudaDriverEntryPointSuccess)
      fn = (PFN_tensorMapEncodeTiled)p;
  }
  return fn;
}

inline const char* tma_map_2d(CUtensorMap* m, const void* base, long long cols, long long rows, long long ld, int box_rows, int kb) {
  PFN_tensorMapEncodeTiled enc = tma_encoder();
  if (!enc) return "cuTensorMapEncodeTiled entry point not available";
  cuuint64_t dims[2] = {(cuuint64_t)cols, (cuuint64_t)rows};
  cuuint64_t strides[1] = {(cuuint64_t)ld * 2};
  cuuint32_t box[2] = {(cuuint32_t)kb, (cuuint32_t)box_rows};
  cuuint32_t es[2] = {1, 1};
  if (((uintptr_t)base & 15) || (strides[0] & 15) || box_rows < 1 || box_rows > 256) return "tma_map_2d: alignment / box";
  CUresult r = enc(m, CU_TENSOR_MAP_DATA_TYPE_BFLOAT16, 2, const_cast<void*>(base), dims, strides, box, es, CU_TENSOR_MAP_INTERLEAVE_NONE,
                   kb == 32 ? CU_TENSOR_MAP_SWIZZLE_64B : CU_TENSOR_MAP_SWIZZLE_128B, CU_TENSOR_MAP_L2_PROMOTION_L2_128B,
                   CU_TENSOR_MAP_FLOAT_OOB_FILL_NONE);
  return r == CUDA_SUCCESS ? nullptr : "cuTensorMapEncodeTiled (2d) failed";
}

inline const char* tma_map_halo(CUtensorMap* m, const void* base, int B, int H, int W, int ld) {
  PFN_tensorMapEncodeTiled enc = tma_encoder();
  if (!enc) return "cuTensorMapEncodeTiled entry point not available";
  cuuint64_t dims[4] = {(cuuint64_t)ld, (cuuint64_t)W, (cuuint64_t)H, (cuuint64_t)B};
  cuuint64_t strides[3] = {(cuuint64_t)ld * 2, (cuuint64_t)W * ld * 2, (cuuint64_t)H * W * ld * 2};
  cuuint32_t box[4] = {64, (cuuint32_t)kHtHaloW, (cuuint32_t)kHtHaloH, 1};
  cuuint32_t es[4] = {1, 1, 1, 1};
  if (((uintptr_t)base & 15) || (strides[0] & 15)) return "tma_map_halo: alignment";
  CUresult r = enc(m, CU_TENSOR_MAP_DATA_TYPE_BFLOAT16, 4, const_cast<void*>(base), dims, strides, box, es, CU_TENSOR_MAP_INTERLEAVE_NONE,
                   CU_TENSOR_MAP_SWIZZLE_128B, CU_TENSOR_MAP_L2_PROMOTION_L2_128B, CU_TENSOR_MAP_FLOAT_OOB_FILL_NONE);
  return r == CUDA_SUCCESS ? nullptr : "cuTensorMapEncodeTiled (halo) failed";
}

inline int tma_pick_bn(int N, int mode) {
  const int tiles = cdiv(N, 256);
  int bn = cdiv(cdiv(N, tiles), 32) * 32;
  if (mode == MODE_HALO) bn = bn <= 32 ? 32 : (bn <= 64 ? 64 : (bn <= 128 ? 128 : 256));
  return bn;
}

inline int tma_pick_bn_gemm(long long M, int N, int K, int sm_count) {
  const int base = tma_pick_bn(N, MODE_GEMM);
  const long long mt = cdivl(M, 128);
  if (mt * cdiv(N, base) * 4 > 3LL * sm_count) return base;
  int best = base;
  double best_cost = 1e30;
  for (int bn = base; bn >= 32; bn -= 32) {
    const long long tiles = mt * cdiv(N, bn);
    const double waves = (double)cdivl(tiles, sm_count);
    const double mma = 3.0 * bn, load = 1.6 * (128 + bn);
    const double cost = waves * ((K / 16) * (mma > load ? mma : load) + 3000.0);
    if (cost < best_cost - 1e-9) { best_cost = cost; best = bn; }
  }
  return best;
}

inline int tma_pick_kb(int bn, int K, int mode) {
  const int lim = mode == MODE_HALO ? 128 : 64;
  return (bn <= lim && K % 64 == 0) ? 64 : 32;
}

inline void tma_pick_tile(int mode, long long M, int N, int K, int sm_count, int& bn, int& kb) {
  bn = mode == MODE_GEMM ? tma_pick_bn_gemm(M, N, K, sm_count) : tma_pick_bn(N, mode);
  kb = tma_pick_kb(bn, K, mode);
}

constexpr int kPingPongKMax = 512;
inline bool tma_pick_pingpong(long long M, int N, int K, int bn, int sm_count) {
  return K <= kPingPongKMax && cdivl(M, 64) * cdiv(N, bn) >= 2LL * sm_count;
}

struct PredTail { const float* w; const float* b; float* out; int nc, mode; };

template <int BN, int MODE, int KB, bool PP = false, int NP = 3>
inline cudaError_t gemm_tma_launch_bn(const TmaMaps& maps, const TmaGemmParams& p, int sm_count, cudaStream_t st, const PredTail* pred) {
  using Cfg = TmaCfg<BN, MODE, KB, PP, NP>;
  const int tiles_x = MODE == MODE_HALO ? cdiv(p.W, kHtTileW) : 0, tiles_y = MODE == MODE_HALO ? cdiv(p.H, kHtTileH) : 0;
  const long long m_tiles = MODE == MODE_GEMM ? cdiv(p.M, Cfg::kTileM) : (long long)p.B * tiles_x * tiles_y;
  const long long total = m_tiles * cdiv(p.N, BN) * p.groups;
  const unsigned grid = (unsigned)(total < sm_count ? total : sm_count);
  if (MODE == MODE_HALO && ((p.Cin == 64 && 9 * (64 / KB) <= Cfg::kStages && (p.groups > 1 || cdiv(p.N, BN) > 1)) || pred)) {
    cudaError_t last = cudaSuccess;
    for (int g = 0; g < p.groups; ++g)
      for (int nt = 0; nt < cdiv(p.N, BN); ++nt) {
        TmaGemmParams q = p;
        q.groups = 1;
        q.a_c0 = p.a_c0 + g * p.a_gc;
        q.bias = p.bias ? p.bias + (long long)g * p.bias_gstride : nullptr;
        q.c_coff = p.c_coff + g * p.c_gcoff; q.s_coff = p.s_coff + g * p.s_gcoff;
        q.r_coff = p.r_coff + g * p.r_gcoff; q.r2_coff = p.r2_coff + g * p.r2_gcoff;
        q.b_row0 = g * p.N;
        if (pred) { q.pred_w = pred[g].w; q.pred_b = pred[g].b; q.pred_out = pred[g].out; q.pred_nc = pred[g].nc; q.pred_mode = pred[g].mode; }
        if (cdiv(p.N, BN) > 1) return cudaErrorInvalidValue;
        const unsigned gr = (unsigned)(m_tiles < sm_count ? m_tiles : sm_count);
        last = launch_pdl(gemm_tma_kernel<BN, MODE, KB, false, NP>, dim3(gr), dim3(kTmaThreads), Cfg::kSmemBytes, st, maps, q, tiles_x, tiles_y);
        if (last != cudaSuccess) return last;
      }
    return last;
  }
  return launch_pdl(gemm_tma_kernel<BN, MODE, KB, PP, NP>, dim3(grid), dim3(kTmaThreads), Cfg::kSmemBytes, st, maps, p, tiles_x, tiles_y);
}

#define PF_TMA_VARIANTS(X)                                                                                                  \
  X(256, MODE_GEMM, 32) X(224, MODE_GEMM, 32) X(192, MODE_GEMM, 32) X(160, MODE_GEMM, 32) X(128, MODE_GEMM, 32) X(96, MODE_GEMM, 32) \
  X(64, MODE_GEMM, 32) X(32, MODE_GEMM, 32) X(64, MODE_GEMM, 64) X(32, MODE_GEMM, 64)                                        \
  X(256, MODE_HALO, 32) X(128, MODE_HALO, 64) X(64, MODE_HALO, 64) X(32, MODE_HALO, 64)
#define PF_TMA_PINGPONG_VARIANTS(X)                                                                                         \
  X(256, 32) X(224, 32) X(192, 32) X(160, 32) X(128, 32) X(96, 32) X(64, 32) X(32, 32) X(64, 64) X(32, 64)

template <int NP>
inline cudaError_t gemm_tma_configure_np() {
  cudaError_t e = cudaSuccess;
#define PF_TMA_CFG(BN_, MODE_, KB_)                                                                                          \
  if (e == cudaSuccess) e = cudaFuncSetAttribute(gemm_tma_kernel<BN_, MODE_, KB_, false, NP>, cudaFuncAttributeMaxDynamicSharedMemorySize, TmaCfg<BN_, MODE_, KB_, false, NP>::kSmemBytes);
  PF_TMA_VARIANTS(PF_TMA_CFG)
#undef PF_TMA_CFG
#define PF_TMA_CFG_PP(BN_, KB_)                                                                                               \
  if (e == cudaSuccess) e = cudaFuncSetAttribute(gemm_tma_kernel<BN_, MODE_GEMM, KB_, true, NP>, cudaFuncAttributeMaxDynamicSharedMemorySize, TmaCfg<BN_, MODE_GEMM, KB_, true, NP>::kSmemBytes);
  PF_TMA_PINGPONG_VARIANTS(PF_TMA_CFG_PP)
#undef PF_TMA_CFG_PP
  return e;
}
inline cudaError_t gemm_tma_configure_device(int np) {
  return np == 1 ? gemm_tma_configure_np<1>() : (np == 3 ? gemm_tma_configure_np<3>() : cudaErrorInvalidValue);
}

template <int NP>
inline int tma_stages_np(int mode, int bn, int kb, bool pp) {
#define PF_TMA_NS(BN_, MODE_, KB_) if (!pp && mode == MODE_ && bn == BN_ && kb == KB_) return TmaCfg<BN_, MODE_, KB_, false, NP>::kStages;
  PF_TMA_VARIANTS(PF_TMA_NS)
#undef PF_TMA_NS
#define PF_TMA_NS_PP(BN_, KB_) if (pp && mode == MODE_GEMM && bn == BN_ && kb == KB_) return TmaCfg<BN_, MODE_GEMM, KB_, true, NP>::kStages;
  PF_TMA_PINGPONG_VARIANTS(PF_TMA_NS_PP)
#undef PF_TMA_NS_PP
  return 0;
}
inline int tma_stages(int mode, int bn, int kb, bool pp, int np) {
  return np == 1 ? tma_stages_np<1>(mode, bn, kb, pp) : (np == 3 ? tma_stages_np<3>(mode, bn, kb, pp) : 0);
}

inline const char* gemm_tma_check(int mode, const TmaGemmParams& p, int bn, int kb, bool pred, bool pp, int np) {
  const int ns = tma_stages(mode, bn, kb, pp, np);
  if (!ns) return pp ? "no ping-pong engine instantiation for this (mode, bn, kb)" : "no engine instantiation for this (mode, bn, kb)";
  if (mode == MODE_GEMM) return p.K % kb ? "GEMM mode: K must be a multiple of the K step" : nullptr;
  if (p.phase4 && (p.N != 128 || bn != 128)) return "phase4 needs N = 128 in one 128-wide tile";
  if (pred && bn != (p.phase4 ? 128 : 32)) return "the fused prediction tail needs N = 32 (phase4: 128) in one tile";
  const bool resident = p.Cin == 64 && 9 * (64 / kb) <= ns;
  if ((resident || pred) && cdiv(p.N, bn) > 1) return "resident weights (Cin = 64) and the prediction tail need one N tile per launch";
  return nullptr;
}

template <int NP>
inline cudaError_t gemm_tma_launch_np(int mode, const TmaMaps& maps, const TmaGemmParams& p, int bn, int kb, bool pp, int sm_count, cudaStream_t st,
                                      const PredTail* pred) {
#define PF_TMA_CASE(BN_, MODE_, KB_) if (!pp && mode == MODE_ && bn == BN_ && kb == KB_) return gemm_tma_launch_bn<BN_, MODE_, KB_, false, NP>(maps, p, sm_count, st, pred);
  PF_TMA_VARIANTS(PF_TMA_CASE)
#undef PF_TMA_CASE
#define PF_TMA_CASE_PP(BN_, KB_) if (pp && mode == MODE_GEMM && bn == BN_ && kb == KB_) return gemm_tma_launch_bn<BN_, MODE_GEMM, KB_, true, NP>(maps, p, sm_count, st, pred);
  PF_TMA_PINGPONG_VARIANTS(PF_TMA_CASE_PP)
#undef PF_TMA_CASE_PP
  return cudaErrorInvalidValue;
}
inline cudaError_t gemm_tma_launch(int mode, const TmaMaps& maps, const TmaGemmParams& p, int bn, int kb, bool pp, int np, int sm_count, cudaStream_t st,
                                   const PredTail* pred = nullptr) {
  if (np == 1) return gemm_tma_launch_np<1>(mode, maps, p, bn, kb, pp, sm_count, st, pred);
  if (np == 3) return gemm_tma_launch_np<3>(mode, maps, p, bn, kb, pp, sm_count, st, pred);
  return cudaErrorInvalidValue;
}

}
```

Measured before the change: 787.6.

## Fuse ConvNeXt MLP pointwise GEMMs into one TMA kernel keeping hidden in smem

Adds a MODE_MLP variant of the TMA/wgmma GEMM kernel that computes pw1 + bias + GELU into a 64-wide hidden chunk in shared memory, splits it to bf16 hi/lo, and immediately accumulates it through pw2 into the output accumulator. The param-net ConvNeXt blocks with C=96 use it instead of two separate GEMMs. This avoids writing and re-reading the 4C hidden activation through global memory and removes one launch per block. The cost is serialised per-chunk work (wait<0>, named barriers, GELU in the consumer warps) and fewer ring stages because of the extra y/hidden buffers.

```diff
diff --git a/include/pf_b200.h b/include/pf_b200.h
--- a/include/pf_b200.h
+++ b/include/pf_b200.h
@@ -161,6 +161,8 @@
 } pf_tma_op;
 int pf_op_tma(pf_tma_op* op, void* stream);
 int pf_op_tma_bf16(pf_tma_op* op, void* stream);
+int pf_op_mlp(const void* y_hi, const void* y_lo, int ldy, int64_t M, int C, int hidden, const void* w1_hi, const void* w1_lo, const float* b1,
+              const void* w2_hi, const void* w2_lo, const float* b2, const float* gamma, float* x, int fused, int bf16, void* stream);
 int pf_op_conv1_ring(const void* c_hi, const void* c_lo, int B, int H, int W, const float* wf, const float* bias, float* out,
                      const float* pg_w, const float* pg_b, float* pg_out, const float* pl_w, const float* pl_b, float* pl_out, void* stream);
 int pf_tma_pick_tile(int mode, int64_t M, int N, int K, int sm_count, int* bn, int* kb);
diff --git a/perspectivefields_b200/_native.py b/perspectivefields_b200/_native.py
--- a/perspectivefields_b200/_native.py
+++ b/perspectivefields_b200/_native.py
@@ -143,6 +143,7 @@
         "pf_op_conv_gemm": (i32, [vp, i32, i32, i32, i32, vp, vp, vp, i32, i32, i32, i32, i32, i32, i32, vp, i32, vp, vp]),
         "pf_op_tma": (i32, [ctypes.POINTER(pf_tma_op), vp]),
         "pf_op_tma_bf16": (i32, [ctypes.POINTER(pf_tma_op), vp]),
+        "pf_op_mlp": (i32, [vp, vp, i32, i64, i32, i32, vp, vp, vp, vp, vp, vp, vp, vp, i32, i32, vp]),
         "pf_op_conv1_ring": (i32, [vp, vp, i32, i32, i32, vp, vp, vp, vp, vp, vp, vp, vp, vp, vp]),
         "pf_tma_pick_tile": (i32, [i32, i64, i32, i32, i32, ctypes.POINTER(i32), ctypes.POINTER(i32)]),
         "pf_set_option": (i32, [vp, ctypes.c_char_p, i32]),
@@ -200,7 +201,7 @@
            "pf_profile_kernels_read", "pf_set_option", "pf_debug_enable", "pf_debug_count", "pf_debug_name", "pf_debug_numel",
            "pf_debug_copy", "pf_camera_fields", "pf_camera_fields_vp", "pf_pano_views", "pf_equi_views", "pf_draw_fields", "pf_comm_unique_id", "pf_comm_create", "pf_comm_destroy", "pf_gather",
            "pf_jpeg_create", "pf_jpeg_destroy", "pf_jpeg_info", "pf_jpeg_decode_batch",
-           "pf_op_conv_gemm", "pf_op_tma", "pf_op_tma_bf16", "pf_op_conv1_ring", "pf_tma_pick_tile", "pf_op_layernorm", "pf_op_attention",
+           "pf_op_conv_gemm", "pf_op_tma", "pf_op_tma_bf16", "pf_op_mlp", "pf_op_conv1_ring", "pf_tma_pick_tile", "pf_op_layernorm", "pf_op_attention",
            "pf_op_attention_mma", "pf_op_attention_tc", "pf_op_attention_tc_bf16", "pf_op_attention_tc_keys", "pf_op_dwconv3x3_gelu",
            "pf_op_dwconv7x7", "pf_op_upsample2x", "pf_op_preprocess", "pf_op_preprocess_sized", "pf_op_fill_stream", "pf_op_resize_u8",
            "pf_op_resize_f32", "pf_op_argmax_decode", "pf_op_pred_argmax_decode", "pf_op_postprocess", "pf_op_postprocess_sized"]
diff --git a/perspectivefields_b200/csrc/gemm_tma.cuh b/perspectivefields_b200/csrc/gemm_tma.cuh
--- a/perspectivefields_b200/csrc/gemm_tma.cuh
+++ b/perspectivefields_b200/csrc/gemm_tma.cuh
@@ -5,7 +5,8 @@
 
 namespace pf {
 
-constexpr int MODE_GEMM = 0, MODE_HALO = 1;
+constexpr int MODE_GEMM = 0, MODE_HALO = 1, MODE_MLP = 2;
+constexpr int kMlpChunk = 64;
 constexpr int kTmaThreads = 384;
 constexpr int kHaloBytes = 180 * 128;
 
@@ -26,25 +27,31 @@
   __nv_bfloat16* Shi; __nv_bfloat16* Slo; int lds, s_coff, s_gcoff, split_relu;
   const float* pred_w; const float* pred_b; float* pred_out; int pred_nc, pred_mode;
   int phase4;
+  const float* bias1;
 };
 
 template <int BN, int MODE, int KB, bool PP = false, int NP = 3> struct TmaCfg {
   static_assert(KB == 32 || KB == 64, "KB");
   static_assert(BN % 32 == 0 && BN <= 256, "BN");
   static_assert(!PP || MODE == MODE_GEMM, "the ping-pong schedule is a GEMM-mode schedule");
+  static_assert(MODE != MODE_MLP || (KB == 32 && BN % 32 == 0), "MODE_MLP: BN = C, y / W1 K steps of 32");
   static_assert(NP == 1 || NP == 3, "NP");
   static constexpr int kPlanes = NP == 3 ? 2 : 1;
   static constexpr int kTileM = PP ? 64 : 128;
   static constexpr int kBPlane = BN * KB * 2;
   static constexpr int kAPlane = kTileM * KB * 2;
-  static constexpr int kStage = (MODE == MODE_GEMM ? kPlanes * kAPlane : 0) + kPlanes * kBPlane;
+  static constexpr int kMlpWPlane = BN * 128;
+  static constexpr int kStage = MODE == MODE_MLP ? kPlanes * kMlpWPlane : (MODE == MODE_GEMM ? kPlanes * kAPlane : 0) + kPlanes * kBPlane;
   static constexpr int kABuf = kPlanes * kHtPlaneBytes;
+  static constexpr int kYPlane = 128 * BN * 2;
+  static constexpr int kHPlane = 64 * kMlpChunk * 2;
+  static constexpr int kPre = MODE == MODE_HALO ? 2 * kABuf : (MODE == MODE_MLP ? kPlanes * kYPlane + 2 * kPlanes * kHPlane : 0);
   static constexpr int kAccPitch = 68;
   static constexpr int kAccStage = 2 * 64 * kAccPitch * 4;
-  static constexpr int kBudget = 225 * 1024 - kAccStage - (MODE == MODE_HALO ? 2 * kABuf : 0);
+  static constexpr int kBudget = 225 * 1024 - kAccStage - kPre;
   static constexpr int kStagesRaw = kBudget / kStage;
   static constexpr int kStages = kStagesRaw > 16 ? 16 : kStagesRaw;
-  static constexpr int kSmemBytes = (MODE == MODE_HALO ? 2 * kABuf : 0) + kStages * kStage + kAccStage + 512 + 1024;
+  static constexpr int kSmemBytes = kPre + kStages * kStage + kAccStage + 512 + 1024;
   static_assert(kStages >= 2, "ring too shallow");
   static_assert(kSmemBytes <= 227 * 1024, "shared memory per block");
 };
@@ -60,12 +67,14 @@
   asm volatile("cp.async.bulk.tensor.4d.shared::cluster.global.mbarrier::complete_tx::bytes [%0], [%1, {%3, %4, %5, %6}], [%2];\n"
                ::"r"(dst), "l"(reinterpret_cast<uint64_t>(map)), "r"(bar), "r"(c0), "r"(c1), "r"(c2), "r"(c3) : "memory");
 }
+__device__ __forceinline__ void fence_proxy_async_smem() { asm volatile("fence.proxy.async.shared::cta;\n" ::: "memory"); }
 __device__ __forceinline__ void tma_prefetch_desc(const CUtensorMap* map) {
   asm volatile("prefetch.tensormap [%0];\n" ::"l"(reinterpret_cast<uint64_t>(map)) : "memory");
 }
 
 struct TmaMaps {
   CUtensorMap a_hi, a_lo, a2_hi, a2_lo, b_hi, b_lo;
+  CUtensorMap b2_hi, b2_lo;
 };
 
 template <int BN, int MODE, int KB, bool PP = false, int NP = 3>
@@ -80,7 +89,7 @@
   const uint32_t sbase = (raw + 1023u) & ~1023u;
   unsigned char* sm = smem_dyn + (sbase - raw);
   const uint32_t a_base = sbase;
-  const uint32_t ring = sbase + (MODE == MODE_HALO ? 2 * Cfg::kABuf : 0);
+  const uint32_t ring = sbase + Cfg::kPre;
   const uint32_t acc_base = ring + NS * Cfg::kStage;
   const uint32_t bars = acc_base + Cfg::kAccStage;
   auto full_b = [&](int s) { return bars + 8u * s; };
@@ -91,15 +100,16 @@
 
   const int tid = threadIdx.x, lane = tid & 31, warp = tid >> 5;
   const int n_tiles = cdiv(p.N, BN);
-  const int m_tiles = MODE == MODE_GEMM ? cdiv(p.M, Cfg::kTileM) : p.B * tiles_x * tiles_y;
+  const int m_tiles = MODE != MODE_HALO ? cdiv(p.M, Cfg::kTileM) : p.B * tiles_x * tiles_y;
   const int total_tiles = m_tiles * n_tiles * p.groups;
   const int nchunks = MODE == MODE_HALO ? p.Cin / 64 : 0;
-  const int nk = MODE == MODE_GEMM ? p.K / KB : nchunks * SPC;
+  const int nk = MODE == MODE_GEMM ? p.K / KB : (MODE == MODE_MLP ? 2 * (p.K / kMlpChunk) : nchunks * SPC);
   const bool b_resident = MODE == MODE_HALO && nchunks == 1 && SPC <= NS;
 
   if (tid == 0) {
     tma_prefetch_desc(&maps.a_hi); tma_prefetch_desc(&maps.b_hi);
     if (kLo) { tma_prefetch_desc(&maps.a_lo); tma_prefetch_desc(&maps.b_lo); }
+    if (MODE == MODE_MLP) { tma_prefetch_desc(&maps.b2_hi); if (kLo) tma_prefetch_desc(&maps.b2_lo); }
     for (int s = 0; s < NS; ++s) { mbar_init(full_b(s), 1); mbar_init(empty_b(s), kConsumerWarps); }
     for (int i = 0; i < 2; ++i) { mbar_init(full_a(i), 1); mbar_init(empty_a(i), kConsumerWarps); mbar_init(order_b(i), 4); }
     fence_mbar_init();
@@ -117,7 +127,36 @@
 
   if (warp < 4) {
     asm volatile("setmaxnreg.dec.sync.aligned.u32 40;\n");
-    if (warp == 0 && lane == 0) {
+    if constexpr (MODE == MODE_MLP) {
+      if (warp == 0 && lane == 0) {
+        int it = 0, ity = 0;
+        for (int tile = blockIdx.x; tile < total_tiles; tile += gridDim.x, ++ity) {
+          int mt, g, n0;
+          decode(tile, mt, g, n0);
+          mbar_wait(empty_a(0), (ity & 1) ^ 1);
+          mbar_expect_tx(full_a(0), Cfg::kPlanes * Cfg::kYPlane);
+          for (int kb = 0; kb < BN / 32; ++kb) {
+            tma_load_2d(sbase + kb * 128 * 64, &maps.a_hi, full_a(0), p.a_c0 + kb * 32, mt * 128);
+            if (kLo) tma_load_2d(sbase + Cfg::kYPlane + kb * 128 * 64, &maps.a_lo, full_a(0), p.a_c0 + kb * 32, mt * 128);
+          }
+          for (int kc = 0; kc < nk; ++kc, ++it) {
+            const int s = it % NS, j = kc >> 1;
+            mbar_wait(empty_b(s), ((it / NS) & 1) ^ 1);
+            mbar_expect_tx(full_b(s), Cfg::kStage);
+            const uint32_t st = ring + s * Cfg::kStage;
+            if ((kc & 1) == 0) {
+              for (int kb = 0; kb < BN / 32; ++kb) {
+                tma_load_2d(st + kb * 64 * 64, &maps.b_hi, full_b(s), kb * 32, j * kMlpChunk);
+                if (kLo) tma_load_2d(st + Cfg::kMlpWPlane + kb * 64 * 64, &maps.b_lo, full_b(s), kb * 32, j * kMlpChunk);
+              }
+            } else {
+              tma_load_2d(st, &maps.b2_hi, full_b(s), j * kMlpChunk, 0);
+              if (kLo) tma_load_2d(st + Cfg::kMlpWPlane, &maps.b2_lo, full_b(s), j * kMlpChunk, 0);
+            }
+          }
+        }
+      }
+    } else if (warp == 0 && lane == 0) {
       int it = 0;
       for (int tile = blockIdx.x; tile < total_tiles; tile += gridDim.x) {
         int mt, g, n0;
@@ -184,68 +223,159 @@
       it = tl * nk;
       if (tl > 0) mbar_wait(order_b(wg ^ 1), ((tl - 1) >> 1) & 1);
     }
-    int prev_s = -1, prev_buf = -1;
-    fence_regs(acc);
-    for (int kc = 0; kc < nk; ++kc, ++it) {
-      const int s = it % NS;
-      uint32_t a_hi, a_lo;
-      bool chunk_end = false;
-      int buf = 0;
-      if (MODE == MODE_HALO) {
-        const int c = kc / SPC, u = kc - c * SPC;
-        const int tap = KB == 32 ? (u >> 1) : u, ky = tap / 3, kx = tap - ky * 3;
-        buf = ita & 1;
-        if (u == 0) mbar_wait(full_a(buf), (ita >> 1) & 1);
-        a_hi = a_base + buf * Cfg::kABuf + ((ky + 8 * wg) * kHtHaloW + kx) * 128 + (KB == 32 ? (u & 1) * 64 : 0);
-        a_lo = a_hi + kHtPlaneBytes;
-        chunk_end = u == SPC - 1;
-      } else {
-        a_hi = ring + s * Cfg::kStage + (PP ? 0 : wg * 64 * KB * 2);
-        a_lo = a_hi + Cfg::kAPlane;
-      }
-      const int sb = b_resident ? kc : s;
-      if (!b_resident || tl == 0) mbar_wait(full_b(sb), b_resident ? 0 : ((it / NS) & 1));
-      const uint32_t b_hi = ring + sb * Cfg::kStage + (MODE == MODE_GEMM ? Cfg::kPlanes * Cfg::kAPlane : 0);
-      const uint64_t dah = MODE == MODE_HALO ? ht_a_desc(a_hi) : wgmma_tile_desc<KB>(a_hi);
-      const uint64_t dbh = wgmma_tile_desc<KB>(b_hi);
-      wgmma_fence();
-      if (kLo) {
-        const uint64_t dal = MODE == MODE_HALO ? ht_a_desc(a_lo) : wgmma_tile_desc<KB>(a_lo);
-        const uint64_t dbl = wgmma_tile_desc<KB>(b_hi + Cfg::kBPlane);
-#pragma unroll
-        for (int kk = 0; kk < KB / 16; ++kk) {
-          const uint32_t first = (kc | kk) ? 1u : 0u;
-          wgmma_bf16<BN>(acc, dal + 2 * kk, dbh + 2 * kk, first);
-          wgmma_bf16<BN>(acc, dah + 2 * kk, dbl + 2 * kk, 1u);
-          wgmma_bf16<BN>(acc, dah + 2 * kk, dbh + 2 * kk, 1u);
-        }
-      } else {
-#pragma unroll
-        for (int kk = 0; kk < KB / 16; ++kk) wgmma_bf16<BN>(acc, dah + 2 * kk, dbh + 2 * kk, (kc | kk) ? 1u : 0u);
-      }
-      wgmma_commit();
-      wgmma_wait<1>();
+    if constexpr (MODE == MODE_MLP) {
+      constexpr int kYRows = 64 * 64;
+      float hacc[kMlpChunk / 2];
+      const uint32_t ya = sbase + wg * kYRows;
+      const uint32_t hb = sbase + Cfg::kPlanes * Cfg::kYPlane + wg * Cfg::kPlanes * Cfg::kHPlane;
+      unsigned char* hs = sm + (hb - sbase);
+      const int nch = p.K / kMlpChunk;
+      const int frow = (wt >> 5) * 16 + (lane >> 2), fcol = 2 * (lane & 3);
+      int prev_s2 = -1;
+      mbar_wait(full_a(0), ita & 1);
+      fence_regs(acc);
+      for (int j = 0; j < nch; ++j) {
+        const int s1 = it % NS;
+        mbar_wait(full_b(s1), (it / NS) & 1);
+        const uint32_t w1 = ring + s1 * Cfg::kStage;
+        wgmma_fence();
+#pragma unroll
+        for (int kb = 0; kb < BN / 32; ++kb) {
+          const uint64_t dah = wgmma_tile_desc<32>(ya + kb * 128 * 64), dbh = wgmma_tile_desc<32>(w1 + kb * 64 * 64);
+#pragma unroll
+          for (int kk = 0; kk < 2; ++kk) {
+            const uint32_t first = (kb | kk) ? 1u : 0u;
+            if (kLo) {
+              const uint64_t dal = wgmma_tile_desc<32>(ya + Cfg::kYPlane + kb * 128 * 64), dbl = wgmma_tile_desc<32>(w1 + Cfg::kMlpWPlane + kb * 64 * 64);
+              wgmma_bf16<kMlpChunk>(hacc, dal + 2 * kk, dbh + 2 * kk, first);
+              wgmma_bf16<kMlpChunk>(hacc, dah + 2 * kk, dbl + 2 * kk, 1u);
+              wgmma_bf16<kMlpChunk>(hacc, dah + 2 * kk, dbh + 2 * kk, 1u);
+            } else {
+              wgmma_bf16<kMlpChunk>(hacc, dah + 2 * kk, dbh + 2 * kk, first);
+            }
+          }
+        }
+        wgmma_commit();
+        wgmma_wait<0>();
+        fence_regs(hacc);
+        fence_regs(acc);
+        if (lane == 0) {
+          mbar_arrive(empty_b(s1));
+          if (prev_s2 >= 0) mbar_arrive(empty_b(prev_s2));
+          if (j == nch - 1) mbar_arrive(empty_a(0));
+        }
+        ++it;
+        named_bar_sync(1 + wg, 128);
+        const float* __restrict__ b1 = p.bias1 ? p.bias1 + j * kMlpChunk : nullptr;
+#pragma unroll
+        for (int jb = 0; jb < kMlpChunk / 8; ++jb) {
+          const int col = jb * 8 + fcol;
+          float2 bv = make_float2(0.f, 0.f);
+          if (b1) bv = __ldg(reinterpret_cast<const float2*>(b1 + col));
+#pragma unroll
+          for (int hh = 0; hh < 2; ++hh) {
+            const int row = frow + 8 * hh;
+            float v0 = hacc[4 * jb + 2 * hh], v1 = hacc[4 * jb + 2 * hh + 1];
+            if (b1) { v0 += bv.x; v1 += bv.y; }
+            v0 = gelu_erf(v0); v1 = gelu_erf(v1);
+            uint32_t h2, l2;
+            split_bf16x2(v0, v1, h2, l2);
+            const int off = row * 128 + ((jb ^ (row & 7)) << 4) + fcol * 2;
+            *reinterpret_cast<uint32_t*>(hs + off) = h2;
+            if (kLo) *reinterpret_cast<uint32_t*>(hs + Cfg::kHPlane + off) = l2;
+          }
+        }
+        fence_proxy_async_smem();
+        named_bar_sync(1 + wg, 128);
+        const int s2 = it % NS;
+        mbar_wait(full_b(s2), (it / NS) & 1);
+        const uint32_t w2 = ring + s2 * Cfg::kStage;
+        const uint64_t dhh = wgmma_tile_desc<64>(hb), dwh = wgmma_tile_desc<64>(w2);
+        wgmma_fence();
+#pragma unroll
+        for (int kk = 0; kk < kMlpChunk / 16; ++kk) {
+          const uint32_t first = (j | kk) ? 1u : 0u;
+          if (kLo) {
+            const uint64_t dhl = wgmma_tile_desc<64>(hb + Cfg::kHPlane), dwl = wgmma_tile_desc<64>(w2 + Cfg::kMlpWPlane);
+            wgmma_bf16<BN>(acc, dhl + 2 * kk, dwh + 2 * kk, first);
+            wgmma_bf16<BN>(acc, dhh + 2 * kk, dwl + 2 * kk, 1u);
+            wgmma_bf16<BN>(acc, dhh + 2 * kk, dwh + 2 * kk, 1u);
+          } else {
+            wgmma_bf16<BN>(acc, dhh + 2 * kk, dwh + 2 * kk, first);
+          }
+        }
+        wgmma_commit();
+        prev_s2 = s2;
+        ++it;
+      }
+      wgmma_wait<0>();
+      fence_regs(acc);
+      if (lane == 0 && prev_s2 >= 0) mbar_arrive(empty_b(prev_s2));
+      ++ita;
+    } else {
+      int prev_s = -1, prev_buf = -1;
+      fence_regs(acc);
+      for (int kc = 0; kc < nk; ++kc, ++it) {
+        const int s = it % NS;
+        uint32_t a_hi, a_lo;
+        bool chunk_end = false;
+        int buf = 0;
+        if (MODE == MODE_HALO) {
+          const int c = kc / SPC, u = kc - c * SPC;
+          const int tap = KB == 32 ? (u >> 1) : u, ky = tap / 3, kx = tap - ky * 3;
+          buf = ita & 1;
+          if (u == 0) mbar_wait(full_a(buf), (ita >> 1) & 1);
+          a_hi = a_base + buf * Cfg::kABuf + ((ky + 8 * wg) * kHtHaloW + kx) * 128 + (KB == 32 ? (u & 1) * 64 : 0);
+          a_lo = a_hi + kHtPlaneBytes;
+          chunk_end = u == SPC - 1;
+        } else {
+          a_hi = ring + s * Cfg::kStage + (PP ? 0 : wg * 64 * KB * 2);
+          a_lo = a_hi + Cfg::kAPlane;
+        }
+        const int sb = b_resident ? kc : s;
+        if (!b_resident || tl == 0) mbar_wait(full_b(sb), b_resident ? 0 : ((it / NS) & 1));
+        const uint32_t b_hi = ring + sb * Cfg::kStage + (MODE == MODE_GEMM ? Cfg::kPlanes * Cfg::kAPlane : 0);
+        const uint64_t dah = MODE == MODE_HALO ? ht_a_desc(a_hi) : wgmma_tile_desc<KB>(a_hi);
+        const uint64_t dbh = wgmma_tile_desc<KB>(b_hi);
+        wgmma_fence();
+        if (kLo) {
+          const uint64_t dal = MODE == MODE_HALO ? ht_a_desc(a_lo) : wgmma_tile_desc<KB>(a_lo);
+          const uint64_t dbl = wgmma_tile_desc<KB>(b_hi + Cfg::kBPlane);
+  #pragma unroll
+          for (int kk = 0; kk < KB / 16; ++kk) {
+            const uint32_t first = (kc | kk) ? 1u : 0u;
+            wgmma_bf16<BN>(acc, dal + 2 * kk, dbh + 2 * kk, first);
+            wgmma_bf16<BN>(acc, dah + 2 * kk, dbl + 2 * kk, 1u);
+            wgmma_bf16<BN>(acc, dah + 2 * kk, dbh + 2 * kk, 1u);
+          }
+        } else {
+  #pragma unroll
+          for (int kk = 0; kk < KB / 16; ++kk) wgmma_bf16<BN>(acc, dah + 2 * kk, dbh + 2 * kk, (kc | kk) ? 1u : 0u);
+        }
+        wgmma_commit();
+        wgmma_wait<1>();
+        if (lane == 0 && prev_s >= 0) {
+          if (!b_resident) mbar_arrive(empty_b(prev_s));
+          if (MODE == MODE_HALO && prev_buf >= 0) mbar_arrive(empty_a(prev_buf));
+        }
+        prev_s = s;
+        prev_buf = chunk_end ? buf : -1;
+        if (MODE == MODE_HALO && chunk_end) ++ita;
+      }
+      if (PP && lane == 0) mbar_arrive(order_b(wg));
+      wgmma_wait<0>();
+      fence_regs(acc);
       if (lane == 0 && prev_s >= 0) {
         if (!b_resident) mbar_arrive(empty_b(prev_s));
         if (MODE == MODE_HALO && prev_buf >= 0) mbar_arrive(empty_a(prev_buf));
       }
-      prev_s = s;
-      prev_buf = chunk_end ? buf : -1;
-      if (MODE == MODE_HALO && chunk_end) ++ita;
-    }
-    if (PP && lane == 0) mbar_arrive(order_b(wg));
-    wgmma_wait<0>();
-    fence_regs(acc);
-    if (lane == 0 && prev_s >= 0) {
-      if (!b_resident) mbar_arrive(empty_b(prev_s));
-      if (MODE == MODE_HALO && prev_buf >= 0) mbar_arrive(empty_a(prev_buf));
     }
 
     long long m;
     bool valid;
     int cls_off = 0;
     int bimg = 0, oy = 0, ox = 0;
-    if (MODE == MODE_GEMM) {
+    if (MODE != MODE_HALO) {
       m = (long long)mt * Cfg::kTileM + r;
       valid = m < p.M;
     } else {
@@ -426,7 +556,7 @@
           if (col >= BN || n0 + col >= p.N) continue;
           long long mr;
           bool vr;
-          if (MODE == MODE_GEMM) {
+          if (MODE != MODE_HALO) {
             mr = (long long)mt * Cfg::kTileM + (PP ? 0 : wg * 64) + rr;
             vr = mr < p.M;
           } else {
diff --git a/perspectivefields_b200/csrc/pf_b200.cu b/perspectivefields_b200/csrc/pf_b200.cu
--- a/perspectivefields_b200/csrc/pf_b200.cu
+++ b/perspectivefields_b200/csrc/pf_b200.cu
@@ -341,6 +341,9 @@
   static cudaError_t gemm_tma_halo_mode(const TmaMaps& maps, const TmaGemmParams& p, int bn, int kb, bool pp, int np, int sms, cudaStream_t st, const PredTail* pred) {
     return gemm_tma_launch(MODE_HALO, maps, p, bn, kb, pp, np, sms, st, pred);
   }
+  static cudaError_t gemm_tma_mlp_mode(const TmaMaps& maps, const TmaGemmParams& p, int np, int sms, cudaStream_t st) {
+    return gemm_tma_mlp_launch(maps, p, np, sms, st);
+  }
   int np() const { return e->bf16 ? 1 : 3; }
   int force_bn = 0, force_kb = 0;
   int force_sched = 0;
@@ -431,6 +434,44 @@
     if (msg) return fail(PF_ERR_CUDA, "%s", msg);
     maps.a2_hi = maps.a_hi; maps.a2_lo = maps.a_lo;
     return launch_tma(MODE_GEMM, maps, p, bn, kb, pp);
+  }
+  int tmlp(const SplitT& y, long long M, int C, const GemmW& w1, const GemmW& w2, int hidden, const float* gamma, float* x) {
+    if (dry) return PF_OK;
+    if (!tma_mlp_fused(C, hidden) || y.ld % 8 || M < 1 || M > INT32_MAX) return fail(PF_ERR_ARG, "tmlp: no fused MLP for C = %d, hidden %d, %lld rows", C, hidden, M);
+    TmaGemmParams p{};
+    p.M = (int)M; p.Cin = C; p.N = C; p.K = hidden; p.groups = 1;
+    p.bias1 = w1.b;
+    p.bias = w2.b; p.bias_mode = w2.b ? 1 : 0;
+    p.gamma = gamma;
+    p.res = x; p.ldr = C;
+    p.C = x; p.ldc = C;
+    TmaMaps maps{};
+    const char* msg = nullptr;
+    if (!msg) msg = map2d(&maps.a_hi, y.hi, y.ld, M, y.ld, 128, 32);
+    if (!msg) msg = map2d(&maps.a_lo, y.lo, y.ld, M, y.ld, 128, 32);
+    if (!msg) msg = map2d(&maps.b_hi, w1.hi, C, hidden, C, kMlpChunk, 32);
+    if (!msg) msg = map2d(&maps.b_lo, w1.lo, C, hidden, C, kMlpChunk, 32);
+    if (!msg) msg = map2d(&maps.b2_hi, w2.hi, hidden, C, hidden, C, 64);
+    if (!msg) msg = map2d(&maps.b2_lo, w2.lo, hidden, C, hidden, C, 64);
+    if (msg) return fail(PF_ERR_CUDA, "%s", msg);
+    maps.a2_hi = maps.a_hi; maps.a2_lo = maps.a_lo;
+    if (e->profile) {
+      pf_engine::ProfRec r{};
+      for (cudaEvent_t* ev : {&r.a, &r.b}) {
+        if (e->ev_pool.empty()) { CU(cudaEventCreate(ev)); }
+        else { *ev = e->ev_pool.back(); e->ev_pool.pop_back(); }
+      }
+      r.flops = 2.0 * 2.0 * (double)M * C * hidden;
+      r.cfg = 5;
+      r.M = (int)M; r.N = C; r.K = hidden; r.KH = 1; r.stride = 1; r.groups = 1; r.Cin = C;
+      CU(cudaEventRecord(r.a, st));
+      LAUNCHED(gemm_tma_mlp_mode(maps, p, np(), e->sm_count, st));
+      CU(cudaEventRecord(r.b, st));
+      e->prof.push_back(r);
+      return PF_OK;
+    }
+    LAUNCHED(gemm_tma_mlp_mode(maps, p, np(), e->sm_count, st));
+    return PF_OK;
   }
   int thalo(const SplitT& A, int a_c0, int a_gc, const SplitT* A2, int c_split, int a2_c0, int B, int H, int W, int Cin, const GemmW& w, int N,
             int groups, int bias_gstride, const Epi& o, const PredTail* pred = nullptr) {
@@ -876,7 +917,8 @@
       const long long rows = (long long)n * rh * rw;
       float* yf = ar.f(rows * C);
       SplitT y = F.salloc(rows, C);
-      SplitT h = F.salloc(rows, 4 * C);
+      const bool fused_mlp = tma_mlp_fused(C, 4 * C);
+      SplitT h = fused_mlp ? SplitT() : F.salloc(rows, 4 * C);
       for (int j = 0; j < kCnxDepths[s]; ++j) {
         const CnxBlockW& b = e->pn_blocks[s][j];
         if (e->use_dwln) {
@@ -885,8 +927,12 @@
           if (!dry) LAUNCHED(launch_pdl(dwconv7x7_kernel, dim3(ew_grid((long long)n * ((rh + 1) / 2) * ((rw + PF_DW7_PX - 1) / PF_DW7_PX) * (C / 4))), dim3(256), 0, st, x, yf, n, rh, rw, C, b.dw_w, b.dw_b));
           TRY(F.ln_split(yf, y, rows, C, b.ln, 1e-6f));
         }
-        { Epi o; o.S = h; o.act = 2; TRY(F.tgemm(y, rows, C, 0, b.pw1, 4 * C, o)); }
-        { Epi o; o.C = x; o.ldc = C; o.res = x; o.ldr = C; o.gamma = b.gamma; TRY(F.tgemm(h, rows, 4 * C, 0, b.pw2, C, o)); }
+        if (fused_mlp) {
+          TRY(F.tmlp(y, rows, C, b.pw1, b.pw2, 4 * C, b.gamma, x));
+        } else {
+          { Epi o; o.S = h; o.act = 2; TRY(F.tgemm(y, rows, C, 0, b.pw1, 4 * C, o)); }
+          { Epi o; o.C = x; o.ldc = C; o.res = x; o.ldr = C; o.gamma = b.gamma; TRY(F.tgemm(h, rows, 4 * C, 0, b.pw2, C, o)); }
+        }
       }
       TRY(F.tapf(x, rows * C, "cnx.s%d", s));
     }
@@ -1385,6 +1431,40 @@
 }
 int pf_op_tma(pf_tma_op* op, void* stream) { return op_tma(op, stream, false); }
 int pf_op_tma_bf16(pf_tma_op* op, void* stream) { return op_tma(op, stream, true); }
+int pf_op_mlp(const void* y_hi, const void* y_lo, int ldy, int64_t M, int C, int hidden, const void* w1_hi, const void* w1_lo, const float* b1,
+              const void* w2_hi, const void* w2_lo, const float* b2, const float* gamma, float* x, int fused, int bf16, void* stream) {
+  if (!y_hi || !y_lo || !w1_hi || !w1_lo || !w2_hi || !w2_lo || !x) return fail(PF_ERR_ARG, "pf_op_mlp: null argument");
+  if (M < 1 || M > INT32_MAX || C < 32 || C % 32 || hidden < 64 || hidden % 64 || ldy < C || ldy % 8)
+    return fail(PF_ERR_ARG, "pf_op_mlp: M %lld, C %d, hidden %d, ldy %d", (long long)M, C, hidden, ldy);
+  if (fused && !tma_mlp_fused(C, hidden)) return fail(PF_ERR_ARG, "pf_op_mlp: no fused MLP for C = %d, hidden %d", C, hidden);
+  TRY(configure_current_device());
+  int dev = 0;
+  CU(cudaGetDevice(&dev));
+  cudaDeviceProp prop;
+  CU(cudaGetDeviceProperties(&prop, dev));
+  pf_engine tmp;
+  tmp.device = dev;
+  tmp.sm_count = prop.multiProcessorCount;
+  tmp.bf16 = bf16 != 0;
+  cudaStream_t st = (cudaStream_t)stream;
+  Fwd F{&tmp, Arena{}, st, false, 1};
+  const SplitT y{(__nv_bfloat16*)y_hi, (__nv_bfloat16*)y_lo, ldy};
+  const GemmW w1{(const __nv_bfloat16*)w1_hi, (const __nv_bfloat16*)w1_lo, b1}, w2{(const __nv_bfloat16*)w2_hi, (const __nv_bfloat16*)w2_lo, b2};
+  if (fused) return F.tmlp(y, M, C, w1, w2, hidden, gamma, x);
+  const long long hb = M * hidden * 2 + 1024;
+  char* scratch = nullptr;
+  CU(cudaMalloc(&scratch, 2 * hb));
+  F.ar.base = scratch; F.ar.cap = 2 * hb;
+  SplitT h = F.salloc(M, hidden);
+  int r = PF_OK;
+  { Fwd::Epi o; o.S = h; o.act = 2; r = F.tgemm(y, M, C, 0, w1, hidden, o); }
+  if (r == PF_OK) { Fwd::Epi o; o.C = x; o.ldc = C; o.res = x; o.ldr = C; o.gamma = gamma; r = F.tgemm(h, M, hidden, 0, w2, C, o); }
+  cudaError_t se = cudaStreamSynchronize(st);
+  cudaFree(scratch);
+  if (r != PF_OK) return r;
+  if (se != cudaSuccess) return fail(PF_ERR_CUDA, "pf_op_mlp: %s", cudaGetErrorString(se));
+  return PF_OK;
+}
 int pf_op_conv1_ring(const void* c_hi, const void* c_lo, int B, int H, int W, const float* wf, const float* bias, float* out,
                      const float* pg_w, const float* pg_b, float* pg_out, const float* pl_w, const float* pl_b, float* pl_out, void* stream) {
   if (!c_hi || !c_lo || !wf || !bias) return fail(PF_ERR_ARG, "pf_op_conv1_ring: null argument");
diff --git a/perspectivefields_b200/csrc/tma_host.cuh b/perspectivefields_b200/csrc/tma_host.cuh
--- a/perspectivefields_b200/csrc/tma_host.cuh
+++ b/perspectivefields_b200/csrc/tma_host.cuh
@@ -127,6 +127,8 @@
 #define PF_TMA_PINGPONG_VARIANTS(X)                                                                                         \
   X(256, 32) X(224, 32) X(192, 32) X(160, 32) X(128, 32) X(96, 32) X(64, 32) X(32, 32) X(64, 64) X(32, 64)
 
+#define PF_TMA_MLP_VARIANTS(X) X(96)
+
 template <int NP>
 inline cudaError_t gemm_tma_configure_np() {
   cudaError_t e = cudaSuccess;
@@ -138,6 +140,10 @@
   if (e == cudaSuccess) e = cudaFuncSetAttribute(gemm_tma_kernel<BN_, MODE_GEMM, KB_, true, NP>, cudaFuncAttributeMaxDynamicSharedMemorySize, TmaCfg<BN_, MODE_GEMM, KB_, true, NP>::kSmemBytes);
   PF_TMA_PINGPONG_VARIANTS(PF_TMA_CFG_PP)
 #undef PF_TMA_CFG_PP
+#define PF_TMA_CFG_MLP(C_)                                                                                                   \
+  if (e == cudaSuccess) e = cudaFuncSetAttribute(gemm_tma_kernel<C_, MODE_MLP, 32, false, NP>, cudaFuncAttributeMaxDynamicSharedMemorySize, TmaCfg<C_, MODE_MLP, 32, false, NP>::kSmemBytes);
+  PF_TMA_MLP_VARIANTS(PF_TMA_CFG_MLP)
+#undef PF_TMA_CFG_MLP
   return e;
 }
 inline cudaError_t gemm_tma_configure_device(int np) {
@@ -187,4 +193,28 @@
   return cudaErrorInvalidValue;
 }
 
-}
+inline bool tma_mlp_fused(int C, int hidden) {
+  bool ok = false;
+#define PF_TMA_MLP_OK(C_) ok = ok || C == C_;
+  PF_TMA_MLP_VARIANTS(PF_TMA_MLP_OK)
+#undef PF_TMA_MLP_OK
+  return ok && hidden > 0 && hidden % kMlpChunk == 0;
+}
+template <int NP>
+inline cudaError_t gemm_tma_mlp_launch_np(const TmaMaps& maps, const TmaGemmParams& p, int sm_count, cudaStream_t st) {
+  const long long tiles = cdivl(p.M, 128);
+  const unsigned grid = (unsigned)(tiles < sm_count ? tiles : sm_count);
+#define PF_TMA_MLP_CASE(C_)                                                                                                  \
+  if (p.N == C_) return launch_pdl(gemm_tma_kernel<C_, MODE_MLP, 32, false, NP>, dim3(grid), dim3(kTmaThreads), TmaCfg<C_, MODE_MLP, 32, false, NP>::kSmemBytes, st, maps, p, 0, 0);
+  PF_TMA_MLP_VARIANTS(PF_TMA_MLP_CASE)
+#undef PF_TMA_MLP_CASE
+  return cudaErrorInvalidValue;
+}
+inline cudaError_t gemm_tma_mlp_launch(const TmaMaps& maps, const TmaGemmParams& p, int np, int sm_count, cudaStream_t st) {
+  if (!tma_mlp_fused(p.N, p.K)) return cudaErrorInvalidValue;
+  if (np == 1) return gemm_tma_mlp_launch_np<1>(maps, p, sm_count, st);
+  if (np == 3) return gemm_tma_mlp_launch_np<3>(maps, p, sm_count, st);
+  return cudaErrorInvalidValue;
+}
+
+}
```

New measurement: 801.0, median of 6. 1.02x the previous value.
